# GBATZOLIS/ID-diff

Measured on AMD Instinct MI355X. Metric: score-vector evals/sec (rows of S per second incl. the per-point spectrum), 32x32 ncsnpp, higher is better.
Workload: dtype f32 (3x3 convs: Winograd, fp32 transforms, contraction on pairs of fp16 values -- 22 significand bits, 3 products, fp32 accumulate (F(4,3) along the rows x 3 filter rows); 1x1/attention/dense contractions: fp32 operands split exactly into 3 bf16, 6 partial products, fp32 accumulate; the q/k/v projec

## Files before the change

### id-diff_amd/_lib.py

```python
import ctypes
import os
import subprocess
from typing import NamedTuple, Optional

import torch

_HERE = os.path.dirname(os.path.abspath(__file__))
_VARIANT = os.environ.get("IDIFF_LIB_VARIANT", "")
_LIB_PATH = os.path.join(_HERE, "csrc", f"libidiff_hip.{_VARIANT}.so" if _VARIANT else "libidiff_hip.so")
_lib = None

ACT = {None: 0, "none": 0, "linear": 0, "silu": 1, "swish": 1, "elu": 2, "relu": 3, "lrelu": 4}

c_i, c_i64, c_f, c_d, c_p = ctypes.c_int, ctypes.c_int64, ctypes.c_float, ctypes.c_double, ctypes.c_void_p


class Epilogue(ctypes.Structure):
    _fields_ = [("bias", c_p), ("rowbias", c_p), ("ld_rowbias", c_i64), ("rows_per_group", c_i), ("act", c_i),
                ("residual", c_p), ("ld_residual", c_i64), ("out_scale", c_f), ("rowscale", c_p), ("colstats", c_p)]


_SIGNATURES = {
    "idiff_abi_version": (c_i, []),
    "idiff_last_error": (ctypes.c_char_p, []),
    "idiff_source_stamp": (ctypes.c_char_p, []),
    "idiff_variant_flags": (ctypes.c_char_p, []),
    "idiff_set_option": (c_i, [ctypes.c_char_p, c_i]),
    "idiff_gemm_pairs_ok": (c_i, [c_i, c_i, c_i, c_i]),
    "idiff_gemm_pairs_scale_f32": (c_i, [c_p, c_i64, c_i, c_i, c_p, c_p]),
    "idiff_gemm_pairs_f32": (c_i, [c_p, c_i64, c_i64, c_p, c_i64, c_i64, c_p, c_i, c_p, c_p, c_i64, c_i64, c_i, c_i, c_i, c_i, c_p, c_p]),
    "idiff_pairs_act_scale_f32": (c_i, [c_p, c_i, c_i, c_p, c_i, c_i, c_i, c_i, c_p, c_p]),
    "idiff_gemm_pairs_2src_f32": (c_i, [c_p, c_p, c_i64, c_i, c_p, c_p, c_i64, c_p, c_p, c_i64, c_i, c_i, c_i, c_p, c_p]),
    "idiff_set_thread_option": (c_i, [ctypes.c_char_p, c_i, c_i]),
    "idiff_upfirdn2d_f32": (c_i, [c_p, c_p, c_p] + [c_i] * 14 + [c_p]),
    "idiff_upfirdn2d_route": (ctypes.c_char_p, [c_p, c_p] + [c_i] * 14),
    "idiff_upfirdn2d_gn_f32": (c_i, [c_p, c_p, c_p, c_i, c_p] + [c_i] * 14 + [c_p]),
    "idiff_upfirdn2d_gn_ok": (c_i, [c_p, c_p, c_i, c_p] + [c_i] * 14),
    "idiff_fused_bias_act_f32": (c_i, [c_p, c_p, c_p, c_p, c_i64, c_i, c_i, c_i, c_i, c_f, c_f, c_p]),
    "idiff_upfirdn2d_f16": (c_i, [c_p, c_p, c_p] + [c_i] * 14 + [c_p]),
    "idiff_upfirdn2d_f64": (c_i, [c_p, c_p, c_p] + [c_i] * 14 + [c_p]),
    "idiff_fused_bias_act_f16": (c_i, [c_p, c_p, c_p, c_p, c_i64, c_i, c_i, c_i, c_i, c_f, c_f, c_p]),
    "idiff_fused_bias_act_f64": (c_i, [c_p, c_p, c_p, c_p, c_i64, c_i, c_i, c_i, c_i, c_f, c_f, c_p]),
    "idiff_gemm_f32": (c_i, [c_p, c_i64, c_i64, c_p, c_i64, c_i64, c_p, c_i64, c_i64, c_i, c_i, c_i, c_i,
                             ctypes.POINTER(Epilogue), c_p]),
    "idiff_gemm_2src_f32": (c_i, [c_p, c_p, c_i64, c_i, c_p, c_i64, c_p, c_i64, c_i, c_i, c_i, ctypes.POINTER(Epilogue), c_p]),
    "idiff_conv2d_nhwc_f32": (c_i, [c_p, c_p, c_p] + [c_i] * 10 + [ctypes.POINTER(Epilogue), c_p]),
    "idiff_gemm_route": (ctypes.c_char_p, [c_p, c_i64, c_i64, c_p, c_i64, c_i64, c_p, c_i64, c_i64, c_i, c_i, c_i, c_i,
                                           ctypes.POINTER(Epilogue), c_i]),
    "idiff_conv2d_route": (ctypes.c_char_p, [c_p, c_p, c_p] + [c_i] * 10 + [ctypes.POINTER(Epilogue)]),
    "idiff_gemm_colstats_split": (c_i, [c_i, c_i, c_i, c_i64, c_i64, c_i]),
    "idiff_conv2d_colstats_split": (c_i, [c_i] * 10),
    "idiff_conv2d_winograd_ok": (c_i, [c_i] * 5),
    "idiff_winograd_weight_floats": (c_i64, [c_i, c_i]),
    "idiff_winograd_pack_f32": (c_i, [c_p, c_p, c_i, c_i, c_p]),
    "idiff_conv2d_winograd_f32": (c_i, [c_p, c_p, c_p] + [c_i] * 5 + [ctypes.POINTER(Epilogue), c_p]),
    "idiff_conv2d_winograd_colstats_split": (c_i, [c_i] * 5),
    "idiff_conv2d_winograd43_ok": (c_i, [c_i] * 5),
    "idiff_conv2d_winograd43_colstats_split": (c_i, [c_i] * 5),
    "idiff_winograd43_weight_floats": (c_i64, [c_i, c_i]),
    "idiff_winograd43_pack_f32": (c_i, [c_p, c_p, c_i, c_i, c_p]),
    "idiff_conv2d_winograd43_f32": (c_i, [c_p, c_p, c_p, c_i, c_i, c_i, c_i, c_i, ctypes.POINTER(Epilogue), c_p]),
    "idiff_conv2d_winograd43h_ok": (c_i, [c_i] * 5),
    "idiff_winograd43h_weight_floats": (c_i64, [c_i, c_i]),
    "idiff_winograd43h_pack_f32": (c_i, [c_p, c_p, c_i, c_i, c_p]),
    "idiff_conv2d_winograd43h_f32": (c_i, [c_p, c_p, c_p, c_i, c_i, c_i, c_i, c_i, ctypes.POINTER(Epilogue), c_p]),
    "idiff_conv2d_wino1d_ok": (c_i, [c_i] * 5),
    "idiff_conv2d_wino1d_colstats_split": (c_i, [c_i] * 5),
    "idiff_wino1d_weight_floats": (c_i64, [c_i, c_i]),
    "idiff_wino1d_pack_f32": (c_i, [c_p, c_p, c_i, c_i, c_p]),
    "idiff_conv2d_wino1d_f32": (c_i, [c_p, c_p, c_p, c_i, c_i, c_i, c_i, c_i, ctypes.POINTER(Epilogue), c_p]),
    "idiff_conv2d_wino1d_gn_ok": (c_i, [c_i] * 6),
    "idiff_conv2d_wino1d_normload_ok": (c_i, [c_i] * 5),
    "idiff_conv2d_wino1d_normload_f32": (c_i, [c_p, c_p, c_p, c_i, c_i, c_i, c_i, c_i, ctypes.POINTER(Epilogue), c_p, c_i, c_p]),
    "idiff_conv2d_wino1d_normload_2src_ok": (c_i, [c_i] * 6),
    "idiff_conv2d_wino1d_normload_2src_f32": (c_i, [c_p, c_i, c_p, c_i, c_p, c_p, c_i, c_i, c_i, c_i, ctypes.POINTER(Epilogue), c_p, c_i, c_p]),
    "idiff_groupnorm_coef_f32": (c_i, [c_p, c_i, c_i, c_p, c_i, c_i, c_i, c_i, c_i, c_f, c_p, c_p, c_p, c_p]),
    "idiff_conv2d_wino1d_gn_f32": (c_i, [c_p, c_p, c_p, c_i, c_i, c_i, c_i, c_i, ctypes.POINTER(Epilogue), c_i, c_p, c_p, c_f, c_i, c_p]),
    "idiff_conv2d_winograd_split_ok": (c_i, [c_i] * 5),
    "idiff_winograd_split_weight_floats": (c_i64, [c_i, c_i]),
    "idiff_winograd_pack_split_f32": (c_i, [c_p, c_p, c_i, c_i, c_p]),
    "idiff_conv2d_winograd_split_f32": (c_i, [c_p, c_p, c_p] + [c_i] * 5 + [ctypes.POINTER(Epilogue), c_p]),
    "idiff_groupnorm_finalize_f32": (c_i, [c_p, c_i, c_i, c_p, c_i, c_i, c_i, c_i, c_i, c_f, c_p, c_p]),
    "idiff_groupnorm_nsplit": (c_i, [c_i, c_i, c_i]),
    "idiff_groupnorm_stats_f32": (c_i, [c_p, c_i, c_p, c_i, c_i, c_i, c_i, c_f, c_p, c_p, c_p]),
    "idiff_groupnorm_apply_f32": (c_i, [c_p, c_i, c_p, c_i, c_i, c_i, c_i, c_p, c_p, c_p, c_p, c_i64, c_i, c_p, c_p]),
    "idiff_groupnorm_apply_colstats_f32": (c_i, [c_p, c_i, c_p, c_i, c_i, c_i, c_i, c_p, c_i, c_p, c_i, c_f, c_p, c_p, c_p, c_i64,
                                                 c_i, c_p, c_p]),
    "idiff_groupnorm_apply_route": (ctypes.c_char_p, [c_p, c_i, c_p, c_i, c_i, c_i, c_i, c_p, c_p, c_p, c_p]),
    "idiff_groupnorm_apply_colstats_route": (ctypes.c_char_p, [c_p, c_i, c_p, c_i, c_i, c_i, c_i, c_p, c_i, c_p, c_i, c_p, c_p, c_p]),
    "idiff_softmax_rows_f32": (c_i, [c_p, c_p, c_i64, c_i, c_f, c_p]),
    "idiff_softmax_rows_route": (ctypes.c_char_p, [c_p, c_p, c_i64, c_i, c_f]),
    "idiff_attention256_ok": (c_i, [c_i, c_i, c_i]),
    "idiff_attention256_f32": (c_i, [c_p, c_i64, c_p, c_p, c_p, c_p, c_p, c_i, c_i, c_i, c_f, c_p]),
    "idiff_attention_heads_ok": (c_i, [c_i, c_i, c_i, c_i]),
    "idiff_attention_heads_f32": (c_i, [c_p, c_i64, c_p, c_p, c_p, c_p, c_p, c_i, c_i, c_i, c_i, c_f, c_p]),
    "idiff_attention256_route": (ctypes.c_char_p, [c_p, c_i64, c_p, c_p, c_p, c_p, c_p, c_i, c_i, c_i]),
    "idiff_attention_heads_route": (ctypes.c_char_p, [c_p, c_i64, c_p, c_p, c_p, c_p, c_p, c_i, c_i, c_i, c_i]),
    "idiff_affine_act_f32": (c_i, [c_p, c_p, c_i64, c_f, c_f, c_i, c_p, c_i64, c_p]),
    "idiff_add_scale_f32": (c_i, [c_p, c_p, c_p, c_i64, c_f, c_p]),
    "idiff_affine_act_route": (ctypes.c_char_p, [c_p, c_p, c_i64, c_p, c_i64]),
    "idiff_add_scale_route": (ctypes.c_char_p, [c_p, c_p, c_p, c_i64]),
    "idiff_concat_cols_route": (ctypes.c_char_p, [c_p, c_i, c_p, c_i, c_p, c_i64]),
    "idiff_fourier_embed_f32": (c_i, [c_p, c_p, c_p, c_i, c_i, c_p]),
    "idiff_positional_embed_f32": (c_i, [c_p, c_p, c_i, c_i, c_f, c_i, c_p]),
    "idiff_concat_cols_f32": (c_i, [c_p, c_i, c_p, c_i, c_p, c_i64, c_p]),
    "idiff_nchw_to_nhwc_f32": (c_i, [c_p, c_p, c_i, c_i, c_i, c_i, c_f, c_f, c_p]),
    "idiff_nhwc_to_nchw_f32": (c_i, [c_p, c_p, c_i, c_i, c_i, c_i, c_p, c_p]),
    "idiff_resample2x_nhwc_f32": (c_i, [c_p, c_p, c_i, c_i, c_i, c_i, c_i, c_p]),
    "idiff_perturb_f32": (c_i, [c_p, c_p, c_p, c_p, c_p, c_i64, c_i64, c_p]),
    "idiff_perturb_randn_f32": (c_i, [c_p, c_p, c_p, c_p, c_i64, c_i64, c_i64, ctypes.c_uint64, c_p, c_p]),
    "idiff_spectrum_workspace_bytes": (c_i64, [c_i, c_i, c_i]),
    "idiff_spectrum_f32": (c_i, [c_p, c_i, c_i, c_i, c_p, c_i64, c_p, c_p, c_p]),
    "idiff_colmean_f64": (c_i, [c_p, c_i, c_i, c_i, c_p, c_p, c_p]),
    "idiff_centered_gram_f64": (c_i, [c_p, c_p, c_i, c_i, c_i, c_p, c_p]),
    "idiff_centered_gram_rows_f64": (c_i, [c_p, c_p, c_i, c_i, c_i, c_i, c_p, c_p]),
    "idiff_symmetrize_upper_f64": (c_i, [c_p, c_i, c_p]),
    "idiff_symtridiag_scratch_doubles": (c_i64, [c_i]),
    "idiff_symband_ld": (c_i, []),
    "idiff_symband_f64": (c_i, [c_p, c_i, c_p, c_p]),
    "idiff_symtridiag_f64": (c_i, [c_p, c_i, c_i, c_p, c_p, c_p, c_p]),
    "idiff_symtridiag_plan": (c_i, [c_i]),
    "idiff_tridiag_eigvals_f64": (c_i, [c_p, c_p, c_i, c_i, c_p, c_p]),
    "idiff_sym_lowvecs_scratch_doubles": (c_i64, [c_i, c_i]),
    "idiff_sym_lowvecs_f64": (c_i, [c_p, c_i, c_i, c_p, c_p, c_p, c_p, c_p]),
    "idiff_sym_topvecs_scratch_doubles": (c_i64, [c_i, c_i, c_i]),
    "idiff_sym_topvecs_f64": (c_i, [c_p, c_i, c_i, c_i, c_d, c_d, c_d, c_i, c_i, c_p, c_p, c_p, c_p, c_p]),
    "idiff_knn_workspace_bytes": (c_i64, [c_i, c_i, c_i]),
    "idiff_knn_f32": (c_i, [c_p, c_i, c_i, c_i, c_p, c_i64, c_p, c_p, c_p, c_p]),
    "idiff_apsp_tile": (c_i, []),
    "idiff_knn_graph_f64": (c_i, [c_p, c_p, c_i, c_i, c_p, c_p]),
    "idiff_apsp_f64": (c_i, [c_p, c_i, c_p]),
    "idiff_double_center_scratch_doubles": (c_i64, [c_i]),
    "idiff_double_center_f64": (c_i, [c_p, c_i, c_p, c_p, c_p, c_p]),
    "idiff_component_labels_f64": (c_i, [c_p, c_i, c_p, c_p, c_p, c_p]),
    "idiff_component_bridges_workspace_bytes": (c_i64, [c_i]),
    "idiff_component_bridges_f64": (c_i, [c_p, c_i, c_i, c_p, c_i, c_p, c_i64, c_p, c_p, c_p, c_p]),
    "idiff_minplus_f64": (c_i, [c_p, c_i64, c_p, c_i64, c_p, c_i64, c_i, c_i, c_i, c_p]),
    "idiff_symmetrize_min_f64": (c_i, [c_p, c_i, c_p]),
    "idiff_knn_cross_workspace_bytes": (c_i64, [c_i, c_i]),
    "idiff_knn_cross_f64": (c_i, [c_p, c_i, c_p, c_i, c_i, c_i, c_p, c_i64, c_p, c_p, c_p]),
    "idiff_isomap_project_scratch_doubles": (c_i64, [c_i]),
    "idiff_isomap_project_f64": (c_i, [c_p, c_p, c_i, c_i, c_p, c_i, c_p, c_i, c_p, c_p, c_p, c_p, c_p]),
    "idiff_render_squares_f32": (c_i, [c_p, c_p, c_p, c_i, c_i, c_i, c_p]),
    "idiff_render_gaussians_f32": (c_i, [c_p, c_p, c_p, c_i, c_i, c_i, c_p]),
    "idiff_ksphere_union_ok": (c_i, [c_i, c_i, c_i]),
    "idiff_ksphere_union_score_f32": (c_i, [c_p, c_p, c_p, c_p, c_p, c_p, c_p, c_i, c_i, c_i, c_i, c_p]),
    "idiff_local_pca_ok": (c_i, [c_i, c_i, c_i, c_i]),
    "idiff_local_pca_chunk": (c_i, []),
    "idiff_local_pca_f64": (c_i, [c_p, c_i, c_i, c_p, c_p, c_i, c_i, c_i, c_p, c_p, c_p, c_p]),
    "idiff_empirical_score_ok": (c_i, [c_i64, c_i]),
    "idiff_empirical_score_f32": (c_i, [c_p, c_p, c_p, c_p, c_p, c_p, c_p, c_p, c_i, c_i64, c_i, c_p]),
    "idiff_empirical_jacobian_ok": (c_i, [c_i64, c_i]),
    "idiff_empirical_jacobian_f64": (c_i, [c_p, c_p, c_p, c_p, c_p, c_p, c_i, c_i64, c_i, c_p]),
    "idiff_gemm_nn_ok": (c_i, [c_i, c_i, c_i]),
    "idiff_gemm_nn_f32": (c_i, [c_p, c_i64, c_p, c_i64, c_p, c_i64, c_p, c_i64, c_i, c_i, c_i, c_p]),
    "idiff_gemm_tn_ok": (c_i, [c_i, c_i, c_i]),
    "idiff_gemm_tn_f32": (c_i, [c_p, c_i64, c_p, c_i64, c_p, c_i64, c_p, c_i, c_i, c_i, c_p]),
    "idiff_dsm_loss_grad_f32": (c_i, [c_p, c_p, c_p, c_p, c_i64, c_p, c_p, c_i, c_i, c_i, c_p]),
    "idiff_grad_sumsq_f32": (c_i, [c_p, c_i64, c_p, c_p, c_p]),
    "idiff_adam_step_f32": (c_i, [c_p, c_p, c_p, c_p, c_i64, c_p, c_d, c_d, c_d, c_d, c_d, c_d, c_i64, c_p]),
    "idiff_fcn_train_input_f32": (c_i, [c_p, c_p, c_p, c_p, c_p, c_p, c_i64, c_i, c_i, c_p]),
    "idiff_sampler_step_f32": (c_i, [c_p, c_i64, c_p, c_i64, c_p, c_i64, c_p, c_i64, c_p, c_i64, c_i64, c_i, c_d, c_d, c_d, c_p, c_d, c_d,
                                     ctypes.c_uint64, c_i64, c_i, c_f, c_p]),
    "idiff_sampler_noise_norm_f32": (c_i, [c_p, c_i64, c_i64, c_i, ctypes.c_uint64, c_i64, c_p, c_p, c_p]),
    "idiff_jvp_layer_ok": (c_i, [c_i, c_i, c_i]),
    "idiff_jvp_seed_f32": (c_i, [c_p, c_i64, c_p, c_i64, c_p, c_i64, c_i64, c_i, c_i, c_i, c_p]),
    "idiff_jvp_layer_f32": (c_i, [c_p, c_i64, c_i64, c_p, c_i64, c_p, c_i64, c_p, c_i64, c_i64, c_i, c_i, c_i, c_i, c_p]),
    "idiff_rk_stage_f64": (c_i, [c_p, c_i64, c_p, c_i64, c_i64, c_p, c_i, c_p, c_i64, c_p, c_i64, c_i64, c_i, c_i, c_f, c_p]),
    "idiff_rk_error_f64": (c_i, [c_p, c_i64, c_i64, c_p, c_p, c_i64, c_p, c_i64, c_i64, c_i, c_d, c_d, c_p, c_p, c_p]),
    "idiff_flow_rhs_f64": (c_i, [c_p, c_i64, c_p, c_i64, c_d, c_d, c_p, c_i64, c_i64, c_i, c_i, c_p, c_i64, c_p, c_i64, c_p, c_p]),
    "idiff_jvp_trace_f64": (c_i, [c_p, c_i64, c_i64, c_p, c_i64, c_p, c_i, c_i, c_i, c_p]),
}

EXPORTED_SYMBOLS = tuple(_SIGNATURES)


def library_path():
    return _LIB_PATH


def build(verbose=False):
    out = subprocess.run(["bash", os.path.join(_HERE, "csrc", "build.sh")], capture_output=True, text=True)
    if out.returncode != 0:
        raise RuntimeError("building libidiff_hip.so failed:\n" + out.stdout + out.stderr)
    if verbose:
        print(out.stdout.strip())
    return _LIB_PATH


def source_stamp():
    import hashlib
    csrc = os.path.join(_HERE, "csrc")
    names = sorted(f for f in os.listdir(csrc) if f.endswith(".hip") or f.endswith(".h"))
    h = hashlib.sha256()
    for f in [os.path.join(csrc, n) for n in names] + [os.path.join(os.path.dirname(_HERE), "include", "idiff_hip.h")]:
        with open(f, "rb") as fh:
            h.update(fh.read())
    return h.hexdigest()[:16]
# ... 48 lines not shown
    def __exit__(self, *exc):
        lib().idiff_set_thread_option(self.name, 0, 0)
        return False


def _check(rc, what):
    if rc != 0:
        msg = lib().idiff_last_error().decode(errors="replace")
        raise RuntimeError(f"{what} failed (code {rc}): {msg}")


def _stream():
    return torch.cuda.current_stream().cuda_stream


def _dev(t, name, dtype=torch.float32, contiguous=True):
    if not isinstance(t, torch.Tensor):
        raise TypeError(f"{name}: expected a torch.Tensor, got {type(t).__name__}")
    if t.device.type != "cuda":
        raise RuntimeError(f"{name}: expected a tensor on the MI355X (cuda device), got {t.device}; "
                           "id-diff_amd has no CPU path")
    if t.dtype != dtype:
        raise RuntimeError(f"{name}: expected dtype {dtype}, got {t.dtype}")
    if contiguous and not t.is_contiguous():
        raise RuntimeError(f"{name}: expected a contiguous tensor")
    return t


def _ptr(t):
    return 0 if t is None else t.data_ptr()


def make_epilogue(bias=None, rowbias=None, rows_per_group=1, act=None, residual=None, out_scale=1.0,
                  ld_rowbias=None, ld_residual=None, rowscale=None, colstats=None):
    ep = Epilogue()
    ep.bias = _ptr(bias)
    ep.rowbias = _ptr(rowbias)
    ep.ld_rowbias = (rowbias.stride(0) if ld_rowbias is None else ld_rowbias) if rowbias is not None else 0
    ep.rows_per_group = int(rows_per_group)
    ep.act = ACT[act]
    ep.residual = _ptr(residual)
    ep.ld_residual = (residual.shape[-1] if ld_residual is None else ld_residual) if residual is not None else 0
    ep.out_scale = float(out_scale)
    ep.rowscale = _ptr(rowscale)
    ep.colstats = _ptr(colstats)
    ep._keepalive = (bias, rowbias, residual, rowscale, colstats)
    return ep


def with_groupnorm(ep, groups, gamma, beta, eps, act):
    _dev(gamma, "gamma"); _dev(beta, "beta")
    ep.groupnorm = (int(groups), gamma, beta, float(eps), ACT[act])
    return ep


class NormLoad(NamedTuple):
    coef: torch.Tensor
    act: int
    x2: Optional[torch.Tensor]
    C1: Optional[int]


def with_normload(ep, coef, act, x2=None, C1=None):
    _dev(coef, "coef")
    if (x2 is None) != (C1 is None):
        raise RuntimeError("with_normload: a second source x2 and the first one's channel count C1 come together or not at all")
    if x2 is not None:
        _dev(x2, "x2")
    ep.normload = NormLoad(coef, ACT[act], x2, None if C1 is None else int(C1))
    return ep


def _ep_ref(epilogue, what):
    if epilogue is None:
        return None
    if getattr(epilogue, "normload", None) is not None:
        raise RuntimeError(f"{what}: the epilogue asks for a GroupNorm in the loader (with_normload), which only conv2d_wino1d serves")
    if getattr(epilogue, "groupnorm", None) is not None:
        raise RuntimeError(f"{what}: the epilogue asks for a fused GroupNorm (with_groupnorm), which only conv2d_wino1d serves")
    return ctypes.byref(epilogue)


OP_DTYPES = {torch.float32: "f32", torch.float16: "f16", torch.float64: "f64"}


def op_suffix(t, name):
    try:
        return OP_DTYPES[t.dtype]
    except KeyError:
        raise RuntimeError(f"{name}: dtype {t.dtype} is not one of float32 / float16 / float64 (the reference's native ops "
                           "dispatch on floating types and half, op/upfirdn2d_kernel.cu:311)") from None


def upfirdn2d_raw(x, k, out, major, in_h, in_w, minor, up_x, up_y, down_x, down_y, px0, px1, py0, py1):
    kh, kw = k.shape
    sfx = op_suffix(x, "upfirdn2d")
    if k.dtype != x.dtype or out.dtype != x.dtype:
        raise RuntimeError(f"upfirdn2d: input {x.dtype}, kernel {k.dtype} and output {out.dtype} must share one dtype")
    fn = getattr(lib(), "idiff_upfirdn2d_" + sfx)
    _check(fn(x.data_ptr(), k.data_ptr(), out.data_ptr(), major, in_h, in_w, minor, kh, kw,
              up_x, up_y, down_x, down_y, px0, px1, py0, py1, _stream()), "idiff_upfirdn2d_" + sfx)


def upfirdn2d_route(x, out, major, in_h, in_w, minor, kh, kw, up_x, up_y, down_x, down_y, px0, px1, py0, py1):
    addr = lambda t: t if isinstance(t, int) else t.data_ptr()
    name = lib().idiff_upfirdn2d_route(addr(x), addr(out), major, in_h, in_w, minor, kh, kw, up_x, up_y, down_x, down_y,
                                       px0, px1, py0, py1)
    return None if name is None else name.decode()


def upfirdn2d_gn(x, k, coef, act, out, major, in_h, in_w, minor, up_x, up_y, down_x, down_y, px0, px1, py0, py1):
    kh, kw = k.shape
    for t, name in ((x, "input"), (k, "kernel"), (coef, "coef"), (out, "output")):
        _dev(t, name)
    if coef.numel() != major * minor * 2:
        raise RuntimeError(f"upfirdn2d_gn: coef holds {coef.numel()} floats, [major, minor, 2] = {major * minor * 2} expected")
    _check(lib().idiff_upfirdn2d_gn_f32(x.data_ptr(), k.data_ptr(), coef.data_ptr(), ACT[act], out.data_ptr(), major, in_h, in_w, minor,
                                        kh, kw, up_x, up_y, down_x, down_y, px0, px1, py0, py1, _stream()), "idiff_upfirdn2d_gn_f32")


def upfirdn2d_gn_ok(x, coef, act, out, major, in_h, in_w, minor, kh, kw, up_x, up_y, down_x, down_y, px0, px1, py0, py1):
    addr = lambda t: t if isinstance(t, int) else t.data_ptr()
    return bool(lib().idiff_upfirdn2d_gn_ok(addr(x), addr(coef), ACT[act], addr(out), major, in_h, in_w, minor, kh, kw, up_x, up_y,
                                            down_x, down_y, px0, px1, py0, py1))


def upfirdn2d_out_size(in_size, up, down, pad0, pad1, k):
    return (in_size * up + pad0 + pad1 - k) // down + 1


def fused_bias_act(x, bias, ref, act, grad, alpha, scale):
    sfx = op_suffix(x, "fused_bias_act")
    _dev(x, "input", dtype=x.dtype)
    out = torch.empty_like(x)
    has_b = bias is not None and bias.numel() > 0
    has_r = ref is not None and ref.numel() > 0
    if has_b:
        _dev(bias, "bias", dtype=x.dtype)
        if x.ndim < 2 or bias.numel() != x.shape[1]:
            raise RuntimeError(f"bias has {bias.numel()} entries but input dim 1 is {tuple(x.shape)}")
    if has_r:
        _dev(ref, "refer", dtype=x.dtype)
        if ref.shape != x.shape:
            raise RuntimeError("refer must have the shape of input")
    step_b = 1
    for d in x.shape[2:]:
        step_b *= d
    _check(getattr(lib(), "idiff_fused_bias_act_" + sfx)(x.data_ptr(), _ptr(bias if has_b else None), _ptr(ref if has_r else None),
                                                         out.data_ptr(), x.numel(), step_b, bias.numel() if has_b else 0, act, grad,
                                                         alpha, scale, _stream()), "idiff_fused_bias_act_" + sfx)
    return out


def gemm(a, bt, out=None, epilogue=None, M=None, N=None, K=None, lda=None, ldb=None, ldc=None,
         batch=1, stride_a=0, stride_b=0, stride_c=0):
    explicit = M is not None
    _dev(a, "a", contiguous=not explicit); _dev(bt, "bt", contiguous=not explicit)
    if M is None:
        M, K = a.shape
        N = bt.shape[0]
        if bt.shape[1] != K:
            raise RuntimeError(f"gemm: inner dimensions differ: {tuple(a.shape)} x {tuple(bt.shape)}^T")
        lda, ldb = a.stride(0), bt.stride(0)
    if out is None:
        out = torch.empty((M, N) if batch == 1 else (batch, M, N), device=a.device, dtype=torch.float32)
        ldc = N
        stride_c = M * N
    elif ldc is None:
        ldc = out.stride(-2)
    _dev(out, "out", contiguous=not explicit)
    ep = _ep_ref(epilogue, "gemm")
    _check(lib().idiff_gemm_f32(a.data_ptr(), lda, stride_a, bt.data_ptr(), ldb, stride_b, out.data_ptr(), ldc, stride_c,
                                M, N, K, batch, ep, _stream()), "idiff_gemm_f32")
    return out


def gemm_pairs_ok(M, N, K, batch=1):
    return bool(lib().idiff_gemm_pairs_ok(M, N, K, batch))


def gemm_pairs_scale(w):
    _dev(w, "w")
    out = torch.empty(2, device=w.device, dtype=torch.float32)
    _check(lib().idiff_gemm_pairs_scale_f32(w.data_ptr(), w.stride(0), w.shape[0], w.shape[1], out.data_ptr(), _stream()),
           "idiff_gemm_pairs_scale_f32")
    return out


def gemm_pairs(a, bt, w_scale, out, epilogue=None, weight_is_a=False, M=None, N=None, K=None, lda=None, ldb=None, ldc=None,
               batch=1, stride_a=0, stride_b=0, stride_c=0, act_scale=None):
    explicit = M is not None
    _dev(a, "a", contiguous=not explicit); _dev(bt, "bt", contiguous=not explicit); _dev(out, "out", contiguous=not explicit)
    _dev(w_scale, "w_scale")
    if M is None:
        M, K = a.shape
        N = bt.shape[0]
        if bt.shape[1] != K or out.shape[0] != M or out.shape[1] != N:
            raise RuntimeError(f"gemm_pairs: shapes {tuple(a.shape)} x {tuple(bt.shape)}^T -> {tuple(out.shape)}")
        lda, ldb, ldc = a.stride(0), bt.stride(0), out.stride(0)
    ep = _ep_ref(epilogue, "gemm_pairs")
    _check(lib().idiff_gemm_pairs_f32(a.data_ptr(), lda, stride_a, bt.data_ptr(), ldb, stride_b, w_scale.data_ptr(), int(bool(weight_is_a)),
                                      _ptr(act_scale), out.data_ptr(), ldc, stride_c, M, N, K, batch, ep, _stream()), "idiff_gemm_pairs_f32")
    return out


def pairs_act_scale(stats1, C1, stats2, C2, B, HW):
    out = torch.empty(8, device=stats1[0].device, dtype=torch.float32)
    _check(lib().idiff_pairs_act_scale_f32(stats1[0].data_ptr(), stats1[1], C1, _ptr(stats2[0]) if stats2 is not None else None,
                                           stats2[1] if stats2 is not None else 0, C2, B, HW, out.data_ptr(), _stream()),
           "idiff_pairs_act_scale_f32")
    return out


def gemm_pairs_2src(a1, a2, act_scale, bt, w_scale, out, epilogue=None):
    _dev(a1, "a1"); _dev(a2, "a2"); _dev(bt, "bt"); _dev(out, "out"); _dev(act_scale, "act_scale"); _dev(w_scale, "w_scale")
    M, K1 = a1.shape
    K = K1 + a2.shape[1]
    if a2.shape[0] != M or a1.stride(0) != a2.stride(0) or bt.shape[1] != K:
        raise RuntimeError(f"gemm_pairs_2src: shapes {tuple(a1.shape)} | {tuple(a2.shape)} x {tuple(bt.shape)}^T")
    ep = _ep_ref(epilogue, "gemm_pairs_2src")
    _check(lib().idiff_gemm_pairs_2src_f32(a1.data_ptr(), a2.data_ptr(), a1.stride(0), K1, act_scale.data_ptr(), bt.data_ptr(), bt.stride(0),
                                           w_scale.data_ptr(), out.data_ptr(), out.stride(0), M, bt.shape[0], K, ep, _stream()),
           "idiff_gemm_pairs_2src_f32")
    return out


def gemm_normed(cache, a, w, out, epilogue=None, pairs=True):
    M, K = a.shape
    if not pairs or not gemm_pairs_ok(M, w.shape[0], K):
        return gemm(a, w, out=out, epilogue=epilogue)
    return gemm_pairs(a, w, _pairs_scale_of(cache, w), out, epilogue=epilogue)


def _pairs_scale_of(cache, w):
    sc = cache.setdefault("pairs_scale", {})
    if id(w) not in sc:
        sc[id(w)] = (gemm_pairs_scale(w), w)
    return sc[id(w)][0]


def gemm_weight_times_normed_t(cache, w, x, out, B, HW, C, pairs=True):
    kw = dict(M=C, N=HW, K=C, lda=C, ldb=C, ldc=HW, batch=B, stride_a=0, stride_b=HW * C, stride_c=C * HW)
    if not pairs or not gemm_pairs_ok(C, HW, C, B):
        return gemm(w, x, out=out, **kw)
    return gemm_pairs(w, x, _pairs_scale_of(cache, w), out, weight_is_a=True, **kw)


def gemm_2src(a1, a2, bt, out, epilogue=None):
    _dev(a1, "a1"); _dev(a2, "a2"); _dev(bt, "bt"); _dev(out, "out")
    M, K1 = a1.shape
    K = K1 + a2.shape[1]
    if a2.shape[0] != M or a1.stride(0) != a2.stride(0) or bt.shape[1] != K:
        raise RuntimeError(f"gemm_2src: shapes {tuple(a1.shape)} | {tuple(a2.shape)} x {tuple(bt.shape)}^T")
    ep = _ep_ref(epilogue, "gemm_2src")
    _check(lib().idiff_gemm_2src_f32(a1.data_ptr(), a2.data_ptr(), a1.stride(0), K1, bt.data_ptr(), bt.stride(0), out.data_ptr(),
                                     out.stride(0), M, bt.shape[0], K, ep, _stream()), "idiff_gemm_2src_f32")
    return out


def conv2d_nhwc(x, wt, out, B, H, W, Cin, Cout, KH, KW, stride, pad, epilogue=None, pad_hi=None):
    ep = _ep_ref(epilogue, "conv2d_nhwc")
    _check(lib().idiff_conv2d_nhwc_f32(x.data_ptr(), wt.data_ptr(), out.data_ptr(), B, H, W, Cin, Cout, KH, KW, stride,
                                       pad, pad if pad_hi is None else pad_hi, ep, _stream()), "idiff_conv2d_nhwc_f32")
    return out


def _addr(t):
    return t if isinstance(t, int) else t.data_ptr()


def gemm_route(a, bt, out, M, N, K, lda, ldb, ldc, epilogue=None, batch=1, stride_a=0, stride_b=0, stride_c=0, pairs=False):
    name = lib().idiff_gemm_route(_addr(a), lda, stride_a, _addr(bt), ldb, stride_b, _addr(out), ldc, stride_c, M, N, K, batch,
                                  _ep_ref(epilogue, "gemm_route"), int(bool(pairs)))
    return None if name is None else name.decode()


def conv2d_route(x, wt, out, B, H, W, Cin, Cout, KH, KW, stride, pad, epilogue=None, pad_hi=None):
    name = lib().idiff_conv2d_route(_addr(x), _addr(wt), _addr(out), B, H, W, Cin, Cout, KH, KW, stride, pad, pad if pad_hi is None else pad_hi,
                                    _ep_ref(epilogue, "conv2d_route"))
    return None if name is None else name.decode()


def _wino_pack(stem, name, wt, Cin, Cout):
    _dev(wt, "wt")
    if tuple(wt.shape) != (Cout, 3, 3, Cin):
        raise RuntimeError(f"{name}: expected {Cout}x3x3x{Cin} weights, got {tuple(wt.shape)}")
    entry = "idiff_winograd_pack_split_f32" if stem == "winograd_split" else f"idiff_{stem}_pack_f32"
    u = torch.empty(getattr(lib(), f"idiff_{stem}_weight_floats")(Cin, Cout), device=wt.device, dtype=torch.float32)
    _check(getattr(lib(), entry)(wt.data_ptr(), u.data_ptr(), Cin, Cout, _stream()), entry)
    return u


def _wino_conv(stem, packed_by, x, u, out, B, H, W, Cin, Cout, epilogue):
    want = getattr(lib(), f"idiff_{stem}_weight_floats")(Cin, Cout)
    if u.numel() != want:
        raise RuntimeError(f"conv2d_{stem}: a filter bank of {u.numel()} floats ({want} expected): pack it with {packed_by}")
    gn = getattr(epilogue, "groupnorm", None)
    nl = getattr(epilogue, "normload", None)
    if nl is not None and stem == "wino1d":
        if gn is not None:
            raise RuntimeError("conv2d_wino1d: a GroupNorm in the loader (with_normload) and one in the tail (with_groupnorm) in one launch")
        if nl.coef.numel() != B * Cin * 2:
            raise RuntimeError(f"conv2d_wino1d: {nl.coef.numel()} loader coefficients for [B, Cin, 2] = [{B}, {Cin}, 2]")
        if nl.x2 is not None:
            _check(lib().idiff_conv2d_wino1d_normload_2src_f32(x.data_ptr(), nl.C1, nl.x2.data_ptr(), Cin - nl.C1, u.data_ptr(), out.data_ptr(),
                                                               B, H, W, Cout, ctypes.byref(epilogue), nl.coef.data_ptr(), nl.act, _stream()),
                   "idiff_conv2d_wino1d_normload_2src_f32")
        else:
            _check(lib().idiff_conv2d_wino1d_normload_f32(x.data_ptr(), u.data_ptr(), out.data_ptr(), B, H, W, Cin, Cout, ctypes.byref(epilogue),
                                                          nl.coef.data_ptr(), nl.act, _stream()), "idiff_conv2d_wino1d_normload_f32")
        return out
    if gn is not None and stem == "wino1d":
        groups, gamma, beta, eps, act = gn
        if gamma.numel() != Cout or beta.numel() != Cout:
            raise RuntimeError(f"conv2d_wino1d: fused GroupNorm with {gamma.numel()} / {beta.numel()} gamma / beta entries for {Cout} channels")
        _check(lib().idiff_conv2d_wino1d_gn_f32(x.data_ptr(), u.data_ptr(), out.data_ptr(), B, H, W, Cin, Cout, ctypes.byref(epilogue), groups,
                                                gamma.data_ptr(), beta.data_ptr(), eps, act, _stream()), "idiff_conv2d_wino1d_gn_f32")
        return out
    ep = _ep_ref(epilogue, f"conv2d_{stem}")
    entry = f"idiff_conv2d_{stem}_f32"
    _check(getattr(lib(), entry)(x.data_ptr(), u.data_ptr(), out.data_ptr(), B, H, W, Cin, Cout, ep, _stream()), entry)
    return out


def conv2d_winograd_ok(B, H, W, Cin, Cout):
    return bool(lib().idiff_conv2d_winograd_ok(B, H, W, Cin, Cout))


def conv2d_winograd_split_ok(B, H, W, Cin, Cout):
    return bool(lib().idiff_conv2d_winograd_split_ok(B, H, W, Cin, Cout))


def conv2d_winograd_colstats_split(B, H, W, Cin, Cout):
    return lib().idiff_conv2d_winograd_colstats_split(B, H, W, Cin, Cout)


def winograd_pack(wt, Cin, Cout, split=False):
    return _wino_pack("winograd_split" if split else "winograd", "winograd_pack", wt, Cin, Cout)


def conv2d_winograd(x, u, out, B, H, W, Cin, Cout, epilogue=None, split=False):
    return _wino_conv("winograd_split" if split else "winograd", f"winograd_pack(..., split={split})", x, u, out, B, H, W, Cin, Cout, epilogue)


def conv2d_winograd43_ok(B, H, W, Cin, Cout):
    return bool(lib().idiff_conv2d_winograd43_ok(B, H, W, Cin, Cout))


def conv2d_winograd43h_ok(B, H, W, Cin, Cout):
    return bool(lib().idiff_conv2d_winograd43h_ok(B, H, W, Cin, Cout))


def conv2d_winograd43_colstats_split(B, H, W, Cin, Cout):
    return lib().idiff_conv2d_winograd43_colstats_split(B, H, W, Cin, Cout)


def winograd43_pack(wt, Cin, Cout, pairs=False):
    return _wino_pack("winograd43h" if pairs else "winograd43", "winograd43_pack", wt, Cin, Cout)


def conv2d_winograd43(x, u, out, B, H, W, Cin, Cout, epilogue=None, pairs=False):
    if pairs:
        return _wino_conv("winograd43h", "winograd43_pack(..., pairs=True)", x, u, out, B, H, W, Cin, Cout, epilogue)
    return _wino_conv("winograd43", "winograd43_pack", x, u, out, B, H, W, Cin, Cout, epilogue)


def conv2d_wino1d_ok(B, H, W, Cin, Cout):
    return bool(lib().idiff_conv2d_wino1d_ok(B, H, W, Cin, Cout))


def conv2d_wino1d_colstats_split(B, H, W, Cin, Cout):
    return lib().idiff_conv2d_wino1d_colstats_split(B, H, W, Cin, Cout)


def conv2d_wino1d_gn_ok(B, H, W, Cin, Cout, groups):
    return bool(lib().idiff_conv2d_wino1d_gn_ok(B, H, W, Cin, Cout, groups))


def conv2d_wino1d_normload_ok(B, H, W, Cin, Cout):
    return bool(lib().idiff_conv2d_wino1d_normload_ok(B, H, W, Cin, Cout))


def conv2d_wino1d_normload_2src_ok(B, H, W, C1, C2, Cout):
    return bool(lib().idiff_conv2d_wino1d_normload_2src_ok(B, H, W, C1, C2, Cout))


def groupnorm_coef(ws1, ns1, C1, ws2, ns2, C2, B, HW, G, eps, gamma, beta, coef):
    _dev(coef, "coef"); _dev(gamma, "gamma"); _dev(beta, "beta")
    if coef.numel() != B * (C1 + (C2 if ws2 is not None else 0)) * 2:
        raise RuntimeError(f"groupnorm_coef: coef holds {coef.numel()} floats, [B, C, 2] = {B * (C1 + C2) * 2} expected")
    _check(lib().idiff_groupnorm_coef_f32(ws1.data_ptr(), ns1, C1, _ptr(ws2), ns2, C2, B, HW, G, eps, gamma.data_ptr(), beta.data_ptr(),
                                          coef.data_ptr(), _stream()), "idiff_groupnorm_coef_f32")
    return coef


def groupnorm_reader_coef(ws, ns, C, B, HW, G, eps, gamma, beta, coef):
    _dev(coef, "coef"); _dev(gamma, "gamma"); _dev(beta, "beta")
    if coef.numel() != B * C * 2:
        raise RuntimeError(f"groupnorm_reader_coef: coef holds {coef.numel()} floats, [B, C, 2] = {B * C * 2} expected")
    _check(lib().idiff_groupnorm_coef_f32(ws.data_ptr(), ns, C, 0, 0, 0, B, HW, G, eps, gamma.data_ptr(), beta.data_ptr(),
                                          coef.data_ptr(), _stream()), "idiff_groupnorm_coef_f32")
    return coef


def wino1d_pack(wt, Cin, Cout):
    return _wino_pack("wino1d", "wino1d_pack", wt, Cin, Cout)

# ... 1114 lines not shown
```

### id-diff_amd/csrc/common.h

```cpp
#pragma once
#include <hip/hip_runtime.h>
#include <stdint.h>
#include <stdio.h>
#include <stdarg.h>

#include "../../include/idiff_hip.h"

#define IDIFF_API extern "C" __attribute__((visibility("default")))

namespace idiff {

void set_error(const char *fmt, ...);

inline int fail(const char *fmt, ...) {
  char buf[512];
  va_list ap;
  va_start(ap, fmt);
  vsnprintf(buf, sizeof(buf), fmt, ap);
  va_end(ap);
  set_error("%s", buf);
  return IDIFF_EINVAL;
}

inline int launch_status(const char *what) {
  hipError_t e = hipGetLastError();
  if (e != hipSuccess) {
    set_error("%s: %s", what, hipGetErrorString(e));
    return (int)e;
  }
  return 0;
}

enum Option { OPT_NO_WINOGRAD, OPT_NO_COLSTATS, OPT_NO_PIPE, OPT_SCALAR_EPILOGUE, OPT_DBUF_ONLY, OPT_TRIDIAG_ONESTAGE,
              OPT_UFD_ROWS, OPT_CHASE_WAVEFRONT, OPT_WINO_NGROUP, OPT_GRAM_SMALL_TILES, OPT_CHASE_SPIN_LIMIT, OPT_FAKE_CU_COUNT,
              OPT_SBR_SYNC, OPT_SBR_FULL, OPT_NO_SPLIT, OPT_WINO_SPLIT, OPT_SBR_LOOKAHEAD, OPT_NO_WINO43, OPT_NO_WINO43H, OPT_NO_PAIRS, OPT_PAIRS_MIN_TILES, OPT_NO_FUSED_ATTN, OPT_NO_WINO1D, OPT_NO_FUSED_GN, OPT_NO_FUSED_GN_LOAD, OPT_NO_FUSED_GN_LOAD_2SRC, OPT_NO_FUSED_GN_FIR, OPT_COUNT };
bool option(Option o);
int option_value(Option o);

struct AttrGuard { unsigned long long done_mask = 0; };
int set_dynamic_lds_once(AttrGuard &g, const void *const *fns, int n_fns, int bytes, const char *what);

bool conv3x3_narrow_ok(int B, int H, int W, int Cin, int Cout, int KH, int KW, int stride, int pad_lo, int pad_hi,
                       const idiff_epilogue *ep);
int conv3x3_narrow(const float *x, const float *wt, float *out, int B, int H, int W, int Cin, int Cout,
                   const idiff_epilogue *ep, hipStream_t stream);

template <class P> inline void set_epilogue(P &p, const idiff_epilogue *ep) {
  p.has_ep = ep ? 1 : 0;
  p.ep = ep ? *ep : idiff_epilogue{};
  if (!ep) p.ep.out_scale = 1.f;
  if (p.ep.rows_per_group <= 0) p.ep.rows_per_group = 1;
}

inline idiff_epilogue shift_epilogue(const idiff_epilogue &ep, int64_t m0) {
  idiff_epilogue e = ep;
  const int64_t g0 = m0 / (ep.rows_per_group > 0 ? ep.rows_per_group : 1);
  if (e.rowbias) e.rowbias += g0 * ep.ld_rowbias;
  if (e.residual) e.residual += m0 * ep.ld_residual;
  if (e.rowscale) e.rowscale += g0;
  return e;
}
inline int64_t host_cut_row(int64_t units, int64_t unit_rows, const idiff_epilogue *ep) {
  const int64_t rpg = (ep && ep->rows_per_group > 0) ? ep->rows_per_group : 1;
  const int64_t half = units / 2 * unit_rows;
  return unit_rows == 1 ? half / rpg * rpg : half % rpg ? 0 : half;
}
template <class Run> inline int run_cut(int64_t rows, int64_t cut, const idiff_epilogue *ep, bool first_only, Run run) {
  if (int rc = run((int64_t)0, cut, ep)) return rc;
  if (first_only) return 0;
  idiff_epilogue hi;
  if (ep) hi = shift_epilogue(*ep, cut);
  return run(cut, rows, ep ? &hi : nullptr);
}

static inline int ceil_div(int a, int b) { return (a + b - 1) / b; }
static inline int64_t ceil_div64(int64_t a, int64_t b) { return (a + b - 1) / b; }

static inline int streaming_grid(int64_t work_items, int block) {
  int64_t g = ceil_div64(work_items, block);
  const int64_t cap = 256 * 8;
  if (g > cap) g = cap;
  if (g < 1) g = 1;
  return (int)g;
}

__device__ __forceinline__ float act_apply(float v, int act) {
  switch (act) {
    case IDIFF_ACT_SILU: return v * __frcp_rn(1.0f + __expf(-v));
    case IDIFF_ACT_ELU: return v > 0.f ? v : (expf(v) - 1.0f);
    case IDIFF_ACT_RELU: return v > 0.f ? v : 0.f;
    case IDIFF_ACT_LRELU: return v > 0.f ? v : 0.2f * v;
    default: return v;
  }
}

}
```

### id-diff_amd/csrc/igemm.hip

```cpp
#include "common.h"
#include <type_traits>
#include <stdlib.h>

namespace {

typedef float floatx16 __attribute__((ext_vector_type(16)));

constexpr int BK = 32;
constexpr int LDS_PITCH = BK + 4;

struct IgemmParams {
  const float *A;
  const float *Bt;
  float *C;
  int64_t lda, ldb, ldc;
  int64_t strideA, strideB, strideC;
  int M, N, K;
  int tiles_m, tiles_n;
  int H, W, Cin, OH, OW, KW, stride, pad;
  idiff_epilogue ep;
  int has_ep;
  uint32_t a_bytes, b_bytes;
  int vec_ep;
  const float *A2;
  int K1;
  uint32_t a2_bytes;
  uint32_t c_bytes, res_bytes;
  int buf_ep;
  const float *scale_a, *scale_b;
};

__device__ __forceinline__ float4 ldg4(const float *p) { return *reinterpret_cast<const float4 *>(p); }

template <int BM, int BN, int WARPS_M, int WARPS_N, bool CONV, bool VEC>
__global__ void __launch_bounds__(WARPS_M *WARPS_N * 64)
igemm_kernel(const IgemmParams p) {
  constexpr int T = WARPS_M * WARPS_N * 64;
  constexpr int WTM = BM / WARPS_M, WTN = BN / WARPS_N;
  constexpr int TM = WTM / 32, TN = WTN / 32;
  constexpr int A_PER_T = BM * (BK / 4) / T;
  constexpr int B_PER_T = BN * (BK / 4) / T;
  static_assert(A_PER_T >= 1 && B_PER_T >= 1, "tile too small for the thread count");
  static_assert(T % (BK / 4) == 0, "a thread keeps one k-column of float4s");

  extern __shared__ __attribute__((aligned(16))) float lds[];
  float *As = lds;
  float *Bs = lds + 2 * BM * LDS_PITCH;

  const int nwg = p.tiles_m * p.tiles_n;
  int bid = blockIdx.x;
  {
    const int q = nwg >> 3, r = nwg & 7, xcd = bid & 7, local = bid >> 3;
    bid = (xcd < r ? xcd * (q + 1) : r * (q + 1) + (xcd - r) * q) + local;
  }
  const int tile_n = bid % p.tiles_n, tile_m = bid / p.tiles_n;
  const int batch = blockIdx.y;
  const int m0 = tile_m * BM, n0 = tile_n * BN;

  const int tid = threadIdx.x, lane = tid & 63, wave = tid >> 6;
  const int wm0 = (wave / WARPS_N) * WTM, wn0 = (wave % WARPS_N) * WTN;

  const float *Ab = p.A + (int64_t)batch * p.strideA;
  const float *Bb = p.Bt + (int64_t)batch * p.strideB;

  const int kc = (tid & 7) * 4;
  const int row_base = tid >> 3;
  constexpr int ROW_STEP = T / 8;

  int64_t a_off[A_PER_T];
  int a_iy[A_PER_T], a_ix[A_PER_T];
  bool a_ok[A_PER_T];
#pragma unroll
  for (int i = 0; i < A_PER_T; ++i) {
    const int m = m0 + row_base + i * ROW_STEP;
    a_ok[i] = m < p.M;
    if (CONV) {
      const int mm = a_ok[i] ? m : 0;
      const int ox = mm % p.OW;
      const int t = mm / p.OW;
      const int oy = t % p.OH;
      const int b = t / p.OH;
      a_off[i] = (int64_t)b * p.H * p.W;
      a_iy[i] = oy * p.stride - p.pad;
      a_ix[i] = ox * p.stride - p.pad;
    } else {
      a_off[i] = (int64_t)m * p.lda;
      a_iy[i] = a_ix[i] = 0;
    }
  }
  int64_t b_off[B_PER_T];
  bool b_ok[B_PER_T];
#pragma unroll
  for (int i = 0; i < B_PER_T; ++i) {
    const int n = n0 + row_base + i * ROW_STEP;
    b_ok[i] = n < p.N;
    b_off[i] = (int64_t)n * p.ldb;
  }

  float4 a_reg[A_PER_T], b_reg[B_PER_T];

  auto load_scalar4 = [&](const float *base, int k, bool ok) -> float4 {
    float4 v = make_float4(0.f, 0.f, 0.f, 0.f);
    if (ok) {
      if (k + 0 < p.K) v.x = base[0];
      if (k + 1 < p.K) v.y = base[1];
      if (k + 2 < p.K) v.z = base[2];
      if (k + 3 < p.K) v.w = base[3];
    }
    return v;
  };

  auto fetch = [&](int kt) {
    const int k = kt * BK + kc;
    if (CONV) {
      const int tap = k / p.Cin, c = k - tap * p.Cin;
      const int ky = tap / p.KW, kx = tap - ky * p.KW;
      const bool kok = k < p.K;
#pragma unroll
      for (int i = 0; i < A_PER_T; ++i) {
        const int iy = a_iy[i] + ky, ix = a_ix[i] + kx;
        const bool ok = kok && a_ok[i] && iy >= 0 && iy < p.H && ix >= 0 && ix < p.W;
        a_reg[i] = ok ? ldg4(Ab + (a_off[i] + (int64_t)iy * p.W + ix) * p.Cin + c) : make_float4(0.f, 0.f, 0.f, 0.f);
      }
    } else {
#pragma unroll
      for (int i = 0; i < A_PER_T; ++i) {
        if (VEC) a_reg[i] = (a_ok[i] && k < p.K) ? ldg4(Ab + a_off[i] + k) : make_float4(0.f, 0.f, 0.f, 0.f);
        else a_reg[i] = load_scalar4(Ab + a_off[i] + k, k, a_ok[i]);
      }
    }
#pragma unroll
    for (int i = 0; i < B_PER_T; ++i) {
      if (VEC) b_reg[i] = (b_ok[i] && k < p.K) ? ldg4(Bb + b_off[i] + k) : make_float4(0.f, 0.f, 0.f, 0.f);
      else b_reg[i] = load_scalar4(Bb + b_off[i] + k, k, b_ok[i]);
    }
  };

  auto stage = [&](int buf) {
    float *a_dst = As + buf * BM * LDS_PITCH;
    float *b_dst = Bs + buf * BN * LDS_PITCH;
#pragma unroll
    for (int i = 0; i < A_PER_T; ++i)
      *reinterpret_cast<float4 *>(a_dst + (row_base + i * ROW_STEP) * LDS_PITCH + kc) = a_reg[i];
#pragma unroll
    for (int i = 0; i < B_PER_T; ++i)
      *reinterpret_cast<float4 *>(b_dst + (row_base + i * ROW_STEP) * LDS_PITCH + kc) = b_reg[i];
  };

  floatx16 acc[TM][TN];
#pragma unroll
  for (int i = 0; i < TM; ++i)
#pragma unroll
    for (int j = 0; j < TN; ++j)
#pragma unroll
      for (int r = 0; r < 16; ++r) acc[i][j][r] = 0.f;

  const int frag_row = lane & 31, frag_k = (lane >> 5) * 4;
  const int nkt = (p.K + BK - 1) / BK;

  fetch(0);
  stage(0);
  __syncthreads();

  for (int kt = 0; kt < nkt; ++kt) {
    const int buf = kt & 1;
    if (kt + 1 < nkt) fetch(kt + 1);
    const float *a_src = As + buf * BM * LDS_PITCH + (wm0 + frag_row) * LDS_PITCH + frag_k;
    const float *b_src = Bs + buf * BN * LDS_PITCH + (wn0 + frag_row) * LDS_PITCH + frag_k;
#pragma unroll
    for (int g = 0; g < BK / 8; ++g) {
      float4 af[TM], bf[TN];
#pragma unroll
      for (int i = 0; i < TM; ++i) af[i] = *reinterpret_cast<const float4 *>(a_src + i * 32 * LDS_PITCH + g * 8);
#pragma unroll
      for (int j = 0; j < TN; ++j) bf[j] = *reinterpret_cast<const float4 *>(b_src + j * 32 * LDS_PITCH + g * 8);
#pragma unroll
      for (int i = 0; i < TM; ++i)
#pragma unroll
        for (int j = 0; j < TN; ++j) {
          acc[i][j] = __builtin_amdgcn_mfma_f32_32x32x2f32(af[i].x, bf[j].x, acc[i][j], 0, 0, 0);
          acc[i][j] = __builtin_amdgcn_mfma_f32_32x32x2f32(af[i].y, bf[j].y, acc[i][j], 0, 0, 0);
          acc[i][j] = __builtin_amdgcn_mfma_f32_32x32x2f32(af[i].z, bf[j].z, acc[i][j], 0, 0, 0);
          acc[i][j] = __builtin_amdgcn_mfma_f32_32x32x2f32(af[i].w, bf[j].w, acc[i][j], 0, 0, 0);
        }
    }
    if (kt + 1 < nkt) stage(buf ^ 1);
    __syncthreads();
  }

  float *Cb = p.C + (int64_t)batch * p.strideC;
  const idiff_epilogue &ep = p.ep;
  const int col_l = lane & 31, row_l = (lane >> 5) * 4;
#pragma unroll
  for (int j = 0; j < TN; ++j) {
    const int n = n0 + wn0 + j * 32 + col_l;
    if (n >= p.N) continue;
    const float bias = (p.has_ep && ep.bias) ? ep.bias[n] : 0.f;
#pragma unroll
    for (int i = 0; i < TM; ++i) {
#pragma unroll
      for (int r = 0; r < 16; ++r) {
        const int m = m0 + wm0 + i * 32 + (r & 3) + 8 * (r >> 2) + row_l;
        if (m >= p.M) continue;
        float v = acc[i][j][r] + bias;
        if (p.has_ep) {
          if (ep.rowbias) v += ep.rowbias[(int64_t)(m / ep.rows_per_group) * ep.ld_rowbias + n];
          v = idiff::act_apply(v, ep.act);
          if (ep.residual) v += ep.residual[(int64_t)m * ep.ld_residual + n];
          v *= ep.out_scale;
          if (ep.rowscale) v *= ep.rowscale[m / ep.rows_per_group];
        }
        Cb[(int64_t)m * p.ldc + n] = v;
      }
    }
  }
}

template <int BM, int BN, int WARPS_M, int WARPS_N, bool CONV, bool VEC>
int launch_cfg(IgemmParams &p, int batch, hipStream_t st) {
  p.tiles_m = idiff::ceil_div(p.M, BM);
  p.tiles_n = idiff::ceil_div(p.N, BN);
  constexpr size_t lds_bytes = (size_t)2 * (BM + BN) * LDS_PITCH * sizeof(float);
  auto kern = igemm_kernel<BM, BN, WARPS_M, WARPS_N, CONV, VEC>;
  if (lds_bytes > 64 * 1024) {
    static idiff::AttrGuard guard;
    const void *fn = reinterpret_cast<const void *>(kern);
    if (int rc = idiff::set_dynamic_lds_once(guard, &fn, 1, (int)lds_bytes, "igemm")) return rc;
  }
  dim3 grid(p.tiles_m * p.tiles_n, batch);
  hipLaunchKernelGGL(kern, grid, dim3(WARPS_M * WARPS_N * 64), lds_bytes, st, p);
  return idiff::launch_status(CONV ? "igemm_conv" : "igemm_linear");
}


typedef unsigned int uintx4 __attribute__((ext_vector_type(4)));
typedef __bf16 bf16x8 __attribute__((ext_vector_type(8)));
constexpr uint32_t OOB = 0xFFFFFFFFu;

constexpr int SP = BK;
__device__ __forceinline__ int split_swz(int row) { return (row ^ (row >> 2)) & 3; }

__device__ __forceinline__ void split4(const float4 v, uint2 &p1, uint2 &p2, uint2 &p3) {
  const float x[4] = {v.x, v.y, v.z, v.w};
  uint32_t t1[4], t2[4], t3[4];
#pragma unroll
  for (int e = 0; e < 4; ++e) {
    t1[e] = __float_as_uint(x[e]) & 0xffff0000u;
    const float r1 = x[e] - __uint_as_float(t1[e]);
    t2[e] = __float_as_uint(r1) & 0xffff0000u;
    t3[e] = __float_as_uint(r1 - __uint_as_float(t2[e]));
  }
  p1 = make_uint2((t1[0] >> 16) | t1[1], (t1[2] >> 16) | t1[3]);
  p2 = make_uint2((t2[0] >> 16) | t2[1], (t2[2] >> 16) | t2[3]);
  p3 = make_uint2((t3[0] >> 16) | (t3[1] & 0xffff0000u), (t3[2] >> 16) | (t3[3] & 0xffff0000u));
}
typedef _Float16 halfx8 __attribute__((ext_vector_type(8)));
__device__ __forceinline__ void pair4(const float4 v, uint2 &hi, uint2 &lo) {
  typedef float f2 __attribute__((ext_vector_type(2)));
  typedef _Float16 h2 __attribute__((ext_vector_type(2)));
  const f2 v01 = {v.x, v.y}, v23 = {v.z, v.w};
  const h2 h01 = __builtin_convertvector(v01, h2), h23 = __builtin_convertvector(v23, h2);
  const f2 r01 = v01 - __builtin_convertvector(h01, f2), r23 = v23 - __builtin_convertvector(h23, f2);
  const h2 l01 = __builtin_convertvector(r01, h2), l23 = __builtin_convertvector(r23, h2);
  hi = make_uint2(__builtin_bit_cast(uint32_t, h01), __builtin_bit_cast(uint32_t, h23));
  lo = make_uint2(__builtin_bit_cast(uint32_t, l01), __builtin_bit_cast(uint32_t, l23));
}
bool aligned16(const void *ptr) { return ((uintptr_t)ptr & 15) == 0; }

__device__ __forceinline__ float4 buf_load4(__amdgpu_buffer_rsrc_t r, uint32_t byte_off) {
  const uintx4 v = __builtin_amdgcn_raw_buffer_load_b128(r, (int)byte_off, 0, 0);
  return __builtin_bit_cast(float4, v);
}

template <int BM, int BN, int WARPS_M, int WARPS_N, bool CONV, bool DBUF, int SPLIT>
__global__ void __launch_bounds__(WARPS_M *WARPS_N * 64, (DBUF || SPLIT) ? 2 : 4)
igemm_pipe_kernel(const IgemmParams p) {
  static_assert(!(SPLIT && DBUF), "the split form uses one LDS buffer");
  constexpr int T = WARPS_M * WARPS_N * 64;
  constexpr int WTM = BM / WARPS_M, WTN = BN / WARPS_N;
  constexpr int TM = WTM / 32, TN = WTN / 32;
  constexpr int A_PER_T = BM * (BK / 4) / T;
  constexpr int B_PER_T = BN * (BK / 4) / T;
  constexpr int ROW_STEP = T / 8;

  extern __shared__ __attribute__((aligned(16))) float lds[];
  float *As = lds;
  float *Bs = lds + (DBUF ? 2 : 1) * BM * LDS_PITCH;
  constexpr int PLANES = SPLIT == 2 ? 2 : 3;
  unsigned short *As16 = reinterpret_cast<unsigned short *>(lds);
  unsigned short *Bs16 = As16 + (DBUF ? 2 : 1) * PLANES * BM * SP;

  const int nwg = p.tiles_m * p.tiles_n;
  int bid = blockIdx.x;
  {
    const int q = nwg >> 3, r = nwg & 7, xcd = bid & 7, local = bid >> 3;
    bid = (xcd < r ? xcd * (q + 1) : r * (q + 1) + (xcd - r) * q) + local;
  }
  const int tile_n = bid % p.tiles_n, tile_m = bid / p.tiles_n;
  const int batch = blockIdx.y;
  const int m0 = tile_m * BM, n0 = tile_n * BN;
  const int tid = threadIdx.x, lane = tid & 63, wave = tid >> 6;
  const int wm0 = (wave / WARPS_N) * WTM, wn0 = (wave % WARPS_N) * WTN;

  const __amdgpu_buffer_rsrc_t rA =
      __builtin_amdgcn_make_buffer_rsrc((void *)(p.A + (int64_t)batch * p.strideA), 0, (int)p.a_bytes, 0x00020000);
  const __amdgpu_buffer_rsrc_t rB =
      __builtin_amdgcn_make_buffer_rsrc((void *)(p.Bt + (int64_t)batch * p.strideB), 0, (int)p.b_bytes, 0x00020000);
  const __amdgpu_buffer_rsrc_t rA2 =
      __builtin_amdgcn_make_buffer_rsrc((void *)(p.K1 > 0 ? p.A2 : p.A), 0, (int)(p.K1 > 0 ? p.a2_bytes : p.a_bytes), 0x00020000);

  const int kc = (tid & 7) * 4;
  const int row_base = tid >> 3;

  uint32_t a_base[A_PER_T], a_mask[A_PER_T];
#pragma unroll
  for (int i = 0; i < A_PER_T; ++i) {
    const int m = m0 + row_base + i * ROW_STEP;
    const bool ok = m < p.M;
    if (CONV) {
      const int mm = ok ? m : 0;
      const int ox = mm % p.OW;
      const int t = mm / p.OW;
      const int oy = t % p.OH;
      const int b = t / p.OH;
      const int iy0 = oy * p.stride - p.pad, ix0 = ox * p.stride - p.pad;
      a_base[i] = (uint32_t)(((b * p.H + iy0) * p.W + ix0) * p.Cin + kc) * 4u;
      uint32_t mask = 0;
      const int KH = p.K / (p.KW * p.Cin);
      for (int ky = 0; ky < KH; ++ky)
        for (int kx = 0; kx < p.KW; ++kx) {
          const int iy = iy0 + ky, ix = ix0 + kx;
          if (ok && iy >= 0 && iy < p.H && ix >= 0 && ix < p.W) mask |= 1u << (ky * p.KW + kx);
        }
      a_mask[i] = mask;
    } else {
      a_base[i] = (uint32_t)((int64_t)m * p.lda + kc) * 4u;
      a_mask[i] = ok ? 1u : 0u;
    }
  }
  uint32_t b_base[B_PER_T];
  bool b_ok[B_PER_T];
#pragma unroll
  for (int i = 0; i < B_PER_T; ++i) {
    const int n = n0 + row_base + i * ROW_STEP;
    b_ok[i] = n < p.N;
    b_base[i] = (uint32_t)((int64_t)n * p.ldb + kc) * 4u;
  }

  float4 a_reg[A_PER_T], b_reg[B_PER_T];
  int f_kt = 0, f_c0 = 0, f_tap = 0, f_ky = 0, f_kx = 0;

  const int ntaps = CONV ? p.K / p.Cin : 1;
  auto fetch = [&]() {
    const int k = f_kt * BK + kc;
    const bool kok = k < p.K;
    uint32_t koffb = (uint32_t)f_kt * (BK * 4u);
    if (CONV && p.Cin == 4) {
      const int tap = f_kt * 8 + (tid & 7);
      const int ky = tap / p.KW, kx = tap - ky * p.KW;
      const uint32_t tapoff = (uint32_t)((ky * p.W + kx) * 4 - kc) * 4u;
#pragma unroll
      for (int i = 0; i < A_PER_T; ++i) {
        const bool ok = tap < ntaps && ((a_mask[i] >> tap) & 1u);
        a_reg[i] = buf_load4(rA, ok ? a_base[i] + tapoff : OOB);
      }
    } else if (CONV) {
      const uint32_t tapoff = (uint32_t)((f_ky * p.W + f_kx) * p.Cin + f_c0) * 4u;
      koffb = (uint32_t)(f_tap * p.Cin + f_c0) * 4u;
#pragma unroll
      for (int i = 0; i < A_PER_T; ++i) {
        const bool ok = (a_mask[i] >> f_tap) & 1u;
        a_reg[i] = buf_load4(rA, ok ? a_base[i] + tapoff : OOB);
      }
      ++f_tap;
      if (++f_kx == p.KW) { f_kx = 0; ++f_ky; }
      if (f_tap == ntaps) { f_tap = 0; f_kx = 0; f_ky = 0; f_c0 += BK; }
    } else {
      const bool second = p.K1 > 0 && f_kt * BK >= p.K1;
      const __amdgpu_buffer_rsrc_t rS = second ? rA2 : rA;
      const uint32_t koff = (uint32_t)(f_kt * BK - (second ? p.K1 : 0)) * 4u;
#pragma unroll
      for (int i = 0; i < A_PER_T; ++i) a_reg[i] = buf_load4(rS, (a_mask[i] && kok) ? a_base[i] + koff : OOB);
    }
#pragma unroll
    for (int i = 0; i < B_PER_T; ++i) b_reg[i] = buf_load4(rB, (b_ok[i] && kok) ? b_base[i] + koffb : OOB);
    ++f_kt;
  };

  static_assert(ROW_STEP % 16 == 0 && BM % 32 == 0 && BN % 32 == 0, "split-plane swizzle");
  const int kc_sw = (((kc >> 3) ^ split_swz(row_base)) << 3) + (kc & 7);
  const float pair_sa = (SPLIT == 2 && p.scale_a) ? p.scale_a[0] : 1.f, pair_s = (SPLIT == 2 && p.scale_b) ? p.scale_b[0] : 1.f;
  auto stage = [&](int buf) {
    if (SPLIT == 2) {
      unsigned short *a_dst = As16, *b_dst = Bs16;
#pragma unroll
      for (int i = 0; i < A_PER_T; ++i) {
        uint2 hi, lo;
        const float4 av = a_reg[i];
        pair4(make_float4(av.x * pair_sa, av.y * pair_sa, av.z * pair_sa, av.w * pair_sa), hi, lo);
        unsigned short *d = a_dst + (row_base + i * ROW_STEP) * SP + kc_sw;
        *reinterpret_cast<uint2 *>(d) = hi;
        *reinterpret_cast<uint2 *>(d + BM * SP) = lo;
      }
#pragma unroll
      for (int i = 0; i < B_PER_T; ++i) {
        uint2 hi, lo;
        const float4 w = b_reg[i];
        pair4(make_float4(w.x * pair_s, w.y * pair_s, w.z * pair_s, w.w * pair_s), hi, lo);
        unsigned short *d = b_dst + (row_base + i * ROW_STEP) * SP + kc_sw;
        *reinterpret_cast<uint2 *>(d) = hi;
        *reinterpret_cast<uint2 *>(d + BN * SP) = lo;
      }
      return;
    }
    if (SPLIT) {
      unsigned short *a_dst = As16 + buf * 3 * BM * SP, *b_dst = Bs16 + buf * 3 * BN * SP;
#pragma unroll
      for (int i = 0; i < A_PER_T; ++i) {
        uint2 q1, q2, q3;
        split4(a_reg[i], q1, q2, q3);
        unsigned short *d = a_dst + (row_base + i * ROW_STEP) * SP + kc_sw;
        *reinterpret_cast<uint2 *>(d) = q1;
        *reinterpret_cast<uint2 *>(d + BM * SP) = q2;
        *reinterpret_cast<uint2 *>(d + 2 * BM * SP) = q3;
      }
#pragma unroll
      for (int i = 0; i < B_PER_T; ++i) {
        uint2 q1, q2, q3;
        split4(b_reg[i], q1, q2, q3);
        unsigned short *d = b_dst + (row_base + i * ROW_STEP) * SP + kc_sw;
        *reinterpret_cast<uint2 *>(d) = q1;
        *reinterpret_cast<uint2 *>(d + BN * SP) = q2;
        *reinterpret_cast<uint2 *>(d + 2 * BN * SP) = q3;
      }
      return;
    }
    float *a_dst = As + buf * BM * LDS_PITCH;
    float *b_dst = Bs + buf * BN * LDS_PITCH;
#pragma unroll
    for (int i = 0; i < A_PER_T; ++i)
      *reinterpret_cast<float4 *>(a_dst + (row_base + i * ROW_STEP) * LDS_PITCH + kc) = a_reg[i];
#pragma unroll
    for (int i = 0; i < B_PER_T; ++i)
      *reinterpret_cast<float4 *>(b_dst + (row_base + i * ROW_STEP) * LDS_PITCH + kc) = b_reg[i];
  };

  floatx16 acc[TM][TN];

  const int frag_row = lane & 31, frag_k = (lane >> 5) * 4;
  const int nkt = (p.K + BK - 1) / BK;

  fetch();
  stage(0);
  if (nkt > 1) fetch();
  __syncthreads();

  auto ktile = [&](int kt, auto first) {
    const int buf = DBUF ? (kt & 1) : 0;
    if (DBUF && !SPLIT) {
      if (kt + 1 < nkt) stage(buf ^ 1);
      if (kt + 2 < nkt) fetch();
    }
    if (SPLIT == 2) {
      const int c0 = (lane >> 5) ^ split_swz(frag_row);
      const unsigned short *a16 = As16 + (wm0 + frag_row) * SP, *b16 = Bs16 + (wn0 + frag_row) * SP;
      halfx8 af[BK / 16][TM][2], bf[BK / 16][TN][2];
#pragma unroll
      for (int s = 0; s < BK / 16; ++s) {
#pragma unroll
        for (int i = 0; i < TM; ++i)
#pragma unroll
          for (int q = 0; q < 2; ++q) af[s][i][q] = *reinterpret_cast<const halfx8 *>(a16 + (q * BM + i * 32) * SP + ((c0 ^ (2 * s)) << 3));
#pragma unroll
        for (int j = 0; j < TN; ++j)
#pragma unroll
          for (int q = 0; q < 2; ++q) bf[s][j][q] = *reinterpret_cast<const halfx8 *>(b16 + (q * BN + j * 32) * SP + ((c0 ^ (2 * s)) << 3));
      }
      constexpr int QA[3] = {1, 0, 0}, QB[3] = {0, 1, 0};
#pragma unroll
      for (int s = 0; s < BK / 16; ++s)
#pragma unroll
        for (int t = 0; t < 3; ++t)
#pragma unroll
          for (int i = 0; i < TM; ++i)
#pragma unroll
            for (int j = 0; j < TN; ++j) {
              if (decltype(first)::value && s == 0 && t == 0) {
                const floatx16 zero = {0.f, 0.f, 0.f, 0.f, 0.f, 0.f, 0.f, 0.f, 0.f, 0.f, 0.f, 0.f, 0.f, 0.f, 0.f, 0.f};
                acc[i][j] = __builtin_amdgcn_mfma_f32_32x32x16_f16(af[s][i][QA[t]], bf[s][j][QB[t]], zero, 0, 0, 0);
              } else {
                acc[i][j] = __builtin_amdgcn_mfma_f32_32x32x16_f16(af[s][i][QA[t]], bf[s][j][QB[t]], acc[i][j], 0, 0, 0);
              }
            }
    } else if (SPLIT) {
      const int c0 = (lane >> 5) ^ split_swz(frag_row);
      const unsigned short *a16 = As16 + buf * 3 * BM * SP + (wm0 + frag_row) * SP;
      const unsigned short *b16 = Bs16 + buf * 3 * BN * SP + (wn0 + frag_row) * SP;
      bf16x8 af[BK / 16][TM][3], bf[BK / 16][TN][3];
#pragma unroll
      for (int s = 0; s < BK / 16; ++s) {
#pragma unroll
        for (int i = 0; i < TM; ++i)
#pragma unroll
          for (int q = 0; q < 3; ++q) af[s][i][q] = *reinterpret_cast<const bf16x8 *>(a16 + (q * BM + i * 32) * SP + ((c0 ^ (2 * s)) << 3));
#pragma unroll
        for (int j = 0; j < TN; ++j)
#pragma unroll
          for (int q = 0; q < 3; ++q) bf[s][j][q] = *reinterpret_cast<const bf16x8 *>(b16 + (q * BN + j * 32) * SP + ((c0 ^ (2 * s)) << 3));
      }
      constexpr int PA[6] = {2, 0, 1, 1, 0, 0}, PB[6] = {0, 2, 1, 0, 1, 0};
#pragma unroll
      for (int s = 0; s < BK / 16; ++s)
#pragma unroll
        for (int t = 0; t < 6; ++t)
#pragma unroll
          for (int i = 0; i < TM; ++i)
#pragma unroll
            for (int j = 0; j < TN; ++j) {
              if (decltype(first)::value && s == 0 && t == 0) {
                const floatx16 zero = {0.f, 0.f, 0.f, 0.f, 0.f, 0.f, 0.f, 0.f, 0.f, 0.f, 0.f, 0.f, 0.f, 0.f, 0.f, 0.f};
                acc[i][j] = __builtin_amdgcn_mfma_f32_32x32x16_bf16(af[s][i][PA[t]], bf[s][j][PB[t]], zero, 0, 0, 0);
              } else {
                acc[i][j] = __builtin_amdgcn_mfma_f32_32x32x16_bf16(af[s][i][PA[t]], bf[s][j][PB[t]], acc[i][j], 0, 0, 0);
              }
            }
    }
    const float *a_src = As + buf * BM * LDS_PITCH + (wm0 + frag_row) * LDS_PITCH + frag_k;
    const float *b_src = Bs + buf * BN * LDS_PITCH + (wn0 + frag_row) * LDS_PITCH + frag_k;
#pragma unroll
    for (int g = 0; g < (SPLIT ? 0 : BK / 8); ++g) {
      float4 af[TM], bf[TN];
#pragma unroll
      for (int i = 0; i < TM; ++i) af[i] = *reinterpret_cast<const float4 *>(a_src + i * 32 * LDS_PITCH + g * 8);
#pragma unroll
      for (int j = 0; j < TN; ++j) bf[j] = *reinterpret_cast<const float4 *>(b_src + j * 32 * LDS_PITCH + g * 8);
#pragma unroll
      for (int i = 0; i < TM; ++i)
#pragma unroll
        for (int j = 0; j < TN; ++j) {
          if (decltype(first)::value && g == 0) {
            const floatx16 zero = {0.f, 0.f, 0.f, 0.f, 0.f, 0.f, 0.f, 0.f, 0.f, 0.f, 0.f, 0.f, 0.f, 0.f, 0.f, 0.f};
            acc[i][j] = __builtin_amdgcn_mfma_f32_32x32x2f32(af[i].x, bf[j].x, zero, 0, 0, 0);
          } else {
            acc[i][j] = __builtin_amdgcn_mfma_f32_32x32x2f32(af[i].x, bf[j].x, acc[i][j], 0, 0, 0);
          }
          acc[i][j] = __builtin_amdgcn_mfma_f32_32x32x2f32(af[i].y, bf[j].y, acc[i][j], 0, 0, 0);
          acc[i][j] = __builtin_amdgcn_mfma_f32_32x32x2f32(af[i].z, bf[j].z, acc[i][j], 0, 0, 0);
          acc[i][j] = __builtin_amdgcn_mfma_f32_32x32x2f32(af[i].w, bf[j].w, acc[i][j], 0, 0, 0);
        }
    }
    __syncthreads();
    if (!DBUF) {
      if (kt + 1 < nkt) stage(0);
      if (kt + 2 < nkt) fetch();
      __syncthreads();
    }
  };
  ktile(0, std::true_type());
  for (int kt = 1; kt < nkt; ++kt) ktile(kt, std::false_type());

  if (SPLIT == 2) {
    const float inv = (p.scale_a ? p.scale_a[1] : 1.f) * (p.scale_b ? p.scale_b[1] : 1.f);
#pragma unroll
    for (int i = 0; i < TM; ++i)
#pragma unroll
      for (int j = 0; j < TN; ++j)
#pragma unroll
        for (int r = 0; r < 16; ++r) acc[i][j][r] *= inv;
  }
  float *Cb = p.C + (int64_t)batch * p.strideC;
  const idiff_epilogue &ep = p.ep;
  const int col_l = lane & 31, row_l = (lane >> 5) * 4;
  const bool want_stats = p.has_ep && ep.colstats != nullptr;
  double *red = reinterpret_cast<double *>(lds);
  if (p.vec_ep && p.buf_ep) {
    constexpr int C4 = WTN / 4;
    constexpr int RPP = 64 / C4;
    constexpr int PASSES = 32 / RPP;
    constexpr uint32_t OOB_BASE = 0xF0000000u;
    float *tr = lds + (tid >> 6) * (32 * WTN);
// ... 54 lines not shown
              v[0] += rb.x; v[1] += rb.y; v[2] += rb.z; v[3] += rb.w;
            }
            if (has_rs) rsv = ep.rowscale[grp];
          }
        }
        if (act != IDIFF_ACT_NONE) {
#pragma unroll
          for (int e = 0; e < 4; ++e) v[e] = idiff::act_apply(v[e], act);
        }
        if (has_res) {
          const float4 rs = resv[t];
          v[0] += rs.x; v[1] += rs.y; v[2] += rs.z; v[3] += rs.w;
        }
        if (scaled) {
#pragma unroll
          for (int e = 0; e < 4; ++e) v[e] *= sc;
          if (!block_groups && has_rs) {
#pragma unroll
            for (int e = 0; e < 4; ++e) v[e] *= rsv;
          }
        }
        __builtin_amdgcn_raw_buffer_store_b128(__builtin_bit_cast(uintx4, make_float4(v[0], v[1], v[2], v[3])), rC,
                                               (int)(c_off + step * ldc_b), 0, 0);
        if (want_stats) {
#pragma unroll
          for (int e = 0; e < 4; ++e) { s1[e] += (double)v[e]; s2[e] += (double)v[e] * (double)v[e]; }
        }
      }
    }
    if (want_stats) {
#pragma unroll
      for (int off = C4; off < 64; off <<= 1)
#pragma unroll
        for (int e = 0; e < 4; ++e) { s1[e] += __shfl_xor(s1[e], off, 64); s2[e] += __shfl_xor(s2[e], off, 64); }
      __syncthreads();
      if (lane < C4) {
#pragma unroll
        for (int e = 0; e < 4; ++e) {
          const int slot = ((wave / WARPS_N) * BN + wn0 + c4 * 4 + e) * 2;
          red[slot] = s1[e]; red[slot + 1] = s2[e];
        }
      }
    }
  } else if (p.vec_ep) {
    constexpr int C4 = WTN / 4;
    constexpr int RPP = 64 / C4;
    constexpr int PASSES = 32 / RPP;
    float *tr = lds + (tid >> 6) * (32 * WTN);
    const int c4 = lane % C4, r0 = lane / C4;
    const int n = n0 + wn0 + c4 * 4;
    const bool n_ok = n < p.N;
    float4 bias4 = make_float4(0.f, 0.f, 0.f, 0.f);
    if (n_ok && p.has_ep && ep.bias) bias4 = *reinterpret_cast<const float4 *>(ep.bias + n);
    double s1[4] = {0.0, 0.0, 0.0, 0.0}, s2[4] = {0.0, 0.0, 0.0, 0.0};
#pragma unroll
    for (int i = 0; i < TM; ++i) {
#pragma unroll
      for (int j = 0; j < TN; ++j)
#pragma unroll
        for (int r = 0; r < 16; ++r) tr[((r & 3) + 8 * (r >> 2) + row_l) * WTN + j * 32 + col_l] = acc[i][j][r];
#pragma unroll
      for (int t = 0; t < PASSES; ++t) {
        const int row = r0 + RPP * t;
        const float4 a4 = *reinterpret_cast<const float4 *>(tr + row * WTN + c4 * 4);
        const int m = m0 + wm0 + i * 32 + row;
        if (m >= p.M || !n_ok) continue;
        float v[4] = {a4.x + bias4.x, a4.y + bias4.y, a4.z + bias4.z, a4.w + bias4.w};
        if (p.has_ep) {
          const int grp = (ep.rowbias || ep.rowscale) ? m / ep.rows_per_group : 0;
          if (ep.rowbias) {
            const float4 rb = *reinterpret_cast<const float4 *>(ep.rowbias + (int64_t)grp * ep.ld_rowbias + n);
            v[0] += rb.x; v[1] += rb.y; v[2] += rb.z; v[3] += rb.w;
          }
#pragma unroll
          for (int e = 0; e < 4; ++e) v[e] = idiff::act_apply(v[e], ep.act);
          if (ep.residual) {
            const float4 rs = *reinterpret_cast<const float4 *>(ep.residual + (int64_t)m * ep.ld_residual + n);
            v[0] += rs.x; v[1] += rs.y; v[2] += rs.z; v[3] += rs.w;
          }
          const float rsc = ep.rowscale ? ep.rowscale[grp] : 1.f;
#pragma unroll
          for (int e = 0; e < 4; ++e) { v[e] *= ep.out_scale; if (ep.rowscale) v[e] *= rsc; }
        }
        *reinterpret_cast<float4 *>(Cb + (int64_t)m * p.ldc + n) = make_float4(v[0], v[1], v[2], v[3]);
        if (want_stats) {
#pragma unroll
          for (int e = 0; e < 4; ++e) { s1[e] += (double)v[e]; s2[e] += (double)v[e] * (double)v[e]; }
        }
      }
    }
    if (want_stats) {
#pragma unroll
      for (int off = C4; off < 64; off <<= 1)
#pragma unroll
        for (int e = 0; e < 4; ++e) { s1[e] += __shfl_xor(s1[e], off, 64); s2[e] += __shfl_xor(s2[e], off, 64); }
      __syncthreads();
      if (lane < C4) {
#pragma unroll
        for (int e = 0; e < 4; ++e) {
          const int slot = ((wave / WARPS_N) * BN + wn0 + c4 * 4 + e) * 2;
          red[slot] = s1[e]; red[slot + 1] = s2[e];
        }
      }
    }
  } else {
#pragma unroll
  for (int j = 0; j < TN; ++j) {
    const int n = n0 + wn0 + j * 32 + col_l;
    const bool n_ok = n < p.N;
    const float bias = (n_ok && p.has_ep && ep.bias) ? ep.bias[n] : 0.f;
    double s1 = 0.0, s2 = 0.0;
#pragma unroll
    for (int i = 0; i < TM; ++i) {
#pragma unroll
      for (int r = 0; r < 16; ++r) {
        const int m = m0 + wm0 + i * 32 + (r & 3) + 8 * (r >> 2) + row_l;
        if (m >= p.M || !n_ok) continue;
        float v = acc[i][j][r] + bias;
        if (p.has_ep) {
          if (ep.rowbias) v += ep.rowbias[(int64_t)(m / ep.rows_per_group) * ep.ld_rowbias + n];
          v = idiff::act_apply(v, ep.act);
          if (ep.residual) v += ep.residual[(int64_t)m * ep.ld_residual + n];
          v *= ep.out_scale;
          if (ep.rowscale) v *= ep.rowscale[m / ep.rows_per_group];
        }
        Cb[(int64_t)m * p.ldc + n] = v;
        if (want_stats) { s1 += (double)v; s2 += (double)v * (double)v; }
      }
    }
    if (want_stats) {
      s1 += __shfl_xor(s1, 32, 64);
      s2 += __shfl_xor(s2, 32, 64);
      if (lane < 32) {
        const int slot = ((wave / WARPS_N) * BN + wn0 + j * 32 + col_l) * 2;
        red[slot] = s1; red[slot + 1] = s2;
      }
    }
  }
  }
  if (want_stats) {
    __syncthreads();
    for (int c = tid; c < BN; c += T) {
      const int n = n0 + c;
      if (n >= p.N) continue;
      double a = 0.0, b = 0.0;
#pragma unroll
      for (int w = 0; w < WARPS_M; ++w) { a += red[(w * BN + c) * 2]; b += red[(w * BN + c) * 2 + 1]; }
      double *dst = ep.colstats + ((int64_t)tile_m * p.N + n) * 2;
      dst[0] = a; dst[1] = b;
    }
  }
}

template <int BM, int BN, int WARPS_M, int WARPS_N, bool CONV, bool DBUF = true, int SPLIT = 0>
int launch_pipe(IgemmParams &p, int batch, hipStream_t st) {
  p.tiles_m = idiff::ceil_div(p.M, BM);
  p.tiles_n = idiff::ceil_div(p.N, BN);
  constexpr size_t stage_bytes = SPLIT ? (size_t)(DBUF ? 2 : 1) * (BM + BN) * (SPLIT == 2 ? 2 : 3) * SP * sizeof(unsigned short)
                                       : (size_t)(DBUF ? 2 : 1) * (BM + BN) * LDS_PITCH * sizeof(float);
  constexpr size_t patch_bytes = (size_t)WARPS_M * WARPS_N * 32 * (BN / WARPS_N) * sizeof(float);
  constexpr size_t lds_bytes = stage_bytes > patch_bytes ? stage_bytes : patch_bytes;
  auto kern = igemm_pipe_kernel<BM, BN, WARPS_M, WARPS_N, CONV, DBUF, SPLIT>;
  if (lds_bytes > 64 * 1024) {
    static idiff::AttrGuard guard;
    const void *fn = reinterpret_cast<const void *>(kern);
    if (int rc = idiff::set_dynamic_lds_once(guard, &fn, 1, (int)lds_bytes, "igemm")) return rc;
  }
  dim3 grid(p.tiles_m * p.tiles_n, batch);
  hipLaunchKernelGGL(kern, grid, dim3(WARPS_M * WARPS_N * 64), lds_bytes, st, p);
  return idiff::launch_status(CONV ? "igemm_pipe_conv" : "igemm_pipe_linear");
}

enum IgemmFamily { FAM_PIPE, FAM_DIRECT_VEC, FAM_DIRECT_SCALAR, FAM_NARROW };
enum IgemmArith { AR_FP32, AR_FP32_1BUF, AR_SPLIT, AR_PAIRS };
enum IgemmEpForm { EPF_BUF_BLOCK, EPF_BUF_ROW, EPF_VEC64, EPF_SCALAR };
struct IgemmPlan { int family, bm, bn, arith, ep_form; };
enum IgemmWant { WANT_PIPE, WANT_PAIRS, WANT_DIRECT_VEC, WANT_DIRECT_SCALAR };

constexpr int64_t BUF_LIMIT = 0xFFFFFFF0ll;
int64_t extent_bytes(int64_t rows, int64_t ld, int64_t row_len) { return ((rows - 1) * ld + row_len) * 4; }

IgemmPlan igemm_tile(int M, int N, int batch, int want) {
  IgemmPlan c = {};
  const int64_t wg_big = (int64_t)idiff::ceil_div(M, 128) * idiff::ceil_div(N, 128) * batch;
  const int64_t wg_mid = (int64_t)idiff::ceil_div(M, 128) * idiff::ceil_div(N, 64) * batch;
  auto tile = [&](int bm, int bn, int arith) { c.bm = bm; c.bn = bn; c.arith = arith; };
  c.ep_form = EPF_SCALAR;
  if (want == WANT_DIRECT_VEC || want == WANT_DIRECT_SCALAR) {
    c.family = want == WANT_DIRECT_VEC ? FAM_DIRECT_VEC : FAM_DIRECT_SCALAR;
    if (N > 64 && wg_big >= 256) tile(128, 128, AR_FP32);
    else if (wg_mid >= 256 || M >= 4096) tile(128, 64, AR_FP32);
    else tile(64, 64, AR_FP32);
    return c;
  }
  c.family = FAM_PIPE;
  if (want == WANT_PAIRS) tile(128, 128, AR_PAIRS);
  else if (!idiff::option(idiff::OPT_NO_SPLIT)) {
    if (N > 64 && wg_big >= 256) tile(128, 128, AR_SPLIT);
    else if (N <= 32 && M >= 4096) tile(128, 32, AR_SPLIT);
    else if (wg_mid >= 256 || M >= 4096) tile(128, 64, AR_SPLIT);
    else tile(64, 64, AR_SPLIT);
  }
  else if (N > 64 && wg_big >= 1024 && !idiff::option(idiff::OPT_DBUF_ONLY)) tile(128, 128, AR_FP32_1BUF);
  else if (N > 64 && wg_big >= 256) tile(128, 128, AR_FP32);
  else if (N <= 32 && M >= 4096) tile(128, 32, AR_FP32);
  else if (wg_mid >= 256 || M >= 4096) tile(128, 64, AR_FP32);
  else tile(64, 64, AR_FP32);
  return c;
}

IgemmPlan igemm_choose(IgemmParams &p, int batch, int want) {
  IgemmPlan c = igemm_tile(p.M, p.N, batch, want);
  if (c.family != FAM_PIPE) return c;
  const idiff_epilogue &e = p.ep;
  const bool al = (p.N % 4 == 0) && (p.ldc % 4 == 0) && (p.strideC % 4 == 0) && aligned16(p.C) &&
                  (!p.has_ep || ((!e.bias || aligned16(e.bias)) && (!e.rowbias || (aligned16(e.rowbias) && e.ld_rowbias % 4 == 0)) &&
                                 (!e.residual || (aligned16(e.residual) && e.ld_residual % 4 == 0))));
  p.vec_ep = al && !idiff::option(idiff::OPT_SCALAR_EPILOGUE);
  const int64_t c_bytes = extent_bytes(p.M, p.ldc, p.N);
  const int64_t res_bytes = (p.has_ep && e.residual) ? extent_bytes(p.M, e.ld_residual, p.N) : 0;
  const int64_t pitch = p.ldc > e.ld_residual ? p.ldc : e.ld_residual;
  p.buf_ep = p.vec_ep && c_bytes < 0xE0000000ll && res_bytes < 0xE0000000ll && (int64_t)c.bm * pitch * 4 < 0x0FFFFFF0ll;
  p.c_bytes = p.buf_ep ? (uint32_t)c_bytes : 0; p.res_bytes = p.buf_ep ? (uint32_t)res_bytes : 0;
  c.ep_form = !p.vec_ep ? EPF_SCALAR : !p.buf_ep ? EPF_VEC64 : (e.rows_per_group % 32 == 0 ? EPF_BUF_BLOCK : EPF_BUF_ROW);
  return c;
}

template <bool CONV>
int igemm_launch(const IgemmPlan &c, IgemmParams &p, int batch, hipStream_t st) {
  const int t = c.bm * 1000 + c.bn;
  if (c.family == FAM_DIRECT_VEC || c.family == FAM_DIRECT_SCALAR) {
    const bool vec = c.family == FAM_DIRECT_VEC;
    if constexpr (CONV) {
      if (vec && t == 128128) return launch_cfg<128, 128, 2, 2, true, true>(p, batch, st);
      if (vec && t == 128064) return launch_cfg<128, 64, 2, 2, true, true>(p, batch, st);
      if (vec && t == 64064) return launch_cfg<64, 64, 2, 2, true, true>(p, batch, st);
    } else {
      if (t == 128128) return vec ? launch_cfg<128, 128, 2, 2, false, true>(p, batch, st) : launch_cfg<128, 128, 2, 2, false, false>(p, batch, st);
      if (t == 128064) return vec ? launch_cfg<128, 64, 2, 2, false, true>(p, batch, st) : launch_cfg<128, 64, 2, 2, false, false>(p, batch, st);
      if (t == 64064) return vec ? launch_cfg<64, 64, 2, 2, false, true>(p, batch, st) : launch_cfg<64, 64, 2, 2, false, false>(p, batch, st);
    }
  } else if (c.family == FAM_PIPE) {
    switch (c.arith) {
      case AR_PAIRS:
        if constexpr (!CONV) { if (t == 128128) return launch_pipe<128, 128, 2, 2, false, false, 2>(p, batch, st); }
        break;
      case AR_SPLIT:
        if (t == 128128) return launch_pipe<128, 128, 2, 2, CONV, false, 1>(p, batch, st);
        if (t == 128032) return launch_pipe<128, 32, 4, 1, CONV, false, 1>(p, batch, st);
        if (t == 128064) return launch_pipe<128, 64, 2, 2, CONV, false, 1>(p, batch, st);
        if (t == 64064) return launch_pipe<64, 64, 2, 2, CONV, false, 1>(p, batch, st);
        break;
      case AR_FP32_1BUF:
        if (t == 128128) return launch_pipe<128, 128, 2, 2, CONV, false>(p, batch, st);
        break;
      case AR_FP32:
        if (t == 128128) return launch_pipe<128, 128, 2, 2, CONV>(p, batch, st);
        if (t == 128032) return launch_pipe<128, 32, 4, 1, CONV>(p, batch, st);
        if (t == 128064) return launch_pipe<128, 64, 2, 2, CONV>(p, batch, st);
        if (t == 64064) return launch_pipe<64, 64, 2, 2, CONV>(p, batch, st);
        break;
    }
  }
  return idiff::fail("igemm: no kernel for the plan (family %d, tile %d x %d, arithmetic %d)", c.family, c.bm, c.bn, c.arith);
}

const char *igemm_plan_name(const IgemmPlan &c) {
  static const char *const fam[] = {"pipe", "direct-vec", "direct-scalar", "narrow"};
  static const char *const ar[] = {"fp32", "fp32-1buf", "split", "pairs"};
  static const char *const epf[] = {"buf-block", "buf-row", "vec64", "scalar"};
  static thread_local char text[64];
  if (c.family == FAM_NARROW) snprintf(text, sizeof(text), "narrow c%d fp32 %s", c.bn, c.ep_form == 2 ? "elem" : c.ep_form == 1 ? "row" : "none");
  else snprintf(text, sizeof(text), "%s %dx%d %s %s", fam[c.family], c.bm, c.bn, ar[c.arith], epf[c.ep_form]);
  return text;
}

template <bool CONV>
int igemm_run(IgemmParams &p, int batch, int want, hipStream_t st, IgemmPlan *probe) {
  const IgemmPlan c = igemm_choose(p, batch, want);
  if (p.has_ep && p.ep.colstats && c.family == FAM_PIPE && p.M % c.bm)
    return idiff::fail("%s: colstats with M = %d rows in tiles of %d: no whole tiles (ask idiff_%s_colstats_split first)", CONV ? "conv2d" : "gemm",
                       p.M, c.bm, CONV ? "conv2d" : "gemm");
  if (probe) { *probe = c; return 0; }
  return igemm_launch<CONV>(c, p, batch, st);
}

enum PipeServes { PIPE_NO, PIPE_YES, PIPE_A_BEYOND };
bool pitches16(int K, int64_t lda, int64_t ldb) { return K % 4 == 0 && lda % 4 == 0 && ldb % 4 == 0; }
int pipe_fits_linear(int M, int N, int K, int64_t lda, int64_t ldb, int K1 = 0) {
  if (!pitches16(K, lda, ldb) || extent_bytes(N, ldb, K) >= BUF_LIMIT) return PIPE_NO;
  return extent_bytes(M, lda, K1 > K - K1 ? K1 : K - K1) < BUF_LIMIT ? PIPE_YES : PIPE_A_BEYOND;
}
int pipe_serves_linear(int M, int N, int K, int64_t lda, int64_t ldb, int K1 = 0) {
  return idiff::option(idiff::OPT_NO_PIPE) ? PIPE_NO : pipe_fits_linear(M, N, K, lda, ldb, K1);
}
int pipe_serves_conv(int B, int H, int W, int Cin, int Cout, int KH, int KW) {
  const int64_t K = (int64_t)KH * KW * Cin;
  if ((Cin % BK && Cin != 4) || KH * KW > 32 || idiff::option(idiff::OPT_NO_PIPE) || extent_bytes(Cout, K, K) >= BUF_LIMIT) return PIPE_NO;
  return extent_bytes((int64_t)B * H * W, Cin, Cin) < BUF_LIMIT ? PIPE_YES : PIPE_A_BEYOND;
}

IgemmParams igemm_params(const float *A, int64_t lda, const float *Bt, int64_t ldb, float *C, int64_t ldc, int M, int N, int K,
                         const idiff_epilogue *ep) {
  IgemmParams p = {};
  p.A = A; p.Bt = Bt; p.C = C; p.lda = lda; p.ldb = ldb; p.ldc = ldc; p.M = M; p.N = N; p.K = K;
  idiff::set_epilogue(p, ep);
  return p;
}

__global__ void __launch_bounds__(256) pairs_scale_kernel(const float *__restrict__ bt, int64_t ldb, int N, int K, float *__restrict__ out) {
  __shared__ float red[256];
  float m = 0.f;
  for (int64_t i = threadIdx.x; i < (int64_t)N * K; i += 256) m = fmaxf(m, fabsf(bt[(i / K) * ldb + (i % K)]));
  red[threadIdx.x] = m;
  __syncthreads();
  for (int off = 128; off > 0; off >>= 1) {
    if ((int)threadIdx.x < off) red[threadIdx.x] = fmaxf(red[threadIdx.x], red[threadIdx.x + off]);
    __syncthreads();
  }
  if (threadIdx.x == 0) {
    const float mx = red[0];
    int e = 0;
    if (mx > 0.f && mx < INFINITY) (void)frexpf(mx, &e);
    const int sh = mx > 0.f && mx < INFINITY ? 12 - e : 0;
    out[0] = ldexpf(1.f, sh);
    out[1] = ldexpf(1.f, -sh);
  }
}
bool pairs_geometry_ok(int M, int N, int K, int batch) {
  if (M <= 0 || N <= 64 || K <= 0 || K % 4 || batch <= 0 || batch > 65535) return false;
  const int want = idiff::option_value(idiff::OPT_PAIRS_MIN_TILES);
  return (int64_t)idiff::ceil_div(M, 128) * idiff::ceil_div(N, 128) * batch >= (want > 0 ? want : 256);
}
}

IDIFF_API int idiff_gemm_pairs_ok(int M, int N, int K, int batch) {
  if (idiff::option(idiff::OPT_NO_PIPE) || idiff::option(idiff::OPT_NO_SPLIT) || idiff::option(idiff::OPT_NO_PAIRS)) return 0;
  return pairs_geometry_ok(M, N, K, batch) ? 1 : 0;
}

IDIFF_API int idiff_gemm_pairs_scale_f32(const float *Bt, int64_t ldb, int N, int K, float *scale, void *stream) {
  using namespace idiff;
  if (!Bt || !scale) return fail("gemm_pairs_scale: null pointer");
  if (N <= 0 || K <= 0 || ldb < K) return fail("gemm_pairs_scale: bad shape N=%d K=%d ldb=%lld", N, K, (long long)ldb);
  hipLaunchKernelGGL(pairs_scale_kernel, dim3(1), dim3(256), 0, (hipStream_t)stream, Bt, ldb, N, K, scale);
  return launch_status("gemm_pairs_scale");
}

namespace {
__global__ void __launch_bounds__(256) pairs_act_scale_kernel(const double *__restrict__ ws1, int64_t n1, const double *__restrict__ ws2,
                                                              int64_t n2, double count, float *__restrict__ out) {
  __shared__ double red[256];
  double acc = 0.0;
  const int64_t stride = (int64_t)gridDim.x * 256;
  for (int64_t i = (int64_t)blockIdx.x * 256 + threadIdx.x; i < n1; i += stride) acc += ws1[2 * i + 1];
  for (int64_t i = (int64_t)blockIdx.x * 256 + threadIdx.x; i < n2; i += stride) acc += ws2[2 * i + 1];
  red[threadIdx.x] = acc;
  __syncthreads();
  for (int off = 128; off > 0; off >>= 1) {
    if ((int)threadIdx.x < off) red[threadIdx.x] += red[threadIdx.x + off];
    __syncthreads();
  }
  if (threadIdx.x == 0) {
    double *total = reinterpret_cast<double *>(out + 2);
    unsigned int *done = reinterpret_cast<unsigned int *>(out + 4);
    atomicAdd(total, red[0]);
    __threadfence();
    if (atomicAdd(done, 1u) == gridDim.x - 1) {
      __threadfence();
      const double ms = *reinterpret_cast<volatile double *>(total) / count;
      int sh = 0;
      if (ms > 0.0 && ms < 1e300) {
        int e = 0;
        (void)frexp(sqrt(ms), &e);
        sh = -e + ((sqrt(ms) * ldexp(1.0, -e) < 0.70710678118654752) ? 1 : 0);
      }
      out[0] = ldexpf(1.f, sh);
      out[1] = ldexpf(1.f, -sh);
    }
  }
}
}

IDIFF_API int idiff_pairs_act_scale_f32(const double *ws1, int nsplit1, int C1, const double *ws2, int nsplit2, int C2, int B, int HW,
                                        float *out, void *stream) {
  using namespace idiff;
  if (!ws1 || !out || nsplit1 <= 0 || C1 <= 0 || B <= 0 || HW <= 0 || (ws2 && (nsplit2 <= 0 || C2 <= 0)))
    return fail("pairs_act_scale: bad arguments");
  const int64_t n1 = (int64_t)B * nsplit1 * C1, n2 = ws2 ? (int64_t)B * nsplit2 * C2 : 0;
  hipError_t e = hipMemsetAsync(out, 0, 32, (hipStream_t)stream);
  if (e != hipSuccess) return fail("pairs_act_scale: hipMemsetAsync: %s", hipGetErrorString(e));
  const int blocks = (int)std::min<int64_t>(512, (n1 + n2 + 255) / 256);
  hipLaunchKernelGGL(pairs_act_scale_kernel, dim3(blocks), dim3(256), 0, (hipStream_t)stream, ws1, n1, ws2, n2,
                     (double)B * HW * (C1 + (ws2 ? C2 : 0)), out);
  return launch_status("pairs_act_scale");
}

namespace {
struct LinearCall {
  const char *name;
  const float *A, *A2;
  int K1;
  bool two_src;
  const float *Bt;
  float *C;
  int64_t lda, ldb, ldc, strideA, strideB, strideC;
  int M, N, K, batch;
  const idiff_epilogue *ep;
  int want;
  const float *w_scale, *act_scale;
  int weight_is_a;
};

int linear_front(const LinearCall &c, hipStream_t st, IgemmPlan *probe) {
  using namespace idiff;
  const bool pairs = c.want == WANT_PAIRS, colstats = c.ep && c.ep->colstats;
  if (c.M < 0 || c.N < 0 || c.K <= 0 || c.batch < 0 || (c.two_src && (c.K1 <= 0 || c.K1 >= c.K)))
    return c.two_src ? fail("%s: bad sizes M=%d N=%d K=%d K1=%d", c.name, c.M, c.N, c.K, c.K1)
                     : fail("%s: bad sizes M=%d N=%d K=%d batch=%d", c.name, c.M, c.N, c.K, c.batch);
  if (c.M == 0 || c.N == 0 || c.batch == 0) { if (probe) probe->family = -1; return 0; }
  if (!c.A || (c.two_src && !c.A2) || !c.Bt || !c.C || (pairs && !c.w_scale)) return fail("%s: null pointer", c.name);
  if (c.K1 % BK) return fail("%s: the split column K1 = %d must be a multiple of %d", c.name, c.K1, BK);
  if (c.lda < c.K1 || c.lda < c.K - c.K1 || c.ldb < c.K || c.ldc < c.N) return fail("%s: leading dimension smaller than the row length", c.name);
  if (pairs && !pairs_geometry_ok(c.M, c.N, c.K, c.batch))
    return fail("%s: M=%d N=%d K=%d batch=%d not served (ask idiff_gemm_pairs_ok)", c.name, c.M, c.N, c.K, c.batch);
  if (c.batch > 65535) return fail("%s: batch %d exceeds grid.y", c.name, c.batch);
  const bool vec = pitches16(c.K, c.lda, c.ldb) && c.strideA % 4 == 0 && c.strideB % 4 == 0 && aligned16(c.A) &&
                   (!c.two_src || aligned16(c.A2)) && aligned16(c.Bt);
  const int serves = !vec ? PIPE_NO : (pairs ? pipe_fits_linear : pipe_serves_linear)(c.M, c.N, c.K, c.lda, c.ldb, c.K1);
  if (serves == PIPE_A_BEYOND && c.batch == 1 && !pairs) {
    if (colstats) return fail("%s: colstats is not available for operands beyond 4 GiB", c.name);
    if (const int64_t cut = host_cut_row(c.M, 1, c.ep))
      return run_cut(c.M, cut, c.ep, probe != nullptr, [&](int64_t r0, int64_t r1, const idiff_epilogue *e) {
        LinearCall h = c;
        h.A += r0 * c.lda; h.C += r0 * c.ldc; h.M = (int)(r1 - r0); h.ep = e;
        if (c.two_src) h.A2 += r0 * c.lda;
        h.strideA = h.strideB = h.strideC = 0;
        return linear_front(h, st, probe);
      });
    if (c.two_src) return fail("%s: cannot split %d rows inside an epilogue row group of %d", c.name, c.M, c.ep ? c.ep->rows_per_group : 1);
  }
  IgemmParams p = igemm_params(c.A, c.lda, c.Bt, c.ldb, c.C, c.ldc, c.M, c.N, c.K, c.ep);
  p.strideA = c.strideA; p.strideB = c.strideB; p.strideC = c.strideC;
  if (serves != PIPE_YES) {
    if (pairs) return fail("%s: operands must be 16-byte aligned with row pitches and batch strides that are multiples of 4, one "
                           "batch slice inside 4 GiB", c.name);
    if (c.two_src) return fail("%s: operands must be 16-byte aligned with K %% 4 == 0 and lda %% 4 == 0 (use two idiff_gemm_f32 calls)", c.name);
    if (colstats) return fail("%s: colstats requested for a problem the pipelined kernel does not take "
                              "(ask idiff_gemm_colstats_split first)", c.name);
    return igemm_run<false>(p, c.batch, vec ? WANT_DIRECT_VEC : WANT_DIRECT_SCALAR, st, probe);
  }
  if (pairs && colstats && c.batch != 1) return fail("%s: colstats only for unbatched problems", c.name);
  p.a_bytes = (uint32_t)extent_bytes(c.M, c.lda, c.two_src ? c.K1 : c.K); p.b_bytes = (uint32_t)extent_bytes(c.N, c.ldb, c.K);
  if (c.two_src) { p.A2 = c.A2; p.K1 = c.K1; p.a2_bytes = (uint32_t)extent_bytes(c.M, c.lda, c.K - c.K1); }
  if (pairs) { p.scale_a = c.weight_is_a ? c.w_scale : c.act_scale; p.scale_b = c.weight_is_a ? c.act_scale : c.w_scale; }
  return igemm_run<false>(p, c.batch, c.want, st, probe);
}

LinearCall linear_call(const char *name, const float *A, int64_t lda, int64_t strideA, const float *Bt, int64_t ldb, int64_t strideB, float *C,
                       int64_t ldc, int64_t strideC, int M, int N, int K, int batch, const idiff_epilogue *ep, int want) {
  return LinearCall{name, A, nullptr, 0, false, Bt, C, lda, ldb, ldc, strideA, strideB, strideC, M, N, K, batch, ep, want, nullptr, nullptr, 0};
}
LinearCall linear_call_2src(const char *name, const float *A1, const float *A2, int64_t lda, int K1, const float *Bt, int64_t ldb, float *C,
                            int64_t ldc, int M, int N, int K, const idiff_epilogue *ep, int want) {
  LinearCall c = linear_call(name, A1, lda, 0, Bt, ldb, 0, C, ldc, 0, M, N, K, 1, ep, want);
  c.A2 = A2; c.K1 = K1; c.two_src = true;
  return c;
}
}

IDIFF_API int idiff_gemm_f32(const float *A, int64_t lda, int64_t strideA, const float *Bt, int64_t ldb,
                             int64_t strideB, float *C, int64_t ldc, int64_t strideC, int M, int N, int K,
                             int batch, const idiff_epilogue *ep, void *stream) {
  return linear_front(linear_call("gemm", A, lda, strideA, Bt, ldb, strideB, C, ldc, strideC, M, N, K, batch, ep, WANT_PIPE), (hipStream_t)stream,
                      nullptr);
}

IDIFF_API int idiff_gemm_pairs_f32(const float *A, int64_t lda, int64_t strideA, const float *Bt, int64_t ldb, int64_t strideB,
                                   const float *w_scale, int weight_is_a, const float *act_scale, float *C, int64_t ldc, int64_t strideC,
                                   int M, int N, int K, int batch, const idiff_epilogue *ep, void *stream) {
  LinearCall c = linear_call("gemm_pairs", A, lda, strideA, Bt, ldb, strideB, C, ldc, strideC, M, N, K, batch, ep, WANT_PAIRS);
  c.w_scale = w_scale; c.act_scale = act_scale; c.weight_is_a = weight_is_a;
  return linear_front(c, (hipStream_t)stream, nullptr);
}

IDIFF_API int idiff_gemm_2src_f32(const float *A1, const float *A2, int64_t lda, int K1, const float *Bt, int64_t ldb,
                                  float *C, int64_t ldc, int M, int N, int K, const idiff_epilogue *ep, void *stream) {
  return linear_front(linear_call_2src("gemm_2src", A1, A2, lda, K1, Bt, ldb, C, ldc, M, N, K, ep, WANT_PIPE), (hipStream_t)stream, nullptr);
}

IDIFF_API int idiff_gemm_pairs_2src_f32(const float *A1, const float *A2, int64_t lda, int K1, const float *act_scale, const float *Bt,
                                        int64_t ldb, const float *w_scale, float *C, int64_t ldc, int M, int N, int K,
                                        const idiff_epilogue *ep, void *stream) {
  LinearCall c = linear_call_2src("gemm_pairs_2src", A1, A2, lda, K1, Bt, ldb, C, ldc, M, N, K, ep, WANT_PAIRS);
  c.w_scale = w_scale; c.act_scale = act_scale;
  return linear_front(c, (hipStream_t)stream, nullptr);
}

IDIFF_API const char *idiff_gemm_route(const void *A, int64_t lda, int64_t strideA, const void *Bt, int64_t ldb, int64_t strideB,
                                       const void *C, int64_t ldc, int64_t strideC, int M, int N, int K, int batch,
                                       const idiff_epilogue *ep, int pairs) {
  IgemmPlan plan = {};
  LinearCall c = linear_call(pairs ? "gemm_pairs" : "gemm", (const float *)A, lda, strideA, (const float *)Bt, ldb, strideB,
                             (float *)const_cast<void *>(C), ldc, strideC, M, N, K, batch, ep, pairs ? WANT_PAIRS : WANT_PIPE);
  c.w_scale = c.Bt;
  if (linear_front(c, nullptr, &plan)) return nullptr;
  return plan.family < 0 ? "none" : igemm_plan_name(plan);
}

namespace {
int conv_front(const float *x, const float *wt, float *out, int B, int H, int W, int Cin, int Cout, int KH, int KW, int stride, int pad_lo,
               int pad_hi, const idiff_epilogue *ep, void *stream, IgemmPlan *probe) {
  using namespace idiff;
  if (B < 0 || H <= 0 || W <= 0 || Cin <= 0 || Cout <= 0 || KH <= 0 || KW <= 0 || stride <= 0 || pad_lo < 0 || pad_hi < 0)
    return fail("conv2d: bad geometry");
  if (Cin % 4 != 0) return fail("conv2d: Cin must be a multiple of 4 (pad the channels), got %d", Cin);
  if (B == 0) { if (probe) probe->family = -1; return 0; }
  if (!x || !wt || !out) return fail("conv2d: null pointer");
  if (!aligned16(x) || !aligned16(wt)) return fail("conv2d: x and wt must be 16-byte aligned");
  const int OH = (H + pad_lo + pad_hi - KH) / stride + 1, OW = (W + pad_lo + pad_hi - KW) / stride + 1;
  const int pad = pad_lo;
  if (H + pad_lo + pad_hi < KH || W + pad_lo + pad_hi < KW || OH <= 0 || OW <= 0) return fail("conv2d: empty output");
  const int64_t M64 = (int64_t)B * OH * OW;
  if (M64 > 0x7fffffff) return fail("conv2d: B*OH*OW overflows int32");
  if (conv3x3_narrow_ok(B, H, W, Cin, Cout, KH, KW, stride, pad_lo, pad_hi, ep)) {
    if (probe) {
      const int rpg = (ep && ep->rows_per_group > 0) ? ep->rows_per_group : 1;
      *probe = IgemmPlan{FAM_NARROW, 0, Cout, AR_FP32, !(ep && ep->rowscale) ? 0 : rpg % W == 0 ? 1 : 2};
      return 0;
    }
    return conv3x3_narrow(x, wt, out, B, H, W, Cin, Cout, ep, (hipStream_t)stream);
  }
  const int serves = pipe_serves_conv(B, H, W, Cin, Cout, KH, KW);
  if (ep && ep->colstats && serves != PIPE_YES)
    return fail("conv2d: colstats requested for a problem the pipelined kernel does not take "
                "(ask idiff_conv2d_colstats_split first)");
  if (serves == PIPE_A_BEYOND && B > 1) {
    if (const int64_t cut = host_cut_row(B, OH * OW, ep))
      return run_cut(M64, cut, ep, probe != nullptr, [&](int64_t r0, int64_t r1, const idiff_epilogue *e) {
        return conv_front(x + r0 / (OH * OW) * H * W * Cin, wt, out + r0 * Cout, (int)((r1 - r0) / (OH * OW)), H, W, Cin, Cout, KH, KW, stride,
                          pad_lo, pad_hi, e, stream, probe);
      });
  }
  const int K = KH * KW * Cin;
  IgemmParams p = igemm_params(x, 0, wt, K, out, Cout, (int)M64, Cout, K, ep);
  p.H = H; p.W = W; p.Cin = Cin; p.OH = OH; p.OW = OW; p.KW = KW; p.stride = stride; p.pad = pad;
  if (serves != PIPE_YES) return igemm_run<true>(p, 1, WANT_DIRECT_VEC, (hipStream_t)stream, probe);
  p.a_bytes = (uint32_t)extent_bytes((int64_t)B * H * W, Cin, Cin); p.b_bytes = (uint32_t)extent_bytes(Cout, K, K);
  return igemm_run<true>(p, 1, WANT_PIPE, (hipStream_t)stream, probe);
}
}

IDIFF_API int idiff_conv2d_nhwc_f32(const float *x, const float *wt, float *out, int B, int H, int W, int Cin,
                                    int Cout, int KH, int KW, int stride, int pad_lo, int pad_hi,
                                    const idiff_epilogue *ep, void *stream) {
  return conv_front(x, wt, out, B, H, W, Cin, Cout, KH, KW, stride, pad_lo, pad_hi, ep, stream, nullptr);
}

IDIFF_API const char *idiff_conv2d_route(const void *x, const void *wt, const void *out, int B, int H, int W, int Cin, int Cout, int KH,
                                         int KW, int stride, int pad_lo, int pad_hi, const idiff_epilogue *ep) {
  IgemmPlan c = {};
  if (conv_front((const float *)x, (const float *)wt, (float *)const_cast<void *>(out), B, H, W, Cin, Cout, KH, KW, stride, pad_lo, pad_hi, ep,
                 nullptr, &c))
    return nullptr;
  return c.family < 0 ? "none" : igemm_plan_name(c);
}


IDIFF_API int idiff_gemm_colstats_split(int M, int N, int K, int64_t lda, int64_t ldb, int rows_per_sample) {
  if (M <= 0 || N <= 0 || K <= 0 || rows_per_sample <= 0 || M % rows_per_sample || idiff::option(idiff::OPT_NO_COLSTATS)) return 0;
  if (pipe_serves_linear(M, N, K, lda, ldb) != PIPE_YES) return 0;
  const int bm = igemm_tile(M, N, 1, WANT_PIPE).bm;
  return rows_per_sample % bm == 0 ? rows_per_sample / bm : 0;
}

IDIFF_API int idiff_conv2d_colstats_split(int B, int H, int W, int Cin, int Cout, int KH, int KW, int stride, int pad_lo,
                                          int pad_hi) {
  if (B <= 0 || idiff::option(idiff::OPT_NO_COLSTATS) || pipe_serves_conv(B, H, W, Cin, Cout, KH, KW) != PIPE_YES) return 0;
  const int OH = (H + pad_lo + pad_hi - KH) / stride + 1, OW = (W + pad_lo + pad_hi - KW) / stride + 1;
  const int64_t M = (int64_t)B * OH * OW;
  if (OH <= 0 || OW <= 0 || M > 0x7fffffff) return 0;
  const int bm = igemm_tile((int)M, Cout, 1, WANT_PIPE).bm, rps = OH * OW;
  return rps % bm == 0 ? rps / bm : 0;
}
```

### id-diff_amd/csrc/runtime.hip

```cpp
#include "common.h"
#include <stdlib.h>
#include <string.h>
#include <limits.h>

namespace idiff {
static thread_local char g_err[512] = "";
void set_error(const char *fmt, ...) {
  va_list ap;
  va_start(ap, fmt);
  vsnprintf(g_err, sizeof(g_err), fmt, ap);
  va_end(ap);
}

namespace {
const char *const kOptionNames[OPT_COUNT] = {"IDIFF_NO_WINOGRAD", "IDIFF_NO_COLSTATS", "IDIFF_NO_PIPE", "IDIFF_SCALAR_EPILOGUE",
                                             "IDIFF_DBUF_ONLY", "IDIFF_TRIDIAG_ONESTAGE", "IDIFF_UFD_ROWS", "IDIFF_CHASE_WAVEFRONT",
                                             "IDIFF_WINO_NGROUP", "IDIFF_GRAM_SMALL_TILES", "IDIFF_CHASE_SPIN_LIMIT",
                                             "IDIFF_FAKE_CU_COUNT", "IDIFF_SBR_SYNC", "IDIFF_SBR_FULL", "IDIFF_NO_SPLIT", "IDIFF_WINO_SPLIT", "IDIFF_SBR_LOOKAHEAD",
                                             "IDIFF_NO_WINO43", "IDIFF_NO_WINO43H", "IDIFF_NO_PAIRS", "IDIFF_PAIRS_MIN_TILES", "IDIFF_NO_FUSED_ATTN", "IDIFF_NO_WINO1D", "IDIFF_NO_FUSED_GN", "IDIFF_NO_FUSED_GN_LOAD", "IDIFF_NO_FUSED_GN_LOAD_2SRC", "IDIFF_NO_FUSED_GN_FIR"};
struct OptionTable {
  int v[OPT_COUNT];
  OptionTable() {
    for (int i = 0; i < OPT_COUNT; ++i) { const char *e = getenv(kOptionNames[i]); v[i] = (e && *e) ? atoi(e) : 0; }
  }
};
OptionTable g_options;
constexpr int kUnset = INT_MIN;
struct ThreadOptions {
  int v[OPT_COUNT];
  ThreadOptions() { for (int i = 0; i < OPT_COUNT; ++i) v[i] = kUnset; }
};
thread_local ThreadOptions t_options;
}

int option_value(Option o) {
  const int t = t_options.v[o];
  return t != kUnset ? t : __atomic_load_n(&g_options.v[o], __ATOMIC_RELAXED);
}
bool option(Option o) { return option_value(o) != 0; }

int set_dynamic_lds_once(AttrGuard &g, const void *const *fns, int n_fns, int bytes, const char *what) {
  int dev = 0;
  hipError_t e = hipGetDevice(&dev);
  if (e != hipSuccess) { set_error("%s: hipGetDevice: %s", what, hipGetErrorString(e)); return (int)e; }
  const unsigned long long bit = 1ull << (dev & 63);
  if (__atomic_load_n(&g.done_mask, __ATOMIC_ACQUIRE) & bit) return 0;
  for (int i = 0; i < n_fns; ++i) {
    e = hipFuncSetAttribute(fns[i], hipFuncAttributeMaxDynamicSharedMemorySize, bytes);
    if (e != hipSuccess) { set_error("%s: hipFuncSetAttribute: %s", what, hipGetErrorString(e)); return (int)e; }
  }
  __atomic_fetch_or(&g.done_mask, bit, __ATOMIC_RELEASE);
  return 0;
}
}

#ifndef IDIFF_SOURCE_STAMP
#define IDIFF_SOURCE_STAMP "unstamped"
#endif
IDIFF_API int idiff_abi_version(void) { return IDIFF_ABI_VERSION; }
IDIFF_API const char *idiff_source_stamp(void) { return IDIFF_SOURCE_STAMP; }
#ifndef IDIFF_VARIANT_FLAGS
#define IDIFF_VARIANT_FLAGS ""
#endif
IDIFF_API const char *idiff_variant_flags(void) { return IDIFF_VARIANT_FLAGS; }
IDIFF_API const char *idiff_last_error(void) { return idiff::g_err; }

IDIFF_API int idiff_set_option(const char *name, int value) {
  using namespace idiff;
  if (!name) return -1;
  for (int i = 0; i < OPT_COUNT; ++i)
    if (strcmp(name, kOptionNames[i]) == 0) return __atomic_exchange_n(&g_options.v[i], value, __ATOMIC_RELAXED);
  return -1;
}

IDIFF_API int idiff_set_thread_option(const char *name, int value, int set) {
  using namespace idiff;
  if (!name) return -1;
  for (int i = 0; i < OPT_COUNT; ++i)
    if (strcmp(name, kOptionNames[i]) == 0) { t_options.v[i] = set ? value : kUnset; return 0; }
  return -1;
}
```

### id-diff_amd/models/ncsnpp.py

```python
import math
import os

import numpy as np
import torch
import torch.nn as nn

from .. import _lib
from . import utils
from .nhwc import NhwcExecutor, _T, _pad4

_INV_SQRT2 = float(1.0 / np.sqrt(2.0))


def _fan_avg_uniform(shape, scale=1.):
    scale = 1e-10 if scale == 0 else scale
    rf = np.prod(shape) / shape[1] / shape[0]
    variance = scale / ((shape[1] * rf + shape[0] * rf) / 2)
    return (torch.rand(*shape) * 2. - 1.) * np.sqrt(3 * variance)


def _conv(cin, cout, k, init_scale=1., stride=1, padding=None):
    conv = nn.Conv2d(cin, cout, k, stride=stride, padding=(k // 2 if padding is None else padding))
    conv.weight.data = _fan_avg_uniform(conv.weight.shape, init_scale)
    nn.init.zeros_(conv.bias)
# ... 168 lines not shown
                ch = out
                skips.append(ch)
            if lvl != levels - 1:
                if resblock == 'ddpm':
                    step = ["down", add(Downsample(ch, with_conv=m.resamp_with_conv, fir=self.fir)), False]
                else:
                    step = ["down", add(make_res(ch, down=True)), True]
                if prog_in == 'input_skip':
                    step += ["input_skip", add(Combine(pyr_in_ch, ch, combine))]
                    if combine == 'cat':
                        ch *= 2
                elif prog_in == 'residual':
                    step += ["residual", add(Downsample(pyr_in_ch, ch, with_conv=True, fir=self.fir))]
                    pyr_in_ch = ch
                else:
                    step += ["none", None]
                plan.append(tuple(step))
                skips.append(ch)
        ch = skips[-1]
        plan.append(("middle", add(make_res(ch)), add(AttnBlockpp(ch, init_scale)), add(make_res(ch))))
        for lvl in reversed(range(levels)):
            for _ in range(nrb + 1):
                out = nf * ch_mult[lvl]
                plan.append(("res_pop", add(make_res(ch + skips.pop(), out))))
                ch = out
            if res[lvl] in m.attn_resolutions:
                plan.append(("attn", add(AttnBlockpp(ch, init_scale))))
            if prog == 'output_skip':
                plan.append(("out_skip", add(_gn(ch)), add(_conv(ch, C, 3, init_scale=init_scale)), lvl == levels - 1))
            if lvl != 0:
                if resblock == 'ddpm':
                    if m.resamp_with_conv or not self.fir:
                        Upsample(with_conv=m.resamp_with_conv, fir=self.fir)
                    plan.append(("up", add(Upsample(with_conv=False, fir=True)), False))
                else:
                    plan.append(("up", add(make_res(ch, up=True)), True))
        assert not skips
        if prog != 'output_skip':
            plan.append(("head", add(_gn(ch)), add(_conv(ch, C, 3, init_scale=init_scale))))
        else:
            plan.append(("head_pyramid",))
        self.all_modules = nn.ModuleList(mods)
        self._plan = plan

    @staticmethod
    def _pack_nin(nin, cin_split=None):
        w = nin.W.detach().float().t().contiguous()
        if cin_split is None:
            return w
        return [w[:, :cin_split].contiguous(), w[:, cin_split:].contiguous()]

    def _pack(self):
        dev = self.device
        M = self.all_modules
        pk = {"conv": {}, "nin": {}, "gn": {}, "dense_off": {}}
        k = np.asarray(self.fir_kernel, dtype=np.float32)
        k = np.outer(k, k)
        k = k / np.sum(k)
        pk["fir_down"] = torch.tensor(k, device=dev)
        pk["fir_up"] = torch.tensor(k * 4.0, device=dev)
        pk["fir_len"] = int(k.shape[0])
        pk["fir_gain"] = {"down": float(np.abs(k).sum()), "pre_conv": float(np.abs(k).sum()),
                          "up": float(max(np.abs(4.0 * k[py::2, px::2]).sum() for py in (0, 1) for px in (0, 1)))}
        dense_w, dense_b, off = [], [], 0
        for i, mod in enumerate(M):
            if isinstance(mod, (ResnetBlockBigGANpp, ResnetBlockDDPMpp)):
                pk["dense_off"][i] = off
                dense_w.append(mod.Dense_0.weight.detach().float())
                dense_b.append(mod.Dense_0.bias.detach().float())
                off += mod.out_ch
        pk["dense_w"] = torch.cat(dense_w, 0).contiguous()
        pk["dense_b"] = torch.cat(dense_b, 0).contiguous()
        pk["dense_total"] = off
        return pk

    def _conv_w(self, pk, key, conv, cin_split=None):
        if key not in pk["conv"]:
            pk["conv"][key] = (self._pack_conv(conv, cin_split), conv.bias.detach().float().contiguous())
        return pk["conv"][key]

    def _nin_w(self, pk, key, nin, cin_split=None):
        if key not in pk["nin"]:
            pk["nin"][key] = (self._pack_nin(nin, cin_split), nin.b.detach().float().contiguous())
        return pk["nin"][key]

    def _fir(self, x, pk, mode, gn=None, act=None):
        B = x.buf.shape[0]
        n = pk["fir_len"]
        if mode == "up":
            p = n - 2
            k, up, down, p0, p1 = pk["fir_up"], 2, 1, (p + 1) // 2 + 1, p // 2
        elif mode == "down":
            p = n - 2
            k, up, down, p0, p1 = pk["fir_down"], 1, 2, (p + 1) // 2, p // 2
        else:
            p = (n - 2) + 2
            k, up, down, p0, p1 = pk["fir_down"], 1, 1, (p + 1) // 2, p // 2
        OH = _lib.upfirdn2d_out_size(x.H, up, down, p0, p1, n)
        OW = _lib.upfirdn2d_out_size(x.W, up, down, p0, p1, n)
        if gn is not None:
            if x.stats is None or x.pending is not None or _lib.ACT[act] not in (0, 1) or x.C % gn.num_groups or x.C % 4:
                return None
            coef = torch.empty(B * x.C * 2, device=x.buf.device, dtype=torch.float32)
            y = self._new(B, OH, OW, x.C, x.buf)
            if not _lib.upfirdn2d_gn_ok(x.buf, coef, act, y.buf, B, x.H, x.W, x.C, n, n, up, up, down, down, p0, p1, p0, p1):
                return None
            _lib.groupnorm_reader_coef(x.stats[0], x.stats[1], x.C, B, x.H * x.W, gn.num_groups, gn.eps, gn.weight.detach(),
                                       gn.bias.detach(), coef)
            _lib.upfirdn2d_gn(x.buf, k, coef, act, y.buf, B, x.H, x.W, x.C, up, up, down, down, p0, p1, p0, p1)
            y.norm = (gn, (x.C // gn.num_groups) * x.H * x.W, pk["fir_gain"][mode], False)
            return y
        y = self._new(B, OH, OW, x.C, x.buf)
        _lib.upfirdn2d_raw(x.buf, k, y.buf, B, x.H, x.W, x.C, up, up, down, down, p0, p1, p0, p1)
        if x.norm is not None:
            y.norm = (x.norm[0], x.norm[1], x.norm[2] * pk["fir_gain"][mode], x.norm[3])
        return y

    def _resblock(self, idx, x, temb_all, pk, x2=None):
        mod = self.all_modules[idx]
        rs = _INV_SQRT2 if self.skip_rescale else 1.0
        c_in = x.C + (x2.C if x2 is not None else 0)
        assert c_in == mod.in_ch, (c_in, mod.in_ch)
        early_shortcut = False
        if mod.up or mod.down:
            assert x2 is None
            h = self._fir(x, pk, "up" if mod.up else "down", gn=mod.GroupNorm_0, act=self.act_name) if self.fir else None
            if h is None:
                h = self._gn_act(x, mod.GroupNorm_0, self.act_name)
                h = self._fir(h, pk, "up" if mod.up else "down") if self.fir else self._box(h, mod.up)
            resample = (lambda t: self._fir(t, pk, "up" if mod.up else "down")) if self.fir else (lambda t: self._box(t, mod.up))
            early_shortcut = SHORTCUT_BEFORE_UPSAMPLE and mod.up and (hasattr(mod, "Conv_2") or hasattr(mod, "NIN_0"))
            if not early_shortcut:
                x = resample(x)
        else:
            h = self._gn_act(x, mod.GroupNorm_0, self.act_name, x2, conv_cout=mod.out_ch)
        w0, b0 = self._conv_w(pk, (idx, 0), mod.Conv_0)
        off = pk["dense_off"][idx]
        h = self._conv_gn_act(h, w0, b0, mod.GroupNorm_1, self.act_name, rowbias=temb_all[:, off:off + mod.out_ch], normed=True,
                              next_cout=mod.out_ch)
        if hasattr(mod, "Conv_2") or hasattr(mod, "NIN_0"):
            fused = x2 is not None and x.C == x2.C and x.C % 32 == 0
            split = x.C if (x2 is not None and not fused) else None
            if hasattr(mod, "Conv_2"):
                ws, bs = self._conv_w(pk, (idx, 2), mod.Conv_2, split)
                ws = [w.view(w.shape[0], -1) for w in ws] if split is not None else ws.view(ws.shape[0], -1)
            else:
                ws, bs = self._nin_w(pk, (idx, "nin"), mod.NIN_0, split)
            if early_shortcut:
                sc = resample(self._pointwise(x, ws, None))
            elif x2 is None:
                sc = self._pointwise(x, ws, bs)
            elif fused:
                sc = self._new(x.buf.shape[0], x.H, x.W, ws.shape[0], x.buf)
                _lib.gemm_2src(x.buf.view(-1, x.C), x2.buf.view(-1, x2.C), ws, sc.buf.view(-1, ws.shape[0]),
                               epilogue=_lib.make_epilogue(bias=bs))
            else:
                part = self._pointwise(x, ws[0], bs)
                sc = self._pointwise(x2, ws[1], None, residual=part.buf)
        else:
            assert x2 is None
            sc = x
        w1, b1 = self._conv_w(pk, (idx, 1), mod.Conv_1)
        if early_shortcut:
            if (idx, "1+shortcut") not in pk["conv"]:
                pk["conv"][(idx, "1+shortcut")] = (w1, (b1 + bs).contiguous())
            b1 = pk["conv"][(idx, "1+shortcut")][1]
        return self._conv(h, w1, b1, residual=sc.buf, out_scale=rs, stats=True, normed=True)

    def _attn(self, idx, x, pk):
        mod = self.all_modules[idx]
        n = self._gn_act(x, mod.GroupNorm_0, None)
        if (idx, "qk") not in pk["nin"]:
            wq, bq = self._nin_w(pk, (idx, 0), mod.NIN_0)
            wk, bk = self._nin_w(pk, (idx, 1), mod.NIN_1)
            pk["nin"][(idx, "qk")] = (torch.cat([wq, wk], 0).contiguous(), torch.cat([bq, bk], 0).contiguous())
        return self._attention(pk, x, n, mod.GroupNorm_0, *pk["nin"][(idx, "qk")], *self._nin_w(pk, (idx, 2), mod.NIN_2),
                               *self._nin_w(pk, (idx, 3), mod.NIN_3), pk["nin"], (idx, "attn_scale"),
                               out_scale=_INV_SQRT2 if self.skip_rescale else 1.0)

    def _downsample(self, idx, x, pk, **ep):
        mod = self.all_modules[idx] if isinstance(idx, int) else idx
        if mod.fir:
            if not mod.with_conv:
                return self._fir(x, pk, "down")
            key = (id(mod), "firconv")
            if key not in pk["conv"]:
                pk["conv"][key] = (self._pack_conv(mod.Conv2d_0), mod.Conv2d_0.bias.detach().float().contiguous())
            w, b = pk["conv"][key]
            return self._conv(self._fir(x, pk, "pre_conv"), w, b, stride=2, pad=0, **ep)
        if mod.with_conv:
            w, b = self._conv_w(pk, (id(mod), "conv"), mod.Conv_0)
            return self._conv(x, w, b, stride=2, pad=0, pad_hi=1, **ep)
        return self._box(x, False)

    forward_accepts_out = True

    def forward(self, x, time_cond, out_rowscale=None, out=None):
        x, time_cond = self._check_inputs(x, time_cond)
        if x.ndim != 4 or x.shape[1] != self.channels:
            raise RuntimeError(f"ncsnpp: expected [B, {self.channels}, H, W], got {tuple(x.shape)}")
        pk = self.packed()
        M = self.all_modules
        B, C, H, W = x.shape
        dev = x.device
        cp = _pad4(C)
        rs = _INV_SQRT2 if self.skip_rescale else 1.0
        temb = temb_all = h = pyr_in = pyr = None
        hs = []
        for step in self._plan:
            op = step[0]
            if op == "fourier":
                half = self.nf
                temb = torch.empty(B, 2 * half, device=dev, dtype=torch.float32)
                _lib.fourier_embed(time_cond, M[step[1]].W.detach(), temb, B, half)
            elif op == "positional":
                temb = torch.empty(B, self.nf, device=dev, dtype=torch.float32)
                _lib.positional_embed(time_cond, temb, B, self.nf)
            elif op == "temb_mlp":
                l0, l1 = M[step[1]], M[step[2]]
                t1 = _lib.gemm(temb, l0.weight.detach(), epilogue=_lib.make_epilogue(bias=l0.bias.detach(), act=self.act_name))
                t2 = _lib.gemm(t1, l1.weight.detach(), epilogue=_lib.make_epilogue(bias=l1.bias.detach(), act=self.act_name))
                temb_all = _lib.gemm(t2, pk["dense_w"], epilogue=_lib.make_epilogue(bias=pk["dense_b"]))
            elif op == "stem":
                xin = _T(torch.empty(B, H * W, cp, device=dev, dtype=torch.float32), H, W, cp)
                if self.centered:
                    _lib.nchw_to_nhwc(x, xin.buf, B, C, H * W, cp)
                else:
                    _lib.nchw_to_nhwc(x, xin.buf, B, C, H * W, cp, 2.0, -1.0)
                pyr_in = xin
                w, b = self._conv_w(pk, (step[1], "stem"), M[step[1]])
                hs = [self._conv(xin, w, b, stats=True)]
            elif op == "res_push":
                h = self._resblock(step[1], hs[-1], temb_all, pk)
                if step[2] is not None:
                    h = self._attn(step[2], h, pk)
                hs.append(h)
            elif op == "down":
                _, i_down, is_res, mode, i_pyr = step
                h = self._resblock(i_down, hs[-1], temb_all, pk) if is_res else self._downsample(i_down, hs[-1], pk)
                if mode == "input_skip":
                    pyr_in = self._downsample(self.pyramid_downsample, pyr_in, pk)
                    comb = M[i_pyr]
                    wc, bc = self._conv_w(pk, (i_pyr, "comb"), comb.Conv_0)
                    wc = wc.view(wc.shape[0], -1)
                    if comb.method == "cat":
                        h = self._cat(self._pointwise(pyr_in, wc, bc), h)
                    elif comb.method == "sum":
                        h = self._pointwise(pyr_in, wc, bc, residual=h.buf)
                    else:
                        raise ValueError(f'Method {comb.method} not recognized.')
                elif mode == "residual":
                    pyr_in = self._downsample(i_pyr, pyr_in, pk, residual=h.buf, out_scale=rs)
                    h = pyr_in
                hs.append(h)
            elif op == "middle":
                h = self._resblock(step[1], hs[-1], temb_all, pk)
                h = self._attn(step[2], h, pk)
                h = self._resblock(step[3], h, temb_all, pk)
            elif op == "res_pop":
                h = self._resblock(step[1], h, temb_all, pk, x2=hs.pop())
            elif op == "attn":
                h = self._attn(step[1], h, pk)
            elif op == "out_skip":
                n = self._gn_act(h, M[step[1]], self.act_name)
                key = (step[2], "oskip")
                if key not in pk["conv"]:
                    conv = M[step[2]]
                    wt = self._pack_conv(conv)
                    wpad = torch.zeros(cp, *wt.shape[1:], device=dev)
                    wpad[:C] = wt
                    bpad = torch.zeros(cp, device=dev)
                    bpad[:C] = conv.bias.detach().float()
                    pk["conv"][key] = (wpad.contiguous(), bpad)
                w, b = pk["conv"][key]
                if step[3]:
                    pyr = self._conv(n, w, b, normed=True)
                else:
                    pyr = self._conv(n, w, b, residual=self._fir(pyr, pk, "up").buf, normed=True)
            elif op == "up":
                h = self._resblock(step[1], h, temb_all, pk) if step[2] else self._fir(h, pk, "up")
            elif op == "up_plain":
                h = self._box(h, True)
                if M[step[1]].with_conv:
                    w, b = self._conv_w(pk, (step[1], "upconv"), M[step[1]].Conv_0)
                    h = self._conv(h, w, b)
            elif op == "head":
                n = self._gn_act(h, M[step[1]], self.act_name)
                w, b = self._conv_w(pk, (step[2], "head"), M[step[2]])
                h = self._conv(n, w, b, normed=True)
            elif op == "head_pyramid":
                h = pyr
        assert not hs
        c_out = getattr(self, "out_channels", C)
        out = self._out_buffer(out, B, c_out, H, W, dev)
        _lib.nhwc_to_nchw(h.buf, out, B, c_out, H * W, h.C, out_rowscale)
        return out
```

### id-diff_amd/models/nhwc.py

```python
from typing import Callable, NamedTuple, Optional

import torch

from .. import _lib
from .base import HipScoreModel


def _pad4(c):
    return (c + 3) // 4 * 4


class PendingNorm(NamedTuple):
    coef: torch.Tensor
    act: Optional[str]
    src: "_T"
    gn: torch.nn.Module
    src2: Optional["_T"]

    def served(self, B, H, W, cout):
        if self.src2 is None:
            return _lib.conv2d_wino1d_normload_ok(B, H, W, self.src.C, cout)
        return _lib.conv2d_wino1d_normload_2src_ok(B, H, W, self.src.C, self.src2.C, cout)


# ... 45 lines not shown
    form: Callable


CONV3X3_ROUTES = (
    Conv3x3Route("wino1d", "wino1d", _wino1d_serves, "wino1d_pack", "conv2d_wino1d_colstats_split", "conv2d_wino1d",
                 lambda *geom: {}),
    Conv3x3Route("wino43_pairs", "wino43", _wino43_pairs_serves, "winograd43_pack", "conv2d_winograd43_colstats_split",
                 "conv2d_winograd43", lambda *geom: {"pairs": True}),
    Conv3x3Route("wino43_fp32", "wino43", _wino43_fp32_serves, "winograd43_pack", "conv2d_winograd43_colstats_split",
                 "conv2d_winograd43", lambda *geom: {"pairs": False}),
    Conv3x3Route("wino22", "wino", _wino22_serves, "winograd_pack", "conv2d_winograd_colstats_split", "conv2d_winograd",
                 lambda *geom: {"split": _lib.conv2d_winograd_split_ok(*geom)}),
)


def conv3x3_route(B, H, W, cin, cout, normed, per_image):
    for route in CONV3X3_ROUTES:
        if route.serves(B, H, W, cin, cout, normed, per_image):
            return route
    return None


class NhwcExecutor(HipScoreModel):
    @staticmethod
    def _pack_conv(conv, cin_split=None):
        w = conv.weight.detach().float()
        cout, cin, kh, kw = w.shape
        parts = [w] if cin_split is None else [w[:, :cin_split], w[:, cin_split:]]
        out = []
        for part in parts:
            c = part.shape[1]
            buf = torch.zeros(cout, kh, kw, _pad4(c), device=w.device)
            buf[..., :c] = part.permute(0, 2, 3, 1)
            out.append(buf.contiguous())
        return out if cin_split is not None else out[0]

    def _new(self, B, H, W, C, like):
        return _T(torch.empty(B, H * W, C, device=like.device, dtype=torch.float32), H, W, C)

    @staticmethod
    def _colstats(y, ns, ep):
        if ns > 0:
            y.stats = (torch.empty(y.buf.shape[0] * ns * y.C * 2, device=y.buf.device, dtype=torch.float64), ns)
            ep["colstats"] = y.stats[0]

    def _gn_act(self, x, gn, act, x2=None, mod=None, conv_cout=None):
        B = x.buf.shape[0]
        HW = x.H * x.W
        C2 = x2.C if x2 is not None else 0
        G = gn.num_groups
        norm = (gn, ((x.C + C2) // G) * HW, 1.0, mod is not None)
        if conv_cout is not None and mod is None:
            deferred = self._defer_norm(x, x2, gn, act, norm, conv_cout)
            if deferred is not None:
                return deferred
        if x.stats is not None and (x2 is None or x2.stats is not None) and x.C + C2 <= 1024 and B <= 65535:
            ws2, ns2 = x2.stats if x2 is not None else (None, 0)
            y = self._new(B, x.H, x.W, x.C + C2, x.buf)
            _lib.groupnorm_apply_colstats(x.buf, x.C, x2.buf if x2 is not None else None, C2, B, HW, G, x.stats[0], x.stats[1],
                                          ws2, ns2, gn.eps, gn.weight.detach(), gn.bias.detach(), act, y.buf, mod=mod)
            y.norm = norm
            return y
        stats = torch.empty(B * G * 2, device=x.buf.device, dtype=torch.float32)
        if x.stats is not None and (x2 is None or x2.stats is not None):
            ws2, ns2 = x2.stats if x2 is not None else (None, 0)
            _lib.groupnorm_finalize(x.stats[0], x.stats[1], x.C, ws2, ns2, C2, B, HW, G, gn.eps, stats)
        else:
            nsplit = _lib.groupnorm_nsplit(B, HW, x.C + C2)
            ws = torch.empty(B * nsplit * (x.C + C2) * 2, device=x.buf.device, dtype=torch.float64)
            _lib.groupnorm_stats(x.buf, x.C, x2.buf if x2 is not None else None, C2, B, HW, G, gn.eps, ws, stats)
        y = self._new(B, x.H, x.W, x.C + C2, x.buf)
        _lib.groupnorm_apply(x.buf, x.C, x2.buf if x2 is not None else None, C2, B, HW, G, stats,
                             gn.weight.detach(), gn.bias.detach(), act, y.buf, mod=mod)
        y.norm = norm
        return y

    def _defer_norm(self, x, x2, gn, act, norm, conv_cout):
        srcs = (x,) if x2 is None else (x, x2)
        B, C = x.buf.shape[0], sum(s.C for s in srcs)
        pending = PendingNorm(None, act, x, gn, x2)
        if not (all(s.stats is not None and s.pending is None for s in srcs) and x.W == 32 and _lib.ACT[act] in (0, 1)
                and pending.served(B, x.H, x.W, conv_cout)
                and self.pairs_admissible(gn, norm[1], gain=1.0, transform=True, modulated=False)):
            return None
        route = conv3x3_route(B, x.H, x.W, C, conv_cout, True, True)
        if route is None or route.name != "wino1d":
            return None
        ws2, ns2, C2 = (*x2.stats, x2.C) if x2 is not None else (None, 0, 0)
        coef = torch.empty(B * C * 2, device=x.buf.device, dtype=torch.float32)
        _lib.groupnorm_coef(x.stats[0], x.stats[1], x.C, ws2, ns2, C2, B, x.H * x.W, gn.num_groups, gn.eps, gn.weight.detach(),
                            gn.bias.detach(), coef)
        return _T(x.buf, x.H, x.W, C, norm=norm, pending=pending._replace(coef=coef))

    def _conv(self, x, wt, bias, stride=1, pad=1, pad_hi=None, stats=False, normed=False, fuse_gn=None, **ep):
        B = x.buf.shape[0]
        cout, kh, kw, cin = wt.shape
        assert cin == x.C, (cin, x.C)
        if normed:
            assert x.norm is not None, "normed=True on a tensor that is not a GroupNorm's (resampled) output"
            gn, group_elems, gain, modulated = x.norm
            normed = self.pairs_admissible(gn, group_elems, gain=gain, transform=True, modulated=modulated)
        ph = pad if pad_hi is None else pad_hi
        OH = (x.H + pad + ph - kh) // stride + 1
        OW = (x.W + pad + ph - kw) // stride + 1
        y = self._new(B, OH, OW, cout, x.buf)
        if "rows_per_group" not in ep:
            ep["rows_per_group"] = OH * OW
        geom = (B, x.H, x.W, cin, cout)
        route = None
        if (kh, kw, stride, pad, ph) == (3, 3, 1, 1, 1):
            route = conv3x3_route(*geom, normed, ep["rows_per_group"] == OH * OW)
        pending = x.pending
        if pending is not None and (route is None or route.name != "wino1d" or not pending.served(B, x.H, x.W, cout)):
            x, pending = self._gn_act(pending.src, pending.gn, pending.act, pending.src2), None
        if route is None:
            if stats or fuse_gn is not None:
                self._colstats(y, _lib.conv2d_colstats_split(*geom, kh, kw, stride, pad, pad_hi), ep)
            _lib.conv2d_nhwc(x.buf, wt, y.buf, *geom, kh, kw, stride, pad, epilogue=_lib.make_epilogue(bias=bias, **ep), pad_hi=pad_hi)
            return (y, False) if fuse_gn is not None else y
        form = route.form(*geom)
        bank = self._packed.setdefault(route.bank, {})
        key = (id(wt), *form.values()) if form else id(wt)
        if key not in bank:
            bank[key] = (wt, getattr(_lib, route.pack)(wt, cin, cout, **form))
        if (fuse_gn is not None and pending is None and route.name == "wino1d" and _lib.conv2d_wino1d_gn_ok(*geom, fuse_gn[0].num_groups)
                and not (set(ep) - {"rowbias", "ld_rowbias", "rows_per_group"})):
            gn, act = fuse_gn
            epilogue = _lib.with_groupnorm(_lib.make_epilogue(bias=bias, **ep), gn.num_groups, gn.weight.detach(), gn.bias.detach(), gn.eps, act)
            getattr(_lib, route.launch)(x.buf, bank[key][1], y.buf, *geom, epilogue=epilogue, **form)
            y.norm = (gn, (cout // gn.num_groups) * OH * OW, 1.0, False)
            return y, True
        if stats or fuse_gn is not None:
            self._colstats(y, getattr(_lib, route.split)(*geom), ep)
        epilogue = _lib.make_epilogue(bias=bias, **ep)
        if pending is not None:
            two = pending.src2 is not None
            epilogue = _lib.with_normload(epilogue, pending.coef, pending.act, pending.src2.buf if two else None, pending.src.C if two else None)
        getattr(_lib, route.launch)(x.buf, bank[key][1], y.buf, *geom, epilogue=epilogue, **form)
        return (y, False) if fuse_gn is not None else y

    def _conv_gn_act(self, x, wt, bias, gn, act, mod=None, next_cout=None, **conv_args):
        if mod is not None:
            return self._gn_act(self._conv(x, wt, bias, stats=True, **conv_args), gn, act, mod=mod)
        y, fused = self._conv(x, wt, bias, fuse_gn=(gn, act), **conv_args)
        return y if fused else self._gn_act(y, gn, act, conv_cout=next_cout)

    def _pointwise(self, x, w, bias, stats=False, **ep):
        B = x.buf.shape[0]
        cout, cin = w.shape
        assert cin == x.C, (cin, x.C)
        y = self._new(B, x.H, x.W, cout, x.buf)
        if stats:
            self._colstats(y, _lib.gemm_colstats_split(B * x.H * x.W, cout, cin, cin, w.stride(0), x.H * x.W), ep)
        _lib.gemm(x.buf.view(-1, cin), w, out=y.buf.view(-1, cout), epilogue=_lib.make_epilogue(bias=bias, **ep))
        return y

    def _pointwise_pairs(self, pk, x, w, bias, act_scale, stats=False, **ep):
        B = x.buf.shape[0]
        cout, cin = w.shape
        M = B * x.H * x.W
        if not _lib.gemm_pairs_ok(M, cout, cin):
            return self._pointwise(x, w, bias, stats=stats, **ep)
        y = self._new(B, x.H, x.W, cout, x.buf)
        if stats:
            self._colstats(y, _lib.gemm_colstats_split(M, cout, cin, cin, w.stride(0), x.H * x.W), ep)
        _lib.gemm_pairs(x.buf.view(-1, cin), w, _lib._pairs_scale_of(pk, w), y.buf.view(-1, cout),
                        epilogue=_lib.make_epilogue(bias=bias, **ep), act_scale=act_scale)
        return y

    def _attention(self, pk, x, n, gn, wqk, bqk, wv, bv, wo, bo, cache, key, out_scale=1.0, heads=1):
        if heads != 1:
            return self._attention_heads(pk, x, n, gn, wqk, bqk, wv, bv, wo, bo, cache, key, out_scale, heads)
        B, HW, C = x.buf.shape[0], x.H * x.W, x.C
        pairs = self.pairs_admissible(gn, n.norm[1], transform=False)
        dev = x.buf.device
        qk = torch.empty(B * HW, 2 * C, device=dev, dtype=torch.float32)
        _lib.gemm_normed(pk, n.buf.view(-1, C), wqk, qk, epilogue=_lib.make_epilogue(bias=bqk), pairs=pairs)
        vt = torch.empty(B, C, HW, device=dev, dtype=torch.float32)
        _lib.gemm_weight_times_normed_t(pk, wv, n.buf, vt, B, HW, C, pairs=pairs)
        mixed = torch.empty(B, HW, C, device=dev, dtype=torch.float32)
        scale = float(C) ** (-0.5)
        if pairs and _lib.attention256_ok(B, HW, C):
            if key not in cache:
                gam = float(torch.sqrt((gn.weight.detach().double() ** 2).mean() + (gn.bias.detach().double() ** 2).mean()))
                cache[key] = (_lib.pairs_scale_from_rows(wqk, bqk, gam), _lib.pairs_scale_from_rows(wv, bv, gam))
            s_qk, s_v = cache[key]
            _lib.attention256(qk, vt, mixed, B, C, s_qk, s_v, scale, bias_v=bv)
            return self._pointwise_pairs(pk, _T(mixed, x.H, x.W, C), wo, bo, s_v, residual=x.buf, out_scale=out_scale, stats=True)
        logits = torch.empty(B, HW, HW, device=dev, dtype=torch.float32)
        _lib.gemm(qk, qk[:, C:], out=logits, M=HW, N=HW, K=C, lda=2 * C, ldb=2 * C, ldc=HW, batch=B,
                  stride_a=HW * 2 * C, stride_b=HW * 2 * C, stride_c=HW * HW)
        _lib.softmax_rows(logits, logits, B * HW, HW, scale)
        _lib.gemm(logits, vt, out=mixed, M=HW, N=C, K=HW, lda=HW, ldb=HW, ldc=C, batch=B,
                  stride_a=HW * HW, stride_b=C * HW, stride_c=HW * C, epilogue=_lib.make_epilogue(bias=bv))
        return self._pointwise(_T(mixed, x.H, x.W, C), wo, bo, residual=x.buf, out_scale=out_scale, stats=True)

    def _attention_heads(self, pk, x, n, gn, wqk, bqk, wv, bv, wo, bo, cache, key, out_scale, heads):
        B, HW, C = x.buf.shape[0], x.H * x.W, x.C
        D = C // heads
        pairs = self.pairs_admissible(gn, n.norm[1], transform=False)
        dev = x.buf.device
        qk = torch.empty(B * HW, 2 * C, device=dev, dtype=torch.float32)
        _lib.gemm_normed(pk, n.buf.view(-1, C), wqk, qk, epilogue=_lib.make_epilogue(bias=bqk), pairs=pairs)
        vt = torch.empty(B, C, HW, device=dev, dtype=torch.float32)
        _lib.gemm_weight_times_normed_t(pk, wv, n.buf, vt, B, HW, C, pairs=pairs)
        mixed = torch.empty(B, HW, C, device=dev, dtype=torch.float32)
        scale = float(D) ** (-0.5)
        if pairs and _lib.attention_heads_ok(B, HW, heads, D):
            if key not in cache:
                gam = float(torch.sqrt((gn.weight.detach().double() ** 2).mean() + (gn.bias.detach().double() ** 2).mean()))
                cache[key] = (_lib.pairs_scale_from_rows(wqk, bqk, gam), _lib.pairs_scale_from_rows(wv, bv, gam))
            s_qk, s_v = cache[key]
            _lib.attention_heads(qk, vt, mixed, B, HW, heads, D, s_qk, s_v, scale, bias_v=bv)
            return self._pointwise_pairs(pk, _T(mixed, x.H, x.W, C), wo, bo, s_v, residual=x.buf, out_scale=out_scale, stats=True)
        if D % 4:
            raise NotImplementedError(f"attention heads of {D} channels: the GEMM takes a head as a column view only where its width "
                                      "is a multiple of 4")
        logits = torch.empty(B, HW, HW, device=dev, dtype=torch.float32)
        for h in range(heads):
            _lib.gemm(qk[:, h * D:], qk[:, C + h * D:], out=logits, M=HW, N=HW, K=D, lda=2 * C, ldb=2 * C, ldc=HW, batch=B,
                      stride_a=HW * 2 * C, stride_b=HW * 2 * C, stride_c=HW * HW)
            _lib.softmax_rows(logits, logits, B * HW, HW, scale)
            _lib.gemm(logits, vt[:, h * D:(h + 1) * D], out=mixed[..., h * D:], M=HW, N=D, K=HW, lda=HW, ldb=HW, ldc=C, batch=B,
                      stride_a=HW * HW, stride_b=C * HW, stride_c=HW * C, epilogue=_lib.make_epilogue(bias=bv[h * D:(h + 1) * D]))
        return self._pointwise(_T(mixed, x.H, x.W, C), wo, bo, residual=x.buf, out_scale=out_scale, stats=True)

    def _box(self, x, up):
        B = x.buf.shape[0]
        y = self._new(B, x.H * 2 if up else x.H // 2, x.W * 2 if up else x.W // 2, x.C, x.buf)
        _lib.resample2x_nhwc(x.buf, y.buf, B, x.H, x.W, x.C, up)
        y.norm = x.norm
        return y

    def _add(self, a, b, scale):
        y = self._new(a.buf.shape[0], a.H, a.W, a.C, a.buf)
        _lib.add_scale(a.buf, b.buf, y.buf, a.buf.numel(), scale)
        return y

    def _cat(self, a, b):
        B = a.buf.shape[0]
        y = self._new(B, a.H, a.W, a.C + b.C, a.buf)
        _lib.concat_cols(a.buf, a.C, b.buf, b.C, y.buf, B * a.H * a.W)
        return y
```

### include/idiff_hip.h

```cpp
#ifndef IDIFF_HIP_H
#define IDIFF_HIP_H

#include <stdint.h>

#ifdef __cplusplus
extern "C" {
#endif

#define IDIFF_EINVAL 1001
#define IDIFF_ABI_VERSION 1

int idiff_abi_version(void);
const char *idiff_last_error(void);
const char *idiff_source_stamp(void);
const char *idiff_variant_flags(void);

int idiff_set_option(const char *name, int value);

int idiff_set_thread_option(const char *name, int value, int set);


int idiff_upfirdn2d_f32(const float *x, const float *k, float *out, int major, int in_h, int in_w, int minor,
                        int kh, int kw, int up_x, int up_y, int down_x, int down_y, int pad_x0, int pad_x1,
                        int pad_y0, int pad_y1, void *stream);

const char *idiff_upfirdn2d_route(const void *x, const void *out, int major, int in_h, int in_w, int minor, int kh, int kw,
                                  int up_x, int up_y, int down_x, int down_y, int pad_x0, int pad_x1, int pad_y0, int pad_y1);

int idiff_upfirdn2d_gn_f32(const float *x, const float *k, const float *coef, int act, float *out, int major, int in_h, int in_w,
                           int minor, int kh, int kw, int up_x, int up_y, int down_x, int down_y, int pad_x0, int pad_x1, int pad_y0,
                           int pad_y1, void *stream);
int idiff_upfirdn2d_gn_ok(const void *x, const void *coef, int act, const void *out, int major, int in_h, int in_w, int minor, int kh,
                          int kw, int up_x, int up_y, int down_x, int down_y, int pad_x0, int pad_x1, int pad_y0, int pad_y1);

int idiff_fused_bias_act_f32(const float *x, const float *b, const float *ref, float *out, int64_t n,
                             int step_b, int size_b, int act, int grad, float alpha, float scale, void *stream);

int idiff_upfirdn2d_f16(const void *x, const void *k, void *out, int major, int in_h, int in_w, int minor, int kh, int kw,
                        int up_x, int up_y, int down_x, int down_y, int pad_x0, int pad_x1, int pad_y0, int pad_y1, void *stream);
int idiff_upfirdn2d_f64(const double *x, const double *k, double *out, int major, int in_h, int in_w, int minor, int kh, int kw,
                        int up_x, int up_y, int down_x, int down_y, int pad_x0, int pad_x1, int pad_y0, int pad_y1, void *stream);
int idiff_fused_bias_act_f16(const void *x, const void *b, const void *ref, void *out, int64_t n, int step_b, int size_b,
                             int act, int grad, float alpha, float scale, void *stream);
int idiff_fused_bias_act_f64(const double *x, const double *b, const double *ref, double *out, int64_t n, int step_b,
                             int size_b, int act, int grad, float alpha, float scale, void *stream);


#define IDIFF_ACT_NONE 0
#define IDIFF_ACT_SILU 1
#define IDIFF_ACT_ELU 2
#define IDIFF_ACT_RELU 3
#define IDIFF_ACT_LRELU 4

typedef struct idiff_epilogue {
  const float *bias;
  const float *rowbias;
  int64_t ld_rowbias;
  int rows_per_group;
  int act;
  const float *residual;
  int64_t ld_residual;
  float out_scale;
  const float *rowscale;
  double *colstats;
} idiff_epilogue;

int idiff_gemm_f32(const float *A, int64_t lda, int64_t strideA, const float *Bt, int64_t ldb, int64_t strideB,
                   float *C, int64_t ldc, int64_t strideC, int M, int N, int K, int batch,
                   const idiff_epilogue *ep, void *stream);

int idiff_gemm_pairs_ok(int M, int N, int K, int batch);
int idiff_gemm_pairs_scale_f32(const float *w, int64_t ldw, int rows, int K, float *w_scale, void *stream);
int idiff_gemm_pairs_f32(const float *A, int64_t lda, int64_t strideA, const float *Bt, int64_t ldb, int64_t strideB,
                         const float *w_scale, int weight_is_a, const float *act_scale, float *C, int64_t ldc, int64_t strideC,
                         int M, int N, int K, int batch, const idiff_epilogue *ep, void *stream);

int idiff_pairs_act_scale_f32(const double *ws1, int nsplit1, int C1, const double *ws2, int nsplit2, int C2, int B, int HW, float *out,
                              void *stream);
int idiff_gemm_pairs_2src_f32(const float *A1, const float *A2, int64_t lda, int K1, const float *act_scale, const float *Bt, int64_t ldb,
                              const float *w_scale, float *C, int64_t ldc, int M, int N, int K, const idiff_epilogue *ep, void *stream);

int idiff_gemm_2src_f32(const float *A1, const float *A2, int64_t lda, int K1, const float *Bt, int64_t ldb, float *C,
                        int64_t ldc, int M, int N, int K, const idiff_epilogue *ep, void *stream);

int idiff_conv2d_nhwc_f32(const float *x, const float *wt, float *out, int B, int H, int W, int Cin, int Cout,
                          int KH, int KW, int stride, int pad_lo, int pad_hi, const idiff_epilogue *ep, void *stream);

const char *idiff_gemm_route(const void *A, int64_t lda, int64_t strideA, const void *Bt, int64_t ldb, int64_t strideB, const void *C,
                             int64_t ldc, int64_t strideC, int M, int N, int K, int batch, const idiff_epilogue *ep, int pairs);
const char *idiff_conv2d_route(const void *x, const void *wt, const void *out, int B, int H, int W, int Cin, int Cout, int KH, int KW,
                               int stride, int pad_lo, int pad_hi, const idiff_epilogue *ep);

int idiff_gemm_colstats_split(int M, int N, int K, int64_t lda, int64_t ldb, int rows_per_sample);
int idiff_conv2d_colstats_split(int B, int H, int W, int Cin, int Cout, int KH, int KW, int stride, int pad_lo,
                                int pad_hi);

int idiff_conv2d_winograd_ok(int B, int H, int W, int Cin, int Cout);
int64_t idiff_winograd_weight_floats(int Cin, int Cout);
int idiff_winograd_pack_f32(const float *wt, float *u, int Cin, int Cout, void *stream);
int idiff_conv2d_winograd_f32(const float *x, const float *u, float *out, int B, int H, int W, int Cin, int Cout,
                              const idiff_epilogue *ep, void *stream);
int idiff_conv2d_winograd_colstats_split(int B, int H, int W, int Cin, int Cout);
int idiff_conv2d_winograd43_ok(int B, int H, int W, int Cin, int Cout);
int idiff_conv2d_winograd43_colstats_split(int B, int H, int W, int Cin, int Cout);
int64_t idiff_winograd43_weight_floats(int Cin, int Cout);
int idiff_winograd43_pack_f32(const float *wt, float *u, int Cin, int Cout, void *stream);
int idiff_conv2d_winograd43_f32(const float *x, const float *u, float *out, int B, int H, int W, int Cin, int Cout,
                                const idiff_epilogue *ep, void *stream);
int idiff_conv2d_winograd43h_ok(int B, int H, int W, int Cin, int Cout);
int64_t idiff_winograd43h_weight_floats(int Cin, int Cout);
int idiff_winograd43h_pack_f32(const float *wt, float *u, int Cin, int Cout, void *stream);
int idiff_conv2d_winograd43h_f32(const float *x, const float *u, float *out, int B, int H, int W, int Cin, int Cout,
                                 const idiff_epilogue *ep, void *stream);

int idiff_conv2d_wino1d_ok(int B, int H, int W, int Cin, int Cout);
int idiff_conv2d_wino1d_colstats_split(int B, int H, int W, int Cin, int Cout);
int64_t idiff_wino1d_weight_floats(int Cin, int Cout);
int idiff_wino1d_pack_f32(const float *wt, float *u, int Cin, int Cout, void *stream);
int idiff_conv2d_wino1d_f32(const float *x, const float *u, float *out, int B, int H, int W, int Cin, int Cout,
                            const idiff_epilogue *ep, void *stream);
int idiff_conv2d_wino1d_gn_ok(int B, int H, int W, int Cin, int Cout, int groups);
int idiff_conv2d_wino1d_gn_f32(const float *x, const float *u, float *out, int B, int H, int W, int Cin, int Cout,
                               const idiff_epilogue *ep, int groups, const float *gamma, const float *beta, float eps, int act,
                               void *stream);
int idiff_conv2d_wino1d_normload_ok(int B, int H, int W, int Cin, int Cout);
int idiff_conv2d_wino1d_normload_f32(const float *x, const float *u, float *out, int B, int H, int W, int Cin, int Cout,
                                     const idiff_epilogue *ep, const float *coef, int act, void *stream);
int idiff_conv2d_wino1d_normload_2src_ok(int B, int H, int W, int C1, int C2, int Cout);
int idiff_conv2d_wino1d_normload_2src_f32(const float *x1, int C1, const float *x2, int C2, const float *u, float *out, int B, int H, int W,
                                          int Cout, const idiff_epilogue *ep, const float *coef, int act, void *stream);

int idiff_conv2d_winograd_split_ok(int B, int H, int W, int Cin, int Cout);
int64_t idiff_winograd_split_weight_floats(int Cin, int Cout);
int idiff_winograd_pack_split_f32(const float *wt, float *u, int Cin, int Cout, void *stream);
int idiff_conv2d_winograd_split_f32(const float *x, const float *u, float *out, int B, int H, int W, int Cin, int Cout,
                                    const idiff_epilogue *ep, void *stream);


int idiff_groupnorm_nsplit(int B, int HW, int C);
int idiff_groupnorm_stats_f32(const float *x, int C, const float *x2, int C2, int B, int HW, int G, float eps,
                              double *workspace, float *stats, void *stream);
int idiff_groupnorm_finalize_f32(const double *ws1, int nsplit1, int C1, const double *ws2, int nsplit2, int C2, int B,
                                 int HW, int G, float eps, float *stats, void *stream);
int idiff_groupnorm_apply_f32(const float *x, int C, const float *x2, int C2, int B, int HW, int G,
                              const float *stats, const float *gamma, const float *beta, const float *mod,
                              int64_t ld_mod, int act, float *y, void *stream);
int idiff_groupnorm_apply_colstats_f32(const float *x, int C, const float *x2, int C2, int B, int HW, int G,
                                       const double *ws1, int nsplit1, const double *ws2, int nsplit2, float eps,
                                       const float *gamma, const float *beta, const float *mod, int64_t ld_mod,
                                       int act, float *y, void *stream);
const char *idiff_groupnorm_apply_route(const void *x, int C, const void *x2, int C2, int B, int HW, int G, const void *stats,
                                        const void *gamma, const void *beta, const void *y);
const char *idiff_groupnorm_apply_colstats_route(const void *x, int C, const void *x2, int C2, int B, int HW, int G,
                                                 const double *ws1, int nsplit1, const double *ws2, int nsplit2,
                                                 const void *gamma, const void *beta, const void *y);
int idiff_groupnorm_coef_f32(const double *ws1, int nsplit1, int C1, const double *ws2, int nsplit2, int C2, int B, int HW, int G,
                             float eps, const float *gamma, const float *beta, float *coef, void *stream);

int idiff_softmax_rows_f32(const float *x, float *y, int64_t rows, int cols, float scale, void *stream);
const char *idiff_softmax_rows_route(const void *x, const void *y, int64_t rows, int cols, float scale);

int idiff_attention256_ok(int B, int tokens, int C);
int idiff_attention256_f32(const float *qk, int64_t ld_qk, const float *vt, const float *bias_v, const float *s_qk, const float *s_v,
                           float *out, int B, int tokens, int C, float scale, void *stream);

int idiff_attention_heads_ok(int B, int tokens, int H, int D);
int idiff_attention_heads_f32(const float *qk, int64_t ld_qk, const float *vt, const float *bias_v, const float *s_qk, const float *s_v,
                              float *out, int B, int tokens, int H, int D, float scale, void *stream);

const char *idiff_attention256_route(const void *qk, int64_t ld_qk, const void *vt, const void *bias_v, const void *s_qk, const void *s_v,
                                     const void *out, int B, int tokens, int C);
const char *idiff_attention_heads_route(const void *qk, int64_t ld_qk, const void *vt, const void *bias_v, const void *s_qk, const void *s_v,
                                        const void *out, int B, int tokens, int H, int D);

int idiff_affine_act_f32(const float *a, float *y, int64_t n, float alpha, float beta_const, int act,
                         const float *rowscale, int64_t inner, void *stream);
const char *idiff_affine_act_route(const void *a, const void *y, int64_t n, const void *rowscale, int64_t inner);
const char *idiff_add_scale_route(const void *a, const void *b, const void *y, int64_t n);
const char *idiff_concat_cols_route(const void *a, int Ca, const void *b, int Cb, const void *out, int64_t rows);
int idiff_add_scale_f32(const float *a, const float *b, float *y, int64_t n, float scale, void *stream);
int idiff_fourier_embed_f32(const float *t, const float *W, float *out, int B, int half, void *stream);
int idiff_positional_embed_f32(const float *t, float *out, int B, int dim, float max_positions, int mode, void *stream);
int idiff_concat_cols_f32(const float *a, int Ca, const float *b, int Cb, float *out, int64_t rows, void *stream);
int idiff_nchw_to_nhwc_f32(const float *x, float *y, int B, int C, int HW, int Cpad, float alpha, float beta,
                           void *stream);
int idiff_nhwc_to_nchw_f32(const float *x, float *y, int B, int C, int HW, int Cpad, const float *rowscale,
                           void *stream);
int idiff_perturb_f32(const float *x, const float *z, const float *std_, const float *mean_coeff, float *out,
                      int64_t rows, int64_t D, void *stream);
int idiff_perturb_randn_f32(const float *x, const float *std_, const float *mean_coeff, float *out, int64_t rows,
                            int64_t D, int64_t row0, uint64_t seed, float *z_out, void *stream);
int idiff_resample2x_nhwc_f32(const float *x, float *y, int B, int H, int W, int C, int up, void *stream);


int64_t idiff_spectrum_workspace_bytes(int P, int M, int D);
int idiff_spectrum_f32(const float *S, int P, int M, int D, void *workspace, int64_t workspace_bytes, float *sv,
                       double *eig_out, void *stream);
int idiff_colmean_f64(const float *S, int P, int M, int D, double *mean, double *scratch, void *stream);
int idiff_centered_gram_f64(const float *S, const double *mean, int P, int M, int D, double *G, void *stream);
int idiff_centered_gram_rows_f64(const float *S, const double *mean, int M, int D, int row0, int row1, double *G,
                                 void *stream);
int idiff_symmetrize_upper_f64(double *G, int D, void *stream);
int64_t idiff_symtridiag_scratch_doubles(int D);
int idiff_symband_ld(void);
int idiff_symband_f64(double *G, int D, double *scratch, void *stream);
int idiff_symtridiag_f64(double *G, int P, int D, double *diag, double *offdiag, double *scratch, void *stream);
int idiff_symtridiag_plan(int D);
int idiff_tridiag_eigvals_f64(const double *diag, const double *offdiag, int P, int D, double *eig, void *stream);

int64_t idiff_sym_lowvecs_scratch_doubles(int D, int k);
int idiff_sym_lowvecs_f64(double *G, int D, int k, double *T, double *ritz, double *resid, double *scratch, void *stream);

int64_t idiff_sym_topvecs_scratch_doubles(int N, int k, int p);
int idiff_sym_topvecs_f64(const double *K, int N, int k, int p, double lo, double hi, double top, int degree, int sweeps, double *V,
                          double *ritz, double *resid, double *scratch, void *stream);


int64_t idiff_knn_workspace_bytes(int N, int D, int k);
int idiff_knn_f32(const float *X, int N, int D, int k, void *workspace, int64_t workspace_bytes, double *dist, int64_t *idx,
                  int *n_exact_rows, void *stream);


int idiff_apsp_tile(void);
int idiff_knn_graph_f64(const double *dist, const int64_t *idx, int N, int k, double *G, void *stream);
int idiff_apsp_f64(double *G, int N, void *stream);
int64_t idiff_double_center_scratch_doubles(int N);
int idiff_double_center_f64(const double *D, int N, double *K, double *fro2, double *scratch, void *stream);

int64_t idiff_knn_cross_workspace_bytes(int M, int N);
int idiff_knn_cross_f64(const float *Xq, int M, const float *X, int N, int D, int k, void *workspace, int64_t workspace_bytes,
                        double *dist, int64_t *idx, void *stream);
int64_t idiff_isomap_project_scratch_doubles(int c);
int idiff_isomap_project_f64(const double *dist, const int64_t *idx, int M, int k, const double *D, int N, const double *A, int c,
                             const double *colmean, const double *grand, double *Z, double *scratch, void *stream);

int idiff_component_labels_f64(const double *D, int N, int32_t *labels, int32_t *count, int32_t *scratch, void *stream);
int64_t idiff_component_bridges_workspace_bytes(int C);
int idiff_component_bridges_f64(const float *X, int N, int D, const int32_t *labels, int C, void *workspace, int64_t workspace_bytes,
                                int64_t *bi, int64_t *bj, double *bw, void *stream);
int idiff_minplus_f64(const double *A, int64_t lda, const double *B, int64_t ldb, double *C, int64_t ldc, int m, int n, int p,
                      void *stream);
int idiff_symmetrize_min_f64(double *G, int N, void *stream);


// ... 74 lines not shown
```

Baseline: 18980.

## Pre-pack linear weights into LDS-image banks reused by the split/pairs GEMM

Adds a weight bank: each 1x1/attention/dense weight is packed once into the exact bf16-split or fp16-pair LDS tile image, cached per weight, and loaded directly into shared memory by a new BANK variant of the pipelined GEMM kernel. This skips the per-tile fp32 load and split/pair conversion of the weight operand on every call. The cost is extra device memory for the banks, a one-time pack, and new kernel template instantiations. Pre-packing weights, which are parameters and not activations, is legitimate caching.

New measurement: 19030 (median of 6 runs). No clear change (+0.3%).

```diff
diff --git a/id-diff_amd/_lib.py b/id-diff_amd/_lib.py
--- a/id-diff_amd/_lib.py
+++ b/id-diff_amd/_lib.py
@@ -1,6 +1,7 @@
 import ctypes
 import os
 import subprocess
+import weakref
 from typing import NamedTuple, Optional
 
 import torch
@@ -44,6 +45,13 @@
     "idiff_gemm_f32": (c_i, [c_p, c_i64, c_i64, c_p, c_i64, c_i64, c_p, c_i64, c_i64, c_i, c_i, c_i, c_i,
                              ctypes.POINTER(Epilogue), c_p]),
     "idiff_gemm_2src_f32": (c_i, [c_p, c_p, c_i64, c_i, c_p, c_i64, c_p, c_i64, c_i, c_i, c_i, ctypes.POINTER(Epilogue), c_p]),
+    "idiff_gemm_bank_bytes": (c_i64, [c_i, c_i, c_i]),
+    "idiff_gemm_bank_pack_f32": (c_i, [c_p, c_i64, c_i, c_i, c_i, c_p, c_p, c_p]),
+    "idiff_gemm_bank_ok": (c_i, [c_i, c_i, c_i, c_i, c_i]),
+    "idiff_gemm_bank_f32": (c_i, [c_p, c_p, c_i, c_i64, c_i64, c_p, c_i64, c_i64, c_p, c_i, c_i, c_i, c_i, c_p, c_i, c_p, c_p, c_i64, c_i64,
+                                  c_i, c_i, c_i, c_i, ctypes.POINTER(Epilogue), c_p]),
+    "idiff_gemm_bank_route": (ctypes.c_char_p, [c_p, c_p, c_i, c_i64, c_i64, c_p, c_i64, c_i64, c_p, c_i, c_i, c_i, c_i, c_i, c_p, c_i64,
+                                                c_i64, c_i, c_i, c_i, c_i, ctypes.POINTER(Epilogue)]),
     "idiff_conv2d_nhwc_f32": (c_i, [c_p, c_p, c_p] + [c_i] * 10 + [ctypes.POINTER(Epilogue), c_p]),
     "idiff_gemm_route": (ctypes.c_char_p, [c_p, c_i64, c_i64, c_p, c_i64, c_i64, c_p, c_i64, c_i64, c_i, c_i, c_i, c_i,
                                            ctypes.POINTER(Epilogue), c_i]),
@@ -398,6 +406,81 @@
     return out
 
 
+class _WeightBankEntry:
+    __slots__ = ("w", "banks", "__weakref__")
+
+    def __init__(self, w):
+        self.w, self.banks = w, {}
+
+
+_weight_banks = {}
+
+
+def register_weight_bank(cache, w):
+    key = (w.data_ptr(), w.shape[0], w.shape[1], w.stride(0))
+    owned = cache.setdefault("gemm_banks", {})
+    if key not in owned:
+        if w.dim() != 2 or w.stride(1) != 1:
+            raise RuntimeError(f"register_weight_bank: expected a 2-D K-contiguous weight, got shape {tuple(w.shape)} strides {w.stride()}")
+        entry = owned[key] = _WeightBankEntry(w)
+
+        def _gone(ref, key=key):
+            if _weight_banks.get(key) is ref:
+                del _weight_banks[key]
+        _weight_banks[key] = weakref.ref(entry, _gone)
+    return w
+
+
+def gemm_bank_bytes(rows, K, pairs=False):
+    n = lib().idiff_gemm_bank_bytes(rows, K, int(bool(pairs)))
+    if n <= 0:
+        _check(1, "idiff_gemm_bank_bytes")
+    return n
+
+
+def gemm_bank_pack(w, pairs=False, w_scale=None):
+    _dev(w, "w", contiguous=False)
+    rows, K = w.shape
+    bank = torch.empty(gemm_bank_bytes(rows, K, pairs), device=w.device, dtype=torch.uint8)
+    _check(lib().idiff_gemm_bank_pack_f32(w.data_ptr(), w.stride(0), rows, K, int(bool(pairs)), _ptr(w_scale), bank.data_ptr(), _stream()),
+           "idiff_gemm_bank_pack_f32")
+    return bank
+
+
+def gemm_bank_ok(M, N, K, batch=1, pairs=False):
+    return bool(lib().idiff_gemm_bank_ok(M, N, K, batch, int(bool(pairs))))
+
+
+def _weight_bank_for(w, rows, K, ldw, M, N, batch, pairs, w_scale):
+    if not _weight_banks:
+        return None
+    ref = _weight_banks.get((w.data_ptr(), rows, K, ldw))
+    entry = ref() if ref is not None else None
+    if entry is None or not gemm_bank_ok(M, N, K, batch, pairs):
+        return None
+    have = entry.banks.get(pairs)
+    if have is None or (pairs and have[1].data_ptr() != w_scale.data_ptr()):
+        have = entry.banks[pairs] = (gemm_bank_pack(entry.w, pairs, w_scale), w_scale)
+    return have[0]
+
+
+def gemm_bank_launch(a, a2, K1, lda, stride_a, bt, ldb, stride_b, bank, rows, pairs, w_scale, weight_is_a, act_scale, out, ldc, stride_c,
+                     M, N, K, batch, ep):
+    _check(lib().idiff_gemm_bank_f32(a.data_ptr(), _ptr(a2), K1, lda, stride_a, bt.data_ptr(), ldb, stride_b, bank.data_ptr(), rows, K,
+                                     int(bool(pairs)), int(bool(pairs)), _ptr(w_scale), int(bool(weight_is_a)), _ptr(act_scale), out.data_ptr(),
+                                     ldc, stride_c, M, N, K, batch, ep, _stream()), "idiff_gemm_bank_f32")
+    return out
+
+
+def gemm_bank_route(a, bt, bank, rows, out, M, N, K, lda, ldb, ldc, epilogue=None, batch=1, stride_a=0, stride_b=0, stride_c=0, pairs=False,
+                    weight_is_a=False, a2=None, K1=0, bank_K=None, bank_pairs=None):
+    name = lib().idiff_gemm_bank_route(_addr(a), 0 if a2 is None else _addr(a2), K1, lda, stride_a, _addr(bt), ldb, stride_b, _addr(bank),
+                                       rows, K if bank_K is None else bank_K, int(bool(pairs if bank_pairs is None else bank_pairs)),
+                                       int(bool(pairs)), int(bool(weight_is_a)), _addr(out), ldc, stride_c, M, N, K, batch,
+                                       _ep_ref(epilogue, "gemm_bank_route"))
+    return None if name is None else name.decode()
+
+
 def gemm(a, bt, out=None, epilogue=None, M=None, N=None, K=None, lda=None, ldb=None, ldc=None,
          batch=1, stride_a=0, stride_b=0, stride_c=0):
     explicit = M is not None
@@ -416,6 +499,10 @@
         ldc = out.stride(-2)
     _dev(out, "out", contiguous=not explicit)
     ep = _ep_ref(epilogue, "gemm")
+    bank = _weight_bank_for(bt, N, K, ldb, M, N, batch, False, None) if stride_b == 0 else None
+    if bank is not None:
+        return gemm_bank_launch(a, None, 0, lda, stride_a, bt, ldb, stride_b, bank, N, False, None, False, None, out, ldc, stride_c,
+                                M, N, K, batch, ep)
     _check(lib().idiff_gemm_f32(a.data_ptr(), lda, stride_a, bt.data_ptr(), ldb, stride_b, out.data_ptr(), ldc, stride_c,
                                 M, N, K, batch, ep, _stream()), "idiff_gemm_f32")
     return out
@@ -445,6 +532,11 @@
             raise RuntimeError(f"gemm_pairs: shapes {tuple(a.shape)} x {tuple(bt.shape)}^T -> {tuple(out.shape)}")
         lda, ldb, ldc = a.stride(0), bt.stride(0), out.stride(0)
     ep = _ep_ref(epilogue, "gemm_pairs")
+    w, rows, ldw, stride_w = (a, M, lda, stride_a) if weight_is_a else (bt, N, ldb, stride_b)
+    bank = _weight_bank_for(w, rows, K, ldw, M, N, batch, True, w_scale) if stride_w == 0 else None
+    if bank is not None:
+        return gemm_bank_launch(a, None, 0, lda, stride_a, bt, ldb, stride_b, bank, rows, True, w_scale, weight_is_a, act_scale, out, ldc,
+                                stride_c, M, N, K, batch, ep)
     _check(lib().idiff_gemm_pairs_f32(a.data_ptr(), lda, stride_a, bt.data_ptr(), ldb, stride_b, w_scale.data_ptr(), int(bool(weight_is_a)),
                                       _ptr(act_scale), out.data_ptr(), ldc, stride_c, M, N, K, batch, ep, _stream()), "idiff_gemm_pairs_f32")
     return out
@@ -465,6 +557,10 @@
     if a2.shape[0] != M or a1.stride(0) != a2.stride(0) or bt.shape[1] != K:
         raise RuntimeError(f"gemm_pairs_2src: shapes {tuple(a1.shape)} | {tuple(a2.shape)} x {tuple(bt.shape)}^T")
     ep = _ep_ref(epilogue, "gemm_pairs_2src")
+    bank = _weight_bank_for(bt, bt.shape[0], K, bt.stride(0), M, bt.shape[0], 1, True, w_scale)
+    if bank is not None:
+        return gemm_bank_launch(a1, a2, K1, a1.stride(0), 0, bt, bt.stride(0), 0, bank, bt.shape[0], True, w_scale, False, act_scale, out,
+                                out.stride(0), 0, M, bt.shape[0], K, 1, ep)
     _check(lib().idiff_gemm_pairs_2src_f32(a1.data_ptr(), a2.data_ptr(), a1.stride(0), K1, act_scale.data_ptr(), bt.data_ptr(), bt.stride(0),
                                            w_scale.data_ptr(), out.data_ptr(), out.stride(0), M, bt.shape[0], K, ep, _stream()),
            "idiff_gemm_pairs_2src_f32")
@@ -499,6 +595,10 @@
     if a2.shape[0] != M or a1.stride(0) != a2.stride(0) or bt.shape[1] != K:
         raise RuntimeError(f"gemm_2src: shapes {tuple(a1.shape)} | {tuple(a2.shape)} x {tuple(bt.shape)}^T")
     ep = _ep_ref(epilogue, "gemm_2src")
+    bank = _weight_bank_for(bt, bt.shape[0], K, bt.stride(0), M, bt.shape[0], 1, False, None)
+    if bank is not None:
+        return gemm_bank_launch(a1, a2, K1, a1.stride(0), 0, bt, bt.stride(0), 0, bank, bt.shape[0], False, None, False, None, out,
+                                out.stride(0), 0, M, bt.shape[0], K, 1, ep)
     _check(lib().idiff_gemm_2src_f32(a1.data_ptr(), a2.data_ptr(), a1.stride(0), K1, bt.data_ptr(), bt.stride(0), out.data_ptr(),
                                      out.stride(0), M, bt.shape[0], K, ep, _stream()), "idiff_gemm_2src_f32")
     return out
diff --git a/id-diff_amd/csrc/common.h b/id-diff_amd/csrc/common.h
--- a/id-diff_amd/csrc/common.h
+++ b/id-diff_amd/csrc/common.h
@@ -33,7 +33,7 @@
 
 enum Option { OPT_NO_WINOGRAD, OPT_NO_COLSTATS, OPT_NO_PIPE, OPT_SCALAR_EPILOGUE, OPT_DBUF_ONLY, OPT_TRIDIAG_ONESTAGE,
               OPT_UFD_ROWS, OPT_CHASE_WAVEFRONT, OPT_WINO_NGROUP, OPT_GRAM_SMALL_TILES, OPT_CHASE_SPIN_LIMIT, OPT_FAKE_CU_COUNT,
-              OPT_SBR_SYNC, OPT_SBR_FULL, OPT_NO_SPLIT, OPT_WINO_SPLIT, OPT_SBR_LOOKAHEAD, OPT_NO_WINO43, OPT_NO_WINO43H, OPT_NO_PAIRS, OPT_PAIRS_MIN_TILES, OPT_NO_FUSED_ATTN, OPT_NO_WINO1D, OPT_NO_FUSED_GN, OPT_NO_FUSED_GN_LOAD, OPT_NO_FUSED_GN_LOAD_2SRC, OPT_NO_FUSED_GN_FIR, OPT_COUNT };
+              OPT_SBR_SYNC, OPT_SBR_FULL, OPT_NO_SPLIT, OPT_WINO_SPLIT, OPT_SBR_LOOKAHEAD, OPT_NO_WINO43, OPT_NO_WINO43H, OPT_NO_PAIRS, OPT_PAIRS_MIN_TILES, OPT_NO_FUSED_ATTN, OPT_NO_WINO1D, OPT_NO_FUSED_GN, OPT_NO_FUSED_GN_LOAD, OPT_NO_FUSED_GN_LOAD_2SRC, OPT_NO_FUSED_GN_FIR, OPT_NO_WEIGHT_BANK, OPT_WEIGHT_BANK_SPLIT, OPT_COUNT };
 bool option(Option o);
 int option_value(Option o);
 
diff --git a/id-diff_amd/csrc/igemm.hip b/id-diff_amd/csrc/igemm.hip
--- a/id-diff_amd/csrc/igemm.hip
+++ b/id-diff_amd/csrc/igemm.hip
@@ -28,6 +28,9 @@
   uint32_t c_bytes, res_bytes;
   int buf_ep;
   const float *scale_a, *scale_b;
+  const void *bank;
+  uint32_t bank_bytes;
+  int bank_side;
 };
 
 __device__ __forceinline__ float4 ldg4(const float *p) { return *reinterpret_cast<const float4 *>(p); }
@@ -272,10 +275,14 @@
   return __builtin_bit_cast(float4, v);
 }
 
-template <int BM, int BN, int WARPS_M, int WARPS_N, bool CONV, bool DBUF, int SPLIT>
+constexpr int BANK_ROWS = 128;
+constexpr int bank_img_bytes(int planes) { return planes * BANK_ROWS * SP * 2; }
+
+template <int BM, int BN, int WARPS_M, int WARPS_N, bool CONV, bool DBUF, int SPLIT, int BANK = 0>
 __global__ void __launch_bounds__(WARPS_M *WARPS_N * 64, (DBUF || SPLIT) ? 2 : 4)
 igemm_pipe_kernel(const IgemmParams p) {
   static_assert(!(SPLIT && DBUF), "the split form uses one LDS buffer");
+  static_assert(!BANK || (SPLIT && !CONV && BM == BANK_ROWS && BN == BANK_ROWS && WARPS_M * WARPS_N == 4), "the bank holds 128-row tiles of a linear form");
   constexpr int T = WARPS_M * WARPS_N * 64;
   constexpr int WTM = BM / WARPS_M, WTN = BN / WARPS_N;
   constexpr int TM = WTM / 32, TN = WTN / 32;
@@ -348,6 +355,15 @@
   }
 
   float4 a_reg[A_PER_T], b_reg[B_PER_T];
+  constexpr int IMG = bank_img_bytes(PLANES);
+  constexpr int W_PER_T = BANK ? IMG / (T * 16) : 1;
+  struct BankState { uintx4 reg[W_PER_T]; __amdgpu_buffer_rsrc_t rsrc; uint32_t base; };
+  struct NoBank {};
+  std::conditional_t<BANK != 0, BankState, NoBank> wb;
+  if constexpr (BANK != 0) {
+    wb.rsrc = __builtin_amdgcn_make_buffer_rsrc(const_cast<void *>(p.bank), 0, (int)p.bank_bytes, 0x00020000);
+    wb.base = (uint32_t)((BANK == 2 ? tile_m : tile_n) * ((p.K + BK - 1) / BK)) * (uint32_t)IMG + (uint32_t)tid * 16u;
+  }
   int f_kt = 0, f_c0 = 0, f_tap = 0, f_ky = 0, f_kx = 0;
 
   const int ntaps = CONV ? p.K / p.Cin : 1;
@@ -380,10 +396,15 @@
       const __amdgpu_buffer_rsrc_t rS = second ? rA2 : rA;
       const uint32_t koff = (uint32_t)(f_kt * BK - (second ? p.K1 : 0)) * 4u;
 #pragma unroll
-      for (int i = 0; i < A_PER_T; ++i) a_reg[i] = buf_load4(rS, (a_mask[i] && kok) ? a_base[i] + koff : OOB);
-    }
-#pragma unroll
-    for (int i = 0; i < B_PER_T; ++i) b_reg[i] = buf_load4(rB, (b_ok[i] && kok) ? b_base[i] + koffb : OOB);
+      for (int i = 0; i < (BANK == 2 ? 0 : A_PER_T); ++i) a_reg[i] = buf_load4(rS, (a_mask[i] && kok) ? a_base[i] + koff : OOB);
+    }
+#pragma unroll
+    for (int i = 0; i < (BANK == 1 ? 0 : B_PER_T); ++i) b_reg[i] = buf_load4(rB, (b_ok[i] && kok) ? b_base[i] + koffb : OOB);
+    if constexpr (BANK != 0) {
+#pragma unroll
+      for (int i = 0; i < W_PER_T; ++i)
+        wb.reg[i] = __builtin_amdgcn_raw_buffer_load_b128(wb.rsrc, (int)(wb.base + (uint32_t)f_kt * (uint32_t)IMG + (uint32_t)(i * T * 16)), 0, 0);
+    }
     ++f_kt;
   };
 
@@ -391,10 +412,15 @@
   const int kc_sw = (((kc >> 3) ^ split_swz(row_base)) << 3) + (kc & 7);
   const float pair_sa = (SPLIT == 2 && p.scale_a) ? p.scale_a[0] : 1.f, pair_s = (SPLIT == 2 && p.scale_b) ? p.scale_b[0] : 1.f;
   auto stage = [&](int buf) {
+    if constexpr (BANK != 0) {
+      char *dst = reinterpret_cast<char *>(BANK == 2 ? As16 : Bs16) + tid * 16;
+#pragma unroll
+      for (int i = 0; i < W_PER_T; ++i) *reinterpret_cast<uintx4 *>(dst + i * T * 16) = wb.reg[i];
+    }
     if (SPLIT == 2) {
       unsigned short *a_dst = As16, *b_dst = Bs16;
 #pragma unroll
-      for (int i = 0; i < A_PER_T; ++i) {
+      for (int i = 0; i < (BANK == 2 ? 0 : A_PER_T); ++i) {
         uint2 hi, lo;
         const float4 av = a_reg[i];
         pair4(make_float4(av.x * pair_sa, av.y * pair_sa, av.z * pair_sa, av.w * pair_sa), hi, lo);
@@ -403,7 +429,7 @@
         *reinterpret_cast<uint2 *>(d + BM * SP) = lo;
       }
 #pragma unroll
-      for (int i = 0; i < B_PER_T; ++i) {
+      for (int i = 0; i < (BANK == 1 ? 0 : B_PER_T); ++i) {
         uint2 hi, lo;
         const float4 w = b_reg[i];
         pair4(make_float4(w.x * pair_s, w.y * pair_s, w.z * pair_s, w.w * pair_s), hi, lo);
@@ -416,7 +442,7 @@
     if (SPLIT) {
       unsigned short *a_dst = As16 + buf * 3 * BM * SP, *b_dst = Bs16 + buf * 3 * BN * SP;
 #pragma unroll
-      for (int i = 0; i < A_PER_T; ++i) {
+      for (int i = 0; i < (BANK == 2 ? 0 : A_PER_T); ++i) {
         uint2 q1, q2, q3;
         split4(a_reg[i], q1, q2, q3);
         unsigned short *d = a_dst + (row_base + i * ROW_STEP) * SP + kc_sw;
@@ -425,7 +451,7 @@
         *reinterpret_cast<uint2 *>(d + 2 * BM * SP) = q3;
       }
 #pragma unroll
-      for (int i = 0; i < B_PER_T; ++i) {
+      for (int i = 0; i < (BANK == 1 ? 0 : B_PER_T); ++i) {
         uint2 q1, q2, q3;
         split4(b_reg[i], q1, q2, q3);
         unsigned short *d = b_dst + (row_base + i * ROW_STEP) * SP + kc_sw;
@@ -786,7 +812,7 @@
   }
 }
 
-template <int BM, int BN, int WARPS_M, int WARPS_N, bool CONV, bool DBUF = true, int SPLIT = 0>
+template <int BM, int BN, int WARPS_M, int WARPS_N, bool CONV, bool DBUF = true, int SPLIT = 0, int BANK = 0>
 int launch_pipe(IgemmParams &p, int batch, hipStream_t st) {
   p.tiles_m = idiff::ceil_div(p.M, BM);
   p.tiles_n = idiff::ceil_div(p.N, BN);
@@ -794,7 +820,7 @@
                                        : (size_t)(DBUF ? 2 : 1) * (BM + BN) * LDS_PITCH * sizeof(float);
   constexpr size_t patch_bytes = (size_t)WARPS_M * WARPS_N * 32 * (BN / WARPS_N) * sizeof(float);
   constexpr size_t lds_bytes = stage_bytes > patch_bytes ? stage_bytes : patch_bytes;
-  auto kern = igemm_pipe_kernel<BM, BN, WARPS_M, WARPS_N, CONV, DBUF, SPLIT>;
+  auto kern = igemm_pipe_kernel<BM, BN, WARPS_M, WARPS_N, CONV, DBUF, SPLIT, BANK>;
   if (lds_bytes > 64 * 1024) {
     static idiff::AttrGuard guard;
     const void *fn = reinterpret_cast<const void *>(kern);
@@ -802,13 +828,13 @@
   }
   dim3 grid(p.tiles_m * p.tiles_n, batch);
   hipLaunchKernelGGL(kern, grid, dim3(WARPS_M * WARPS_N * 64), lds_bytes, st, p);
-  return idiff::launch_status(CONV ? "igemm_pipe_conv" : "igemm_pipe_linear");
+  return idiff::launch_status(CONV ? "igemm_pipe_conv" : BANK ? "igemm_pipe_linear_bank" : "igemm_pipe_linear");
 }
 
 enum IgemmFamily { FAM_PIPE, FAM_DIRECT_VEC, FAM_DIRECT_SCALAR, FAM_NARROW };
 enum IgemmArith { AR_FP32, AR_FP32_1BUF, AR_SPLIT, AR_PAIRS };
 enum IgemmEpForm { EPF_BUF_BLOCK, EPF_BUF_ROW, EPF_VEC64, EPF_SCALAR };
-struct IgemmPlan { int family, bm, bn, arith, ep_form; };
+struct IgemmPlan { int family, bm, bn, arith, ep_form, bank; };
 enum IgemmWant { WANT_PIPE, WANT_PAIRS, WANT_DIRECT_VEC, WANT_DIRECT_SCALAR };
 
 constexpr int64_t BUF_LIMIT = 0xFFFFFFF0ll;
@@ -877,9 +903,15 @@
   } else if (c.family == FAM_PIPE) {
     switch (c.arith) {
       case AR_PAIRS:
-        if constexpr (!CONV) { if (t == 128128) return launch_pipe<128, 128, 2, 2, false, false, 2>(p, batch, st); }
+        if constexpr (!CONV) {
+          if (t == 128128 && c.bank == 1) return launch_pipe<128, 128, 2, 2, false, false, 2, 1>(p, batch, st);
+          if (t == 128128 && c.bank == 2) return launch_pipe<128, 128, 2, 2, false, false, 2, 2>(p, batch, st);
+          if (t == 128128) return launch_pipe<128, 128, 2, 2, false, false, 2>(p, batch, st);
+        }
         break;
       case AR_SPLIT:
+        if constexpr (!CONV) { if (t == 128128 && c.bank == 1) return launch_pipe<128, 128, 2, 2, false, false, 1, 1>(p, batch, st); }
+        if (c.bank) break;
         if (t == 128128) return launch_pipe<128, 128, 2, 2, CONV, false, 1>(p, batch, st);
         if (t == 128032) return launch_pipe<128, 32, 4, 1, CONV, false, 1>(p, batch, st);
         if (t == 128064) return launch_pipe<128, 64, 2, 2, CONV, false, 1>(p, batch, st);
@@ -905,13 +937,19 @@
   static const char *const epf[] = {"buf-block", "buf-row", "vec64", "scalar"};
   static thread_local char text[64];
   if (c.family == FAM_NARROW) snprintf(text, sizeof(text), "narrow c%d fp32 %s", c.bn, c.ep_form == 2 ? "elem" : c.ep_form == 1 ? "row" : "none");
-  else snprintf(text, sizeof(text), "%s %dx%d %s %s", fam[c.family], c.bm, c.bn, ar[c.arith], epf[c.ep_form]);
+  else snprintf(text, sizeof(text), "%s %dx%d %s %s%s", fam[c.family], c.bm, c.bn, ar[c.arith], epf[c.ep_form], c.bank ? " bank" : "");
   return text;
+}
+
+bool bank_routed(const IgemmPlan &c) {
+  return !idiff::option(idiff::OPT_NO_WEIGHT_BANK) && c.family == FAM_PIPE && c.bm == BANK_ROWS && c.bn == BANK_ROWS &&
+         (c.arith == AR_PAIRS || (c.arith == AR_SPLIT && idiff::option(idiff::OPT_WEIGHT_BANK_SPLIT)));
 }
 
 template <bool CONV>
 int igemm_run(IgemmParams &p, int batch, int want, hipStream_t st, IgemmPlan *probe) {
-  const IgemmPlan c = igemm_choose(p, batch, want);
+  IgemmPlan c = igemm_choose(p, batch, want);
+  if (!CONV && p.bank && bank_routed(c)) c.bank = p.bank_side;
   if (p.has_ep && p.ep.colstats && c.family == FAM_PIPE && p.M % c.bm)
     return idiff::fail("%s: colstats with M = %d rows in tiles of %d: no whole tiles (ask idiff_%s_colstats_split first)", CONV ? "conv2d" : "gemm",
                        p.M, c.bm, CONV ? "conv2d" : "gemm");
@@ -960,6 +998,37 @@
     out[0] = ldexpf(1.f, sh);
     out[1] = ldexpf(1.f, -sh);
   }
+}
+template <int PAIRS>
+__global__ void __launch_bounds__(256) bank_pack_kernel(const float *__restrict__ w, int64_t ldw, int rows, int K, const float *__restrict__ scale,
+                                                        unsigned short *__restrict__ bank) {
+  constexpr int PLANES = PAIRS ? 2 : 3;
+  const int nkt = gridDim.x, kt = blockIdx.x, tile = blockIdx.y;
+  const int tid = threadIdx.x, kc = (tid & 7) * 4, row_base = tid >> 3;
+  const float s = (PAIRS && scale) ? scale[0] : 1.f;
+  unsigned short *img = bank + ((int64_t)tile * nkt + kt) * (PLANES * BANK_ROWS * SP);
+#pragma unroll
+  for (int i = 0; i < BANK_ROWS / 32; ++i) {
+    const int row = row_base + i * 32, r = tile * BANK_ROWS + row, k = kt * BK + kc;
+    float4 v = make_float4(0.f, 0.f, 0.f, 0.f);
+    if (r < rows && k < K) v = ldg4(w + (int64_t)r * ldw + k);
+    unsigned short *d = img + row * SP + (((kc >> 3) ^ split_swz(row)) << 3) + (kc & 7);
+    if (PAIRS) {
+      uint2 hi, lo;
+      pair4(make_float4(v.x * s, v.y * s, v.z * s, v.w * s), hi, lo);
+      *reinterpret_cast<uint2 *>(d) = hi;
+      *reinterpret_cast<uint2 *>(d + BANK_ROWS * SP) = lo;
+    } else {
+      uint2 q1, q2, q3;
+      split4(v, q1, q2, q3);
+      *reinterpret_cast<uint2 *>(d) = q1;
+      *reinterpret_cast<uint2 *>(d + BANK_ROWS * SP) = q2;
+      *reinterpret_cast<uint2 *>(d + 2 * BANK_ROWS * SP) = q3;
+    }
+  }
+}
+int64_t bank_bytes(int rows, int K, int pairs) {
+  return (int64_t)idiff::ceil_div(rows, BANK_ROWS) * idiff::ceil_div(K, BK) * bank_img_bytes(pairs ? 2 : 3);
 }
 bool pairs_geometry_ok(int M, int N, int K, int batch) {
   if (M <= 0 || N <= 64 || K <= 0 || K % 4 || batch <= 0 || batch > 65535) return false;
@@ -1044,6 +1113,9 @@
   int want;
   const float *w_scale, *act_scale;
   int weight_is_a;
+  bool banked;
+  const void *bank;
+  int bank_rows, bank_K, bank_pairs;
 };
 
 int linear_front(const LinearCall &c, hipStream_t st, IgemmPlan *probe) {
@@ -1054,6 +1126,18 @@
                      : fail("%s: bad sizes M=%d N=%d K=%d batch=%d", c.name, c.M, c.N, c.K, c.batch);
   if (c.M == 0 || c.N == 0 || c.batch == 0) { if (probe) probe->family = -1; return 0; }
   if (!c.A || (c.two_src && !c.A2) || !c.Bt || !c.C || (pairs && !c.w_scale)) return fail("%s: null pointer", c.name);
+  if (c.banked) {
+    const int rows = c.weight_is_a ? c.M : c.N;
+    if (!c.bank) return fail("%s: null bank", c.name);
+    if (!aligned16(c.bank)) return fail("%s: the bank must be 16-byte aligned", c.name);
+    if (c.bank_pairs != (pairs ? 1 : 0) || c.bank_rows != rows || c.bank_K != c.K)
+      return fail("%s: the bank was packed for %d x %d %s, the weight of this call is %d x %d %s", c.name, c.bank_rows, c.bank_K,
+                  c.bank_pairs ? "fp16 pairs" : "bf16 x 3", rows, c.K, pairs ? "fp16 pairs" : "bf16 x 3");
+    if (c.weight_is_a && !pairs) return fail("%s: the weight as the left operand is a form of the fp16 pairs", c.name);
+    if (c.K % 4 || (c.weight_is_a ? c.lda : c.ldb) % 4) return fail("%s: K and the weight's row pitch must be multiples of 4", c.name);
+    if (c.batch > 1 && (c.weight_is_a ? c.strideA : c.strideB) != 0) return fail("%s: one weight for every batch slice (stride 0)", c.name);
+    if (bank_bytes(rows, c.K, pairs) >= BUF_LIMIT) return fail("%s: bank beyond one buffer descriptor", c.name);
+  }
   if (c.K1 % BK) return fail("%s: the split column K1 = %d must be a multiple of %d", c.name, c.K1, BK);
   if (c.lda < c.K1 || c.lda < c.K - c.K1 || c.ldb < c.K || c.ldc < c.N) return fail("%s: leading dimension smaller than the row length", c.name);
   if (pairs && !pairs_geometry_ok(c.M, c.N, c.K, c.batch))
@@ -1088,12 +1172,14 @@
   p.a_bytes = (uint32_t)extent_bytes(c.M, c.lda, c.two_src ? c.K1 : c.K); p.b_bytes = (uint32_t)extent_bytes(c.N, c.ldb, c.K);
   if (c.two_src) { p.A2 = c.A2; p.K1 = c.K1; p.a2_bytes = (uint32_t)extent_bytes(c.M, c.lda, c.K - c.K1); }
   if (pairs) { p.scale_a = c.weight_is_a ? c.w_scale : c.act_scale; p.scale_b = c.weight_is_a ? c.act_scale : c.w_scale; }
+  if (c.banked) { p.bank = c.bank; p.bank_bytes = (uint32_t)bank_bytes(c.bank_rows, c.bank_K, c.bank_pairs); p.bank_side = c.weight_is_a ? 2 : 1; }
   return igemm_run<false>(p, c.batch, c.want, st, probe);
 }
 
 LinearCall linear_call(const char *name, const float *A, int64_t lda, int64_t strideA, const float *Bt, int64_t ldb, int64_t strideB, float *C,
                        int64_t ldc, int64_t strideC, int M, int N, int K, int batch, const idiff_epilogue *ep, int want) {
-  return LinearCall{name, A, nullptr, 0, false, Bt, C, lda, ldb, ldc, strideA, strideB, strideC, M, N, K, batch, ep, want, nullptr, nullptr, 0};
+  return LinearCall{name, A, nullptr, 0, false, Bt, C, lda, ldb, ldc, strideA, strideB, strideC, M, N, K, batch, ep, want, nullptr, nullptr, 0,
+                    false, nullptr, 0, 0, 0};
 }
 LinearCall linear_call_2src(const char *name, const float *A1, const float *A2, int64_t lda, int K1, const float *Bt, int64_t ldb, float *C,
                             int64_t ldc, int M, int N, int K, const idiff_epilogue *ep, int want) {
@@ -1138,6 +1224,61 @@
   LinearCall c = linear_call(pairs ? "gemm_pairs" : "gemm", (const float *)A, lda, strideA, (const float *)Bt, ldb, strideB,
                              (float *)const_cast<void *>(C), ldc, strideC, M, N, K, batch, ep, pairs ? WANT_PAIRS : WANT_PIPE);
   c.w_scale = c.Bt;
+  if (linear_front(c, nullptr, &plan)) return nullptr;
+  return plan.family < 0 ? "none" : igemm_plan_name(plan);
+}
+
+IDIFF_API int64_t idiff_gemm_bank_bytes(int rows, int K, int pairs) {
+  if (rows <= 0 || K <= 0) { idiff::fail("gemm_bank_bytes: bad shape rows=%d K=%d", rows, K); return 0; }
+  return bank_bytes(rows, K, pairs);
+}
+
+IDIFF_API int idiff_gemm_bank_ok(int M, int N, int K, int batch, int pairs) {
+  if (M <= 0 || N <= 0 || K <= 0 || K % 4 || batch <= 0 || idiff::option(idiff::OPT_NO_PIPE)) return 0;
+  if (pairs && !pairs_geometry_ok(M, N, K, batch)) return 0;
+  return bank_routed(igemm_tile(M, N, batch, pairs ? WANT_PAIRS : WANT_PIPE)) ? 1 : 0;
+}
+
+IDIFF_API int idiff_gemm_bank_pack_f32(const float *W, int64_t ldw, int rows, int K, int pairs, const float *w_scale, void *bank, void *stream) {
+  using namespace idiff;
+  if (!W || !bank || (pairs && !w_scale)) return fail("gemm_bank_pack: null pointer");
+  if (rows <= 0 || K <= 0 || K % 4 || ldw < K || ldw % 4) return fail("gemm_bank_pack: bad shape rows=%d K=%d ldw=%lld (K and ldw multiples of 4)", rows, K, (long long)ldw);
+  if (!aligned16(W) || !aligned16(bank)) return fail("gemm_bank_pack: the weight and the bank must be 16-byte aligned");
+  if (bank_bytes(rows, K, pairs) >= BUF_LIMIT || ceil_div(rows, BANK_ROWS) > 65535) return fail("gemm_bank_pack: weight too large for one bank");
+  const dim3 grid(ceil_div(K, BK), ceil_div(rows, BANK_ROWS));
+  if (pairs) hipLaunchKernelGGL(bank_pack_kernel<1>, grid, dim3(256), 0, (hipStream_t)stream, W, ldw, rows, K, w_scale, (unsigned short *)bank);
+  else hipLaunchKernelGGL(bank_pack_kernel<0>, grid, dim3(256), 0, (hipStream_t)stream, W, ldw, rows, K, (const float *)nullptr, (unsigned short *)bank);
+  return launch_status("gemm_bank_pack");
+}
+
+namespace {
+LinearCall bank_call(const float *A, const float *A2, int K1, int64_t lda, int64_t strideA, const float *Bt, int64_t ldb, int64_t strideB,
+                     const void *bank, int bank_rows, int bank_K, int bank_pairs, int pairs, const float *w_scale, int weight_is_a,
+                     const float *act_scale, float *C, int64_t ldc, int64_t strideC, int M, int N, int K, int batch, const idiff_epilogue *ep) {
+  LinearCall c = linear_call("gemm_bank", A, lda, strideA, Bt, ldb, strideB, C, ldc, strideC, M, N, K, batch, ep, pairs ? WANT_PAIRS : WANT_PIPE);
+  if (A2 || K1) { c.A2 = A2; c.K1 = K1; c.two_src = true; }
+  c.w_scale = w_scale; c.act_scale = act_scale; c.weight_is_a = weight_is_a;
+  c.banked = true; c.bank = bank; c.bank_rows = bank_rows; c.bank_K = bank_K; c.bank_pairs = bank_pairs;
+  return c;
+}
+}
+
+IDIFF_API int idiff_gemm_bank_f32(const float *A, const float *A2, int K1, int64_t lda, int64_t strideA, const float *Bt, int64_t ldb,
+                                  int64_t strideB, const void *bank, int bank_rows, int bank_K, int bank_pairs, int pairs,
+                                  const float *w_scale, int weight_is_a, const float *act_scale, float *C, int64_t ldc, int64_t strideC, int M,
+                                  int N, int K, int batch, const idiff_epilogue *ep, void *stream) {
+  if ((A2 || K1) && batch != 1) return idiff::fail("gemm_bank: two sources are unbatched");
+  return linear_front(bank_call(A, A2, K1, lda, strideA, Bt, ldb, strideB, bank, bank_rows, bank_K, bank_pairs, pairs, w_scale, weight_is_a,
+                                act_scale, C, ldc, strideC, M, N, K, batch, ep), (hipStream_t)stream, nullptr);
+}
+
+IDIFF_API const char *idiff_gemm_bank_route(const void *A, const void *A2, int K1, int64_t lda, int64_t strideA, const void *Bt, int64_t ldb,
+                                            int64_t strideB, const void *bank, int bank_rows, int bank_K, int bank_pairs, int pairs,
+                                            int weight_is_a, const void *C, int64_t ldc, int64_t strideC, int M, int N, int K, int batch,
+                                            const idiff_epilogue *ep) {
+  IgemmPlan plan = {};
+  LinearCall c = bank_call((const float *)A, (const float *)A2, K1, lda, strideA, (const float *)Bt, ldb, strideB, bank, bank_rows, bank_K, bank_pairs,
+                           pairs, (const float *)Bt, weight_is_a, nullptr, (float *)const_cast<void *>(C), ldc, strideC, M, N, K, batch, ep);
   if (linear_front(c, nullptr, &plan)) return nullptr;
   return plan.family < 0 ? "none" : igemm_plan_name(plan);
 }
diff --git a/id-diff_amd/csrc/runtime.hip b/id-diff_amd/csrc/runtime.hip
--- a/id-diff_amd/csrc/runtime.hip
+++ b/id-diff_amd/csrc/runtime.hip
@@ -17,7 +17,7 @@
                                              "IDIFF_DBUF_ONLY", "IDIFF_TRIDIAG_ONESTAGE", "IDIFF_UFD_ROWS", "IDIFF_CHASE_WAVEFRONT",
                                              "IDIFF_WINO_NGROUP", "IDIFF_GRAM_SMALL_TILES", "IDIFF_CHASE_SPIN_LIMIT",
                                              "IDIFF_FAKE_CU_COUNT", "IDIFF_SBR_SYNC", "IDIFF_SBR_FULL", "IDIFF_NO_SPLIT", "IDIFF_WINO_SPLIT", "IDIFF_SBR_LOOKAHEAD",
-                                             "IDIFF_NO_WINO43", "IDIFF_NO_WINO43H", "IDIFF_NO_PAIRS", "IDIFF_PAIRS_MIN_TILES", "IDIFF_NO_FUSED_ATTN", "IDIFF_NO_WINO1D", "IDIFF_NO_FUSED_GN", "IDIFF_NO_FUSED_GN_LOAD", "IDIFF_NO_FUSED_GN_LOAD_2SRC", "IDIFF_NO_FUSED_GN_FIR"};
+                                             "IDIFF_NO_WINO43", "IDIFF_NO_WINO43H", "IDIFF_NO_PAIRS", "IDIFF_PAIRS_MIN_TILES", "IDIFF_NO_FUSED_ATTN", "IDIFF_NO_WINO1D", "IDIFF_NO_FUSED_GN", "IDIFF_NO_FUSED_GN_LOAD", "IDIFF_NO_FUSED_GN_LOAD_2SRC", "IDIFF_NO_FUSED_GN_FIR", "IDIFF_NO_WEIGHT_BANK", "IDIFF_WEIGHT_BANK_SPLIT"};
 struct OptionTable {
   int v[OPT_COUNT];
   OptionTable() {
diff --git a/id-diff_amd/models/ncsnpp.py b/id-diff_amd/models/ncsnpp.py
--- a/id-diff_amd/models/ncsnpp.py
+++ b/id-diff_amd/models/ncsnpp.py
@@ -344,7 +344,7 @@
                 sc = self._pointwise(x, ws, bs)
             elif fused:
                 sc = self._new(x.buf.shape[0], x.H, x.W, ws.shape[0], x.buf)
-                _lib.gemm_2src(x.buf.view(-1, x.C), x2.buf.view(-1, x2.C), ws, sc.buf.view(-1, ws.shape[0]),
+                _lib.gemm_2src(x.buf.view(-1, x.C), x2.buf.view(-1, x2.C), _lib.register_weight_bank(pk, ws), sc.buf.view(-1, ws.shape[0]),
                                epilogue=_lib.make_epilogue(bias=bs))
             else:
                 part = self._pointwise(x, ws[0], bs)
diff --git a/id-diff_amd/models/nhwc.py b/id-diff_amd/models/nhwc.py
--- a/id-diff_amd/models/nhwc.py
+++ b/id-diff_amd/models/nhwc.py
@@ -221,7 +221,8 @@
         y = self._new(B, x.H, x.W, cout, x.buf)
         if stats:
             self._colstats(y, _lib.gemm_colstats_split(B * x.H * x.W, cout, cin, cin, w.stride(0), x.H * x.W), ep)
-        _lib.gemm(x.buf.view(-1, cin), w, out=y.buf.view(-1, cout), epilogue=_lib.make_epilogue(bias=bias, **ep))
+        _lib.gemm(x.buf.view(-1, cin), _lib.register_weight_bank(self._packed, w), out=y.buf.view(-1, cout),
+                  epilogue=_lib.make_epilogue(bias=bias, **ep))
         return y
 
     def _pointwise_pairs(self, pk, x, w, bias, act_scale, stats=False, **ep):
@@ -233,7 +234,7 @@
         y = self._new(B, x.H, x.W, cout, x.buf)
         if stats:
             self._colstats(y, _lib.gemm_colstats_split(M, cout, cin, cin, w.stride(0), x.H * x.W), ep)
-        _lib.gemm_pairs(x.buf.view(-1, cin), w, _lib._pairs_scale_of(pk, w), y.buf.view(-1, cout),
+        _lib.gemm_pairs(x.buf.view(-1, cin), _lib.register_weight_bank(pk, w), _lib._pairs_scale_of(pk, w), y.buf.view(-1, cout),
                         epilogue=_lib.make_epilogue(bias=bias, **ep), act_scale=act_scale)
         return y
 
@@ -244,6 +245,7 @@
         pairs = self.pairs_admissible(gn, n.norm[1], transform=False)
         dev = x.buf.device
         qk = torch.empty(B * HW, 2 * C, device=dev, dtype=torch.float32)
+        _lib.register_weight_bank(pk, wqk); _lib.register_weight_bank(pk, wv)
         _lib.gemm_normed(pk, n.buf.view(-1, C), wqk, qk, epilogue=_lib.make_epilogue(bias=bqk), pairs=pairs)
         vt = torch.empty(B, C, HW, device=dev, dtype=torch.float32)
         _lib.gemm_weight_times_normed_t(pk, wv, n.buf, vt, B, HW, C, pairs=pairs)
@@ -270,6 +272,7 @@
         pairs = self.pairs_admissible(gn, n.norm[1], transform=False)
         dev = x.buf.device
         qk = torch.empty(B * HW, 2 * C, device=dev, dtype=torch.float32)
+        _lib.register_weight_bank(pk, wqk); _lib.register_weight_bank(pk, wv)
         _lib.gemm_normed(pk, n.buf.view(-1, C), wqk, qk, epilogue=_lib.make_epilogue(bias=bqk), pairs=pairs)
         vt = torch.empty(B, C, HW, device=dev, dtype=torch.float32)
         _lib.gemm_weight_times_normed_t(pk, wv, n.buf, vt, B, HW, C, pairs=pairs)
diff --git a/include/idiff_hip.h b/include/idiff_hip.h
--- a/include/idiff_hip.h
+++ b/include/idiff_hip.h
@@ -90,6 +90,17 @@
                              int64_t ldc, int64_t strideC, int M, int N, int K, int batch, const idiff_epilogue *ep, int pairs);
 const char *idiff_conv2d_route(const void *x, const void *wt, const void *out, int B, int H, int W, int Cin, int Cout, int KH, int KW,
                                int stride, int pad_lo, int pad_hi, const idiff_epilogue *ep);
+
+int64_t idiff_gemm_bank_bytes(int rows, int K, int pairs);
+int idiff_gemm_bank_pack_f32(const float *W, int64_t ldw, int rows, int K, int pairs, const float *w_scale, void *bank, void *stream);
+int idiff_gemm_bank_ok(int M, int N, int K, int batch, int pairs);
+int idiff_gemm_bank_f32(const float *A, const float *A2, int K1, int64_t lda, int64_t strideA, const float *Bt, int64_t ldb, int64_t strideB,
+                        const void *bank, int bank_rows, int bank_K, int bank_pairs, int pairs, const float *w_scale, int weight_is_a,
+                        const float *act_scale, float *C, int64_t ldc, int64_t strideC, int M, int N, int K, int batch,
+                        const idiff_epilogue *ep, void *stream);
+const char *idiff_gemm_bank_route(const void *A, const void *A2, int K1, int64_t lda, int64_t strideA, const void *Bt, int64_t ldb,
+                                  int64_t strideB, const void *bank, int bank_rows, int bank_K, int bank_pairs, int pairs, int weight_is_a,
+                                  const void *C, int64_t ldc, int64_t strideC, int M, int N, int K, int batch, const idiff_epilogue *ep);
 
 int idiff_gemm_colstats_split(int M, int N, int K, int64_t lda, int64_t ldb, int rows_per_sample);
 int idiff_conv2d_colstats_split(int B, int H, int W, int Cin, int Cout, int KH, int KW, int stride, int pad_lo,
```
